# SinOncology/BreakID

Hardware: AMD Instinct MI355X
Metric: M reads/s clustered+split-scanned (higher is better)
Workload: dtype int32/u8 (+f64 sd replay)

## Files before the change

breakid_amd/capi.py:

```python
from __future__ import annotations

import ctypes as C
import math
import os
import subprocess

import numpy as np

from . import abi

_HERE = os.path.dirname(os.path.abspath(__file__))
LIB_PATH = os.path.join(_HERE, "libbreakid_hip.so")
_LIB = None


class BreakIDError(RuntimeError):
    def __init__(self, code, msg):
        super().__init__("libbreakid_hip error %d: %s" % (code, msg))
        self.code = code


def build(verbose=False):
    cmd = ["make", "-C", os.path.join(_HERE, "csrc"), "-j8"]
    r = subprocess.run(cmd, capture_output=not verbose, text=True)
    if r.returncode != 0:
        raise RuntimeError("building libbreakid_hip.so failed:\n" + (r.stdout or "")[-4000:] + (r.stderr or "")[-4000:])


EXPORTS = ["bk_init", "bk_prepare_process", "bk_free", "bk_last_error", "bk_set_stream", "bk_sync", "bk_get_stream", "bk_upload_records", "bk_records", "bk_exclude_regions", "bk_isize_stats",
           "bk_discordant_pairs", "bk_mask_and_cluster", "bk_split_evidence", "bk_cluster_summary",
           "bk_split_breakpoints", "bk_normal_support", "bk_ref_support", "bk_genotype_call", "bk_clip_support", "bk_clip_reads", "bk_base_depth", "bk_clip_rescue", "bk_junctions", "bk_junction_sides", "bk_vcf_breakend_alt", "bk_evidence", "bk_unique_support", "bk_clip_consensus", "bk_junction_fit", "bk_locus_similarity", "bk_window_coverage", "bk_call_windows", "bk_fusion_frame", "bk_link_calls", "bk_locus_partners", "bk_call_partner_sites", "bk_run", "bk_fetch", "bk_timing", "bk_timing_enable", "bk_timing_touched", "bk_group_stats", "bk_qname_hash", "bk_qname_check",
           "bk_bam_open", "bk_bam_header", "bk_bam_decode", "bk_bam_close", "bk_bam_extract", "bk_bam_names_free", "bk_bam_reads", "bk_reads_free", "bk_bam_decode_device", "bk_bam_decode_device_part", "bk_bam_decode_device_ctx", "bk_bam_dev_free", "bk_feed_release_caches", "bk_debug_bgzf_inflate", "bk_debug_std_sort", "bk_debug_scan", "bk_debug_radix_sort", "bk_debug_prims_info", "bk_sort_forms", "bk_debug_ahc", "bk_debug_points", "bk_debug_cigar", "bk_debug_vote", "bk_debug_region", "bk_shard_begin", "bk_shard_get_stats", "bk_shard_set_stats",
           "bk_shard_sd_local", "bk_shard_sd_finish", "bk_shard_buffer", "bk_shard_set_buffer", "bk_shard_group_sizes",
           "bk_shard_own_groups", "bk_shard_route_candidates", "bk_shard_group_keys", "bk_shard_route_pairs", "bk_shard_group_pairs", "bk_shard_bp_cov", "bk_shard_bp_vote", "bk_shard_bp_vote_slice", "bk_shard_bp_set_voted", "bk_shard_bp_depth", "bk_shard_bp_finish"]


def lib():
    global _LIB
    if _LIB is None:
        if not os.path.exists(LIB_PATH):
            raise BreakIDError(abi.BK_ERR_NO_DEVICE, "libbreakid_hip.so is not built (run __graft_entry__.build()); "
                                                     "there is no CPU fallback")
        try:
            import torch
        except Exception:
            pass
        L = C.CDLL(LIB_PATH)
        vp, u64p, dp = C.c_void_p, C.POINTER(C.c_uint64), C.POINTER(C.c_double)
        L.bk_init.argtypes = [C.c_int, vp, C.POINTER(C.c_char_p), C.c_int, C.POINTER(vp)]
        L.bk_free.argtypes = [vp]
        L.bk_last_error.restype = C.c_char_p
        L.bk_last_error.argtypes = [vp]
        L.bk_set_stream.argtypes = [vp, vp]
        L.bk_sync.argtypes = [vp]
        L.bk_upload_records.argtypes = [vp, C.POINTER(abi.Soa), C.c_int]
        L.bk_records.argtypes = [vp, C.POINTER(abi.Soa)]
        L.bk_exclude_regions.argtypes = [vp, C.POINTER(abi.Regions), u64p]
        L.bk_isize_stats.argtypes = [vp, dp, dp]
        L.bk_discordant_pairs.argtypes = [vp, C.c_int, C.c_double, u64p, C.POINTER(C.c_uint32)]
        L.bk_mask_and_cluster.argtypes = [vp, C.c_double, C.c_int, u64p]
        L.bk_split_evidence.argtypes = [vp, u64p]
        L.bk_cluster_summary.argtypes = [vp, C.c_double, u64p]
        L.bk_split_breakpoints.argtypes = [vp, C.c_double, u64p]
        L.bk_run.argtypes = [vp, C.c_int, C.c_int, dp, u64p]
        L.bk_normal_support.argtypes = [vp, vp, C.c_double, C.POINTER(vp), u64p]
        L.bk_ref_support.argtypes = [vp, vp, C.c_int, C.c_int, C.c_double, C.POINTER(vp), u64p]
        L.bk_genotype_call.argtypes = [C.c_uint32, C.c_uint32, C.POINTER(C.c_uint8), C.POINTER(C.c_uint8), C.POINTER(C.c_float)]
        L.bk_clip_support.argtypes = [vp, vp, C.c_int, C.c_int, C.c_double, C.POINTER(vp), u64p]
        L.bk_clip_reads.argtypes = [vp, vp, C.c_uint64, C.c_int, C.c_int, C.POINTER(vp), C.POINTER(vp), C.POINTER(vp)]
        L.bk_base_depth.argtypes = [vp, vp, vp, C.c_uint64, C.POINTER(vp)]
        L.bk_clip_rescue.argtypes = [vp, vp, vp, C.c_uint32] + [C.POINTER(C.c_uint32)] * 4
        L.bk_junctions.argtypes = [vp, C.POINTER(vp), u64p]
        L.bk_junction_sides.argtypes = [vp, C.POINTER(C.c_uint8), C.POINTER(C.c_uint8), C.POINTER(C.c_uint8)]
        L.bk_vcf_breakend_alt.argtypes = [C.c_char, C.c_int, C.c_char_p, C.c_uint32, C.c_int, C.c_char_p, C.c_size_t]
        L.bk_evidence.argtypes = [vp, C.POINTER(vp), u64p, C.POINTER(C.POINTER(C.c_uint64))]
        L.bk_unique_support.argtypes = [vp, C.POINTER(vp), u64p, C.POINTER(C.POINTER(C.c_uint64)), u64p]
        L.bk_clip_consensus.argtypes = [vp, C.POINTER(abi.Reads), vp, C.c_uint64, C.c_int, C.c_int, C.c_uint32, C.c_uint32, C.POINTER(vp), C.POINTER(vp), C.POINTER(vp)]
        L.bk_junction_fit.argtypes = [vp, C.POINTER(abi.RefSeq), vp, C.c_uint64, vp, C.c_uint32, C.c_uint32, C.c_uint32, C.c_uint32, C.POINTER(vp)]
        L.bk_locus_similarity.argtypes = [vp, C.POINTER(abi.RefSeq), vp, C.c_uint64, C.c_uint32, C.POINTER(vp)]
        L.bk_window_coverage.argtypes = [vp, vp, C.c_uint64, C.c_int, C.POINTER(vp)]
        L.bk_call_windows.argtypes = [vp, C.c_int, C.c_int, C.c_uint32, vp, vp]
        L.bk_fusion_frame.argtypes = [vp, C.POINTER(abi.TxModel), vp, C.c_uint64, C.POINTER(vp)]
        L.bk_link_calls.argtypes = [vp, vp, C.c_uint64, C.c_uint32, C.POINTER(vp)]
        L.bk_locus_partners.argtypes = [vp, vp, C.c_uint64, C.c_uint32, C.POINTER(vp)]
        L.bk_call_partner_sites.argtypes = [vp, C.c_double, vp]
        L.bk_fetch.argtypes = [vp, C.c_int, C.POINTER(vp), u64p, C.POINTER(C.POINTER(C.c_uint64)), C.POINTER(C.c_uint32)]
        L.bk_timing.argtypes = [vp, C.POINTER(C.POINTER(C.c_char_p)), C.POINTER(C.POINTER(C.c_float)),
                                C.POINTER(C.POINTER(C.c_uint64)), C.POINTER(C.c_int)]
        L.bk_timing_enable.argtypes = [vp, C.c_int]
        L.bk_timing_touched.argtypes = [vp, C.POINTER(C.POINTER(C.c_uint64)), C.POINTER(C.c_int)]
        L.bk_debug_std_sort.argtypes = [vp, vp, vp, C.c_uint32, vp]
        L.bk_debug_scan.argtypes = [vp, C.c_int, vp, C.c_uint64, C.c_int, vp]
        L.bk_debug_radix_sort.argtypes = [vp, vp, vp, C.c_uint64, C.c_int, C.c_int, vp, vp]
        L.bk_debug_prims_info.argtypes = [u64p]
        L.bk_sort_forms.argtypes = [vp, u64p]
        L.bk_debug_ahc.argtypes = [vp, vp, vp, C.c_uint32, C.c_double, vp, vp, C.POINTER(C.c_uint32)]
        L.bk_debug_points.argtypes = [vp, C.c_int, vp, vp, C.c_uint32, C.c_double, vp, vp, C.POINTER(C.c_uint32)]
        L.bk_debug_cigar.argtypes = [vp, C.c_uint32, vp, vp, vp, vp, vp, vp, vp]
        L.bk_debug_vote.argtypes = [vp, vp, C.c_uint32, vp, C.c_uint32, C.c_int32, C.c_int32, vp]
        L.bk_debug_region.argtypes = [vp, C.c_int32, C.c_uint32, C.c_uint32, C.c_uint64, vp, C.c_uint32, C.POINTER(C.c_uint32), C.POINTER(C.c_uint32),
                                      C.POINTER(C.c_uint32)]
        L.bk_shard_begin.argtypes = [vp, C.c_uint64, C.c_int]
        L.bk_shard_get_stats.argtypes = [vp, C.POINTER(abi.ShardStats)]
        L.bk_shard_set_stats.argtypes = [vp, C.POINTER(abi.ShardStats)]
        L.bk_shard_sd_local.argtypes = [vp, u64p, C.POINTER(vp), u64p]
        L.bk_shard_sd_finish.argtypes = [vp, vp, C.c_uint64, C.c_uint64, dp, dp]
        L.bk_shard_buffer.argtypes = [vp, C.c_int, C.POINTER(vp), u64p, C.POINTER(C.c_uint32)]
        L.bk_shard_set_buffer.argtypes = [vp, C.c_int, vp, C.c_uint64]
        L.bk_shard_group_sizes.argtypes = [vp, C.POINTER(C.POINTER(C.c_uint64)), C.POINTER(C.c_uint32)]
        L.bk_shard_own_groups.argtypes = [vp, vp, C.c_uint32]
        L.bk_shard_route_candidates.argtypes = [vp, C.c_uint32, C.POINTER(vp), C.POINTER(C.POINTER(C.c_uint64))]
        L.bk_shard_group_keys.argtypes = [vp, C.POINTER(C.POINTER(C.c_uint32)), C.POINTER(C.c_uint32)]
        L.bk_shard_route_pairs.argtypes = [vp, vp, C.c_uint32, C.c_uint32, C.POINTER(vp), C.POINTER(C.POINTER(C.c_uint64))]
        L.bk_shard_group_pairs.argtypes = [vp, vp, C.c_uint64, vp, C.c_uint32]
        L.bk_shard_bp_cov.argtypes = [vp, C.c_double, C.POINTER(vp), u64p]
        L.bk_shard_bp_vote.argtypes = [vp, C.c_double, vp]
        L.bk_shard_bp_vote_slice.argtypes = [vp, C.c_double, vp, C.c_uint64, C.c_uint64, C.POINTER(vp), C.POINTER(vp)]
        L.bk_shard_bp_set_voted.argtypes = [vp, vp]
        L.bk_shard_bp_depth.argtypes = [vp, C.POINTER(vp), u64p]
        L.bk_shard_bp_finish.argtypes = [vp, vp]
        L.bk_qname_hash.restype = C.c_uint64
        L.bk_qname_hash.argtypes = [C.c_char_p, C.c_size_t]
        L.bk_qname_check.restype = C.c_uint32
        L.bk_qname_check.argtypes = [C.c_char_p, C.c_size_t]
        L.bk_bam_open.argtypes = [C.c_char_p, C.POINTER(vp), C.c_char_p, C.c_size_t]
        L.bk_bam_header.argtypes = [vp, C.POINTER(C.c_int), C.POINTER(C.POINTER(C.c_char_p)), C.POINTER(C.POINTER(C.c_uint32))]
        L.bk_bam_decode.argtypes = [vp, C.POINTER(abi.Soa), C.c_char_p, C.c_size_t]
        L.bk_bam_close.argtypes = [vp]
        L.bk_bam_extract.argtypes = [C.c_char_p, C.c_char_p, vp, C.c_uint64, C.POINTER(C.c_char_p), C.c_uint64, C.POINTER(vp), u64p, C.c_char_p, C.c_size_t]
        L.bk_bam_names_free.argtypes = [vp]
        L.bk_bam_reads.argtypes = [C.c_char_p, vp, C.c_uint64, C.POINTER(abi.Reads), C.c_char_p, C.c_size_t]
        L.bk_reads_free.argtypes = [C.POINTER(abi.Reads)]
        L.bk_reads_free.restype = None
        L.bk_bam_names_free.restype = None
        L.bk_bam_decode_device.argtypes = [C.c_char_p, C.c_int, C.POINTER(vp), C.POINTER(abi.Soa), C.POINTER(C.c_int), C.POINTER(C.POINTER(C.c_char_p)),
                                           C.POINTER(C.POINTER(C.c_uint32)), C.c_char_p, C.c_size_t]
        L.bk_bam_decode_device_part.argtypes = [C.c_char_p, C.c_int, C.c_int, C.c_int, C.POINTER(vp), C.POINTER(abi.Soa), C.POINTER(C.c_int), C.POINTER(C.POINTER(C.c_char_p)),
                                           C.POINTER(C.POINTER(C.c_uint32)), C.c_char_p, C.c_size_t]
        L.bk_bam_dev_free.argtypes = [vp]
        L.bk_feed_release_caches.argtypes = []
        L.bk_feed_release_caches.restype = None
        L.bk_bam_decode_device_ctx.argtypes = [C.c_char_p, C.c_int, C.c_int, C.POINTER(vp), C.POINTER(vp), C.POINTER(C.c_int), C.POINTER(C.POINTER(C.c_char_p)),
                                               C.POINTER(C.POINTER(C.c_uint32)), C.c_char_p, C.c_size_t]
        L.bk_debug_bgzf_inflate.argtypes = [vp, C.c_uint64, vp, C.c_uint64, C.POINTER(C.c_uint64), C.POINTER(C.c_float), C.c_char_p, C.c_size_t]
        _LIB = L
    return _LIB


MULTI_LIB_PATH = os.path.join(_HERE, "libbreakid_rccl.so")
_MULTI = None
TRANSPORT_AUTO, TRANSPORT_RCCL, TRANSPORT_LOCAL = 0, 1, 2


def multi_lib():
    global _MULTI
    if _MULTI is None:
        lib()
        if not os.path.exists(MULTI_LIB_PATH):
            raise BreakIDError(abi.BK_ERR_NO_DEVICE, "libbreakid_rccl.so is not built (run __graft_entry__.build())")
        M = C.CDLL(MULTI_LIB_PATH)
        vp, dp = C.c_void_p, C.POINTER(C.c_double)
        M.bk_multi_run.argtypes = [C.POINTER(abi.Soa), vp, C.POINTER(C.c_char_p), C.c_int, C.c_int, C.c_int, C.c_int, C.c_int, dp, C.POINTER(C.c_uint64), C.POINTER(vp),
                                   C.c_char_p, C.c_size_t]
        M.bk_multi_stats.argtypes = [vp, dp, dp, C.POINTER(vp), C.POINTER(C.c_uint32)]
        M.bk_multi_free.argtypes = [vp]
        M.bk_multi_free.restype = None
        _MULTI = M
    return _MULTI


def multi_run(contigs, cols, n_gpus, transport=TRANSPORT_LOCAL, qual=20, fast=True):
    M = multi_lib()
    qc = cols.get("qcheck")
    cols = {k: np.ascontiguousarray(cols[k], dtype=dt) for k, dt in abi.SOA_COLS}
    if qc is not None:
        cols["qcheck"] = np.ascontiguousarray(qc, dtype=np.uint32)
    for k in ("cigar", "aux"):
        if cols[k].size == 0:
            cols[k] = np.zeros(1, cols[k].dtype)
    soa = abi.soa_from_numpy(cols)
    lens = np.asarray([l for _, l in contigs], dtype=np.uint32)
    names = (C.c_char_p * len(contigs))(*[n.encode() for n, _ in contigs])
    w, ncl, h = C.c_double(), C.c_uint64(), C.c_void_p()
    err = C.create_string_buffer(512)
    rc = M.bk_multi_run(C.byref(soa), lens.ctypes.data, names, len(contigs), int(n_gpus), int(transport), int(qual), int(fast), C.byref(w), C.byref(ncl), C.byref(h), err, 512)
    if rc != 0:
        raise BreakIDError(rc, err.value.decode())
    try:
        mean, sd = C.c_double(), C.c_double()
        rc = M.bk_multi_stats(h, C.byref(mean), C.byref(sd), None, None)
        if rc != 0:
            raise BreakIDError(rc, "bk_multi_stats")
        L = lib()
        clusters, _ = abi.fetch_array(L, h, lambda hh, st, d, c, g, ng: L.bk_fetch(hh, st, d, c, g, ng), abi.STAGE_CLUSTERS)
        return {"w": w.value, "n_clustered": ncl.value, "mean": mean.value, "sd": sd.value, "clusters": clusters}
    finally:
        M.bk_multi_free(h)


def prims_info():
    out = (C.c_uint64 * 4)()
    rc = lib().bk_debug_prims_info(out)
    if rc != 0:
        raise BreakIDError(rc, "bk_debug_prims_info")
    return dict(zip(("BLOCK", "SCAN_TILE", "SCAN_ONE_MAX", "RS_TILE"), (int(v) for v in out)))


def w_from(mean, sd):
    times = 2
    return times * math.sqrt(times) * (mean + 3 * sd)


def genotype_call(alt, ref):
    gt, gq, vaf = C.c_uint8(), C.c_uint8(), C.c_float()
    rc = lib().bk_genotype_call(int(alt), int(ref), C.byref(gt), C.byref(gq), C.byref(vaf))
    if rc != 0:
        raise BreakIDError(rc, "bk_genotype_call")
    return gt.value, gq.value, np.float32(vaf.value)


def junction_sides(row):
    a = np.zeros(1, abi.JUNCTION)
    a[0] = row
    r1, r2, src = C.c_uint8(), C.c_uint8(), C.c_uint8()
    rc = lib().bk_junction_sides(a.ctypes.data, C.byref(r1), C.byref(r2), C.byref(src))
    if rc != 0:
        raise BreakIDError(rc, "bk_junction_sides")
    return r1.value, r2.value, src.value


def clip_rescue(cluster, junction, clip, min_support=3):
    c, j, s = np.zeros(1, abi.CLUSTER), np.zeros(1, abi.JUNCTION), np.zeros(1, abi.CLIP_SUPPORT)
    c[0], j[0], s[0] = cluster, junction, clip
    out = [C.c_uint32() for _ in range(4)]
    rc = lib().bk_clip_rescue(c.ctypes.data, j.ctypes.data, s.ctypes.data, int(min_support), *[C.byref(o) for o in out])
    if rc < 0:
        raise BreakIDError(rc, "bk_clip_rescue")
    return tuple(o.value for o in out) if rc == 1 else None


def call_windows(cluster, right1, right2, flank, target_len):
    c = np.zeros(1, abi.CLUSTER)
    c[0] = cluster
    lens = np.ascontiguousarray(target_len, np.uint32)
    out = np.zeros(5, abi.COV_WINDOW)
    rc = lib().bk_call_windows(c.ctypes.data, int(right1), int(right2), int(flank), lens.ctypes.data, out.ctypes.data)
    if rc != 0:
        raise BreakIDError(rc, "bk_call_windows")
    return out


def call_partner_sites(cluster, w):
    c = np.zeros(1, abi.CLUSTER)
    c[0] = cluster
    out = np.zeros(2, abi.PARTNER_SITE)
    rc = lib().bk_call_partner_sites(c.ctypes.data, float(w), out.ctypes.data)
    if rc != 0:
        raise BreakIDError(rc, "bk_call_partner_sites")
    return out


def vcf_breakend_alt(ref_base, own_right, mate_chr, mate_pos, mate_right, cap=None):
    chrom = mate_chr.encode()
    if cap is None:
        cap = len(chrom) + 32
    buf = C.create_string_buffer(max(int(cap), 1))
    rc = lib().bk_vcf_breakend_alt(ref_base.encode(), int(bool(own_right)), chrom, int(mate_pos), int(bool(mate_right)), buf, int(cap))
    if rc != 0:
        raise BreakIDError(rc, "bk_vcf_breakend_alt")
    return buf.value.decode()


class Context:

    def __init__(self, contigs, device=0):
        self.L = lib()
        self.contigs = list(contigs)
        lens = np.asarray([l for _, l in contigs], dtype=np.uint32)
        names = (C.c_char_p * len(contigs))(*[n.encode() for n, _ in contigs])
        h = C.c_void_p()
        rc = self.L.bk_init(device, lens.ctypes.data, names, len(contigs), C.byref(h))
        if rc != 0:
            raise BreakIDError(rc, (self.L.bk_last_error(None) or b"").decode())
        self.h = h
        self._keep = None

    def close(self):
        if self.h:
            self.L.bk_free(self.h)
            self.h = None

    def __del__(self):
        try:
            self.close()
        except Exception:
            pass

    def _check(self, rc):
        if rc != 0:
            raise BreakIDError(rc, (self.L.bk_last_error(self.h) or b"").decode())

    def set_stream(self, hip_stream_handle):
        self._check(self.L.bk_set_stream(self.h, C.c_void_p(hip_stream_handle)))

    def sync(self):
        self._check(self.L.bk_sync(self.h))

    def upload(self, cols):
        qc = cols.get("qcheck")
        cols = {k: np.ascontiguousarray(cols[k], dtype=dt) for k, dt in abi.SOA_COLS}
        if qc is not None:
            cols["qcheck"] = np.ascontiguousarray(qc, dtype=np.uint32)
        for k in ("cigar", "aux"):
            if cols[k].size == 0:
                cols[k] = np.zeros(1, cols[k].dtype)
        soa = abi.soa_from_numpy(cols)
        self._keep = (cols, soa)
        self._check(self.L.bk_upload_records(self.h, C.byref(soa), abi.BK_MEM_HOST))

    def attach_device_table(self, table):
        self._keep = table
        self._check(self.L.bk_upload_records(self.h, C.byref(table.soa), abi.BK_MEM_DEVICE))

    def upload_soa(self, handle):
        self._keep = handle
        self._check(self.L.bk_upload_records(self.h, C.byref(handle.soa), abi.BK_MEM_HOST))

    def attach_device(self, ptrs, n, n_cigar_words, n_aux_bytes):
        s = abi.Soa()
        s.n = n
        for name, _ in abi.SOA_COLS:
            setattr(s, name, ptrs[name])
        if ptrs.get("qcheck"):
            s.qcheck = ptrs["qcheck"]
        if ptrs.get("side"):
            s.side = ptrs["side"]
        s.n_cigar_words = n_cigar_words
        s.n_aux_bytes = n_aux_bytes
        self._keep = (ptrs, s)
        self._check(self.L.bk_upload_records(self.h, C.byref(s), abi.BK_MEM_DEVICE))

    def exclude_regions(self, tid, beg, end):
        tid, beg, end = (np.ascontiguousarray(a, np.int32).reshape(-1) for a in (tid, beg, end))
        if not len(tid) == len(beg) == len(end):
            raise ValueError("exclude_regions: tid, beg and end differ in length")
        r = abi.Regions(tid.ctypes.data, beg.ctypes.data, end.ctypes.data, len(tid))
        n = C.c_uint64()
        self._check(self.L.bk_exclude_regions(self.h, C.byref(r), C.byref(n)))
        return n.value

    def isize_stats(self):
        m, s = C.c_double(), C.c_double()
        self._check(self.L.bk_isize_stats(self.h, C.byref(m), C.byref(s)))
        return m.value, s.value

    def shard_begin(self, rec_base, qual=20):
        self._check(self.L.bk_shard_begin(self.h, int(rec_base), int(qual)))

    def shard_get_stats(self):
        st = abi.ShardStats()
        self._check(self.L.bk_shard_get_stats(self.h, C.byref(st)))
        return st

    def shard_set_stats(self, st):
        self._check(self.L.bk_shard_set_stats(self.h, C.byref(st)))

    def shard_sd_local(self):
        lt, ex, nex = C.c_uint64(), C.c_void_p(), C.c_uint64()
        self._check(self.L.bk_shard_sd_local(self.h, C.byref(lt), C.byref(ex), C.byref(nex)))
        return lt.value, ex.value, nex.value

    def shard_sd_finish(self, all_ex_ptr, n_all, l_grand):
        m, s = C.c_double(), C.c_double()
        self._check(self.L.bk_shard_sd_finish(self.h, C.c_void_p(all_ex_ptr or 0), int(n_all), int(l_grand), C.byref(m), C.byref(s)))
        return m.value, s.value

    def discordant_pairs(self, qual, w):
        n, g = C.c_uint64(), C.c_uint32()
        self._check(self.L.bk_discordant_pairs(self.h, qual, w, C.byref(n), C.byref(g)))
        return n.value, g.value

    def mask_and_cluster(self, w, fast):
        n = C.c_uint64()
        self._check(self.L.bk_mask_and_cluster(self.h, w, int(fast), C.byref(n)))
        return n.value

    def split_evidence(self):
        n = C.c_uint64()
        self._check(self.L.bk_split_evidence(self.h, C.byref(n)))
        return n.value

    def cluster_summary(self, w):
        n = C.c_uint64()
        self._check(self.L.bk_cluster_summary(self.h, w, C.byref(n)))
        return n.value

    def split_breakpoints(self, w, count=True):
        n = C.c_uint64()
        self._check(self.L.bk_split_breakpoints(self.h, w, C.byref(n) if count else None))
        return n.value

    def normal_support(self, normal, w):
        data, n = C.c_void_p(), C.c_uint64()
        self._check(self.L.bk_normal_support(self.h, normal.h, w, C.byref(data), C.byref(n)))
        if not n.value:
            return np.zeros(0, abi.NORMAL_SUPPORT)
        buf = (C.c_char * (n.value * abi.NORMAL_SUPPORT.itemsize)).from_address(data.value)
        return np.frombuffer(buf, dtype=abi.NORMAL_SUPPORT, count=n.value).copy()

    def junctions(self):
        data, n = C.c_void_p(), C.c_uint64()
        self._check(self.L.bk_junctions(self.h, C.byref(data), C.byref(n)))
        if not n.value:
            return np.zeros(0, abi.JUNCTION)
        buf = (C.c_char * (n.value * abi.JUNCTION.itemsize)).from_address(data.value)
        return np.frombuffer(buf, dtype=abi.JUNCTION, count=n.value).copy()

    def evidence(self):
        data, n, off = C.c_void_p(), C.c_uint64(), C.POINTER(C.c_uint64)()
        self._check(self.L.bk_evidence(self.h, C.byref(data), C.byref(n), C.byref(off)))
        rows = np.zeros(0, abi.EVIDENCE)
        if n.value:
            buf = (C.c_char * (n.value * abi.EVIDENCE.itemsize)).from_address(data.value)
            rows = np.frombuffer(buf, dtype=abi.EVIDENCE, count=n.value).copy()
        d2, ncl = C.c_void_p(), C.c_uint64()
        self._check(self.L.bk_fetch(self.h, abi.STAGE_CLUSTERS, C.byref(d2), C.byref(ncl), None, None))
        return rows, np.ctypeslib.as_array(off, shape=(ncl.value + 1,)).copy()

    def unique_support(self, listing=True):
        data, n, first, n_rows = C.c_void_p(), C.c_uint64(), C.POINTER(C.c_uint64)(), C.c_uint64()
        if listing:
            self._check(self.L.bk_unique_support(self.h, C.byref(data), C.byref(n), C.byref(first), C.byref(n_rows)))
        else:
            self._check(self.L.bk_unique_support(self.h, C.byref(data), C.byref(n), None, None))
        rows = np.zeros(0, abi.UNIQUE_SUPPORT)
        if n.value:
            buf = (C.c_char * (n.value * abi.UNIQUE_SUPPORT.itemsize)).from_address(data.value)
            rows = np.frombuffer(buf, dtype=abi.UNIQUE_SUPPORT, count=n.value).copy()
        if not listing:
            return rows
        return rows, (np.ctypeslib.as_array(first, shape=(n_rows.value,)).copy() if n_rows.value else np.zeros(0, np.uint64))

    def clip_consensus(self, reads, sites, mapq_min, min_clip, max_len=64, min_depth=2, col_depth=True):
        sites = np.ascontiguousarray(sites, abi.CLIP_SITE)
        assert sites.ndim == 1
        n = len(sites)
        t, keep = reads_struct(reads)
        out, bases, depth = C.c_void_p(), C.c_void_p(), C.c_void_p()
        self._check(self.L.bk_clip_consensus(self.h, C.byref(t), sites.ctypes.data if n else None, n, int(mapq_min), int(min_clip), int(max_len), int(min_depth),
                                             C.byref(out), C.byref(bases), C.byref(depth) if col_depth else None))
        del keep
        if not n:
            return np.zeros(0, abi.CONSENSUS), np.zeros((0, int(max_len)), np.uint8), (np.zeros((0, int(max_len)), np.uint32) if col_depth else None)
        buf = (C.c_char * (n * abi.CONSENSUS.itemsize)).from_address(out.value)
        rows = np.frombuffer(buf, dtype=abi.CONSENSUS, count=n).copy()
        b = np.ctypeslib.as_array(C.cast(bases, C.POINTER(C.c_uint8)), shape=(n, int(max_len))).copy()
        d = np.ctypeslib.as_array(C.cast(depth, C.POINTER(C.c_uint32)), shape=(n, int(max_len))).copy() if col_depth else None
        return rows, b, d

    def junction_fit(self, ref, probes, query, max_shift=32, max_ins=32, max_hom=32):
        probes = np.ascontiguousarray(probes, abi.JUNCTION_PROBE)
        query = np.ascontiguousarray(query, np.uint8)
        assert probes.ndim == 1 and query.ndim == 2 and query.shape[0] == len(probes)
        n, max_len = len(probes), query.shape[1]
        t, keep = refseq_struct(ref)
        out = C.c_void_p()
        self._check(self.L.bk_junction_fit(self.h, C.byref(t), probes.ctypes.data if n else None, n, query.ctypes.data if n else None, max_len, int(max_shift), int(max_ins),
                                           int(max_hom), C.byref(out)))
        del keep
        if not n:
            return np.zeros(0, abi.JUNCTION_FIT)
        buf = (C.c_char * (n * abi.JUNCTION_FIT.itemsize)).from_address(out.value)
        return np.frombuffer(buf, dtype=abi.JUNCTION_FIT, count=n).copy()

    def locus_similarity(self, ref, pairs, flank=150):
        pairs = np.ascontiguousarray(pairs, abi.LOCUS_PAIR)
        assert pairs.ndim == 1
        n = len(pairs)
        t, keep = refseq_struct(ref)
        out = C.c_void_p()
        self._check(self.L.bk_locus_similarity(self.h, C.byref(t), pairs.ctypes.data if n else None, n, int(flank), C.byref(out)))
        del keep
        if not n:
            return np.zeros(0, abi.LOCUS_SIM)
        buf = (C.c_char * (n * abi.LOCUS_SIM.itemsize)).from_address(out.value)
        return np.frombuffer(buf, dtype=abi.LOCUS_SIM, count=n).copy()

    def ref_support(self, records, mapq_min, anchor, w):
        data, n = C.c_void_p(), C.c_uint64()
        self._check(self.L.bk_ref_support(self.h, records.h, int(mapq_min), int(anchor), w, C.byref(data), C.byref(n)))
        if not n.value:
            return np.zeros(0, abi.REF_SUPPORT)
        buf = (C.c_char * (n.value * abi.REF_SUPPORT.itemsize)).from_address(data.value)
        return np.frombuffer(buf, dtype=abi.REF_SUPPORT, count=n.value).copy()

    def clip_support(self, records, mapq_min, min_clip, w):
        data, n = C.c_void_p(), C.c_uint64()
        self._check(self.L.bk_clip_support(self.h, records.h, int(mapq_min), int(min_clip), w, C.byref(data), C.byref(n)))
        if not n.value:
            return np.zeros(0, abi.CLIP_SUPPORT)
        buf = (C.c_char * (n.value * abi.CLIP_SUPPORT.itemsize)).from_address(data.value)
        return np.frombuffer(buf, dtype=abi.CLIP_SUPPORT, count=n.value).copy()

    def clip_reads(self, sites, mapq_min, min_clip, listing=True):
        sites = np.ascontiguousarray(sites, abi.CLIP_SITE)
        assert sites.ndim == 1
        n = len(sites)
        counts, rows, off = C.c_void_p(), C.c_void_p(), C.c_void_p()
        self._check(self.L.bk_clip_reads(self.h, sites.ctypes.data if n else None, n, int(mapq_min), int(min_clip), C.byref(counts),
                                         C.byref(rows) if listing else None, C.byref(off) if listing else None))
        cnt = np.ctypeslib.as_array(C.cast(counts, C.POINTER(C.c_uint32)), shape=(n,)).copy() if n else np.zeros(0, np.uint32)
        if not listing:
            return cnt
        site_off = np.ctypeslib.as_array(C.cast(off, C.POINTER(C.c_uint64)), shape=(n + 1,)).copy()
        out = np.zeros(0, abi.CLIP_READ)
        if site_off[-1]:
            buf = (C.c_char * (int(site_off[-1]) * abi.CLIP_READ.itemsize)).from_address(rows.value)
            out = np.frombuffer(buf, dtype=abi.CLIP_READ, count=int(site_off[-1])).copy()
        return cnt, out, site_off

    def base_depth(self, tid, pos):
        tid = np.ascontiguousarray(tid, np.int32)
        pos = np.ascontiguousarray(pos, np.uint32)
        assert tid.shape == pos.shape and tid.ndim == 1
        data = C.c_void_p()
        self._check(self.L.bk_base_depth(self.h, tid.ctypes.data, pos.ctypes.data, len(tid), C.byref(data)))
        if not len(tid):
            return np.zeros(0, np.uint32)
        return np.ctypeslib.as_array(C.cast(data, C.POINTER(C.c_uint32)), shape=(len(tid),)).copy()

    def window_coverage(self, windows, mapq_min=0):
        windows = np.ascontiguousarray(windows, abi.COV_WINDOW)
        assert windows.ndim == 1
        n = len(windows)
        out = C.c_void_p()
        self._check(self.L.bk_window_coverage(self.h, windows.ctypes.data if n else None, n, int(mapq_min), C.byref(out)))
        if not n:
            return np.zeros(0, abi.WINDOW_COV)
        buf = (C.c_char * (n * abi.WINDOW_COV.itemsize)).from_address(out.value)
        return np.frombuffer(buf, dtype=abi.WINDOW_COV, count=n).copy()

    def fusion_frame(self, model, sites):
        sites = np.ascontiguousarray(sites, abi.FRAME_SITE)
        assert sites.ndim == 1
        n = len(sites)
        t, keep = txmodel_struct(model.cols if isinstance(model, TxModel) else model)
        out = C.c_void_p()
        self._check(self.L.bk_fusion_frame(self.h, C.byref(t), sites.ctypes.data if n else None, n, C.byref(out)))
        del keep
        if not n:
            return np.zeros(0, abi.FRAME_CALL)
        buf = (C.c_char * (n * abi.FRAME_CALL.itemsize)).from_address(out.value)
        return np.frombuffer(buf, dtype=abi.FRAME_CALL, count=n).copy()

    def link_calls(self, sites, max_dist=1000):
        sites = np.ascontiguousarray(sites, abi.LINK_SITE)
        assert sites.ndim == 1
        n = len(sites)
        out = C.c_void_p()
        self._check(self.L.bk_link_calls(self.h, sites.ctypes.data if n else None, n, max_dist, C.byref(out)))
        if not n:
            return np.zeros(0, abi.CALL_LINK)
        buf = (C.c_char * (n * abi.CALL_LINK.itemsize)).from_address(out.value)
        return np.frombuffer(buf, dtype=abi.CALL_LINK, count=n).copy()

    def locus_partners(self, sites, max_gap):
        sites = np.ascontiguousarray(sites, abi.PARTNER_SITE)
        assert sites.ndim == 1
        n = len(sites)
        out = C.c_void_p()
        self._check(self.L.bk_locus_partners(self.h, sites.ctypes.data if n else None, n, max_gap, C.byref(out)))
        if not n:
            return np.zeros(0, abi.LOCUS_PARTNERS)
        buf = (C.c_char * (n * abi.LOCUS_PARTNERS.itemsize)).from_address(out.value)
        return np.frombuffer(buf, dtype=abi.LOCUS_PARTNERS, count=n).copy()

    def run(self, qual=20, fast=True):
        w, n = C.c_double(), C.c_uint64()
        self._check(self.L.bk_run(self.h, qual, int(fast), C.byref(w), C.byref(n)))
        return w.value, n.value

    def fetch(self, stage):
        def fn(h, st, d, c, g, ng):
            return self.L.bk_fetch(h, st, d, c, g, ng)
        try:
            return abi.fetch_array(self.L, self.h, fn, stage)
        except RuntimeError:
            self._check(-1 if not self.L.bk_last_error(self.h) else abi.BK_ERR_ARG)
            raise

    def debug_std_sort(self, key, group_off):
        key = np.ascontiguousarray(key, np.uint32)
        group_off = np.ascontiguousarray(group_off, np.uint64)
        perm = np.zeros(len(key), np.uint32)
        self._check(self.L.bk_debug_std_sort(self.h, key.ctypes.data, group_off.ctypes.data, len(group_off) - 1, perm.ctypes.data))
        return perm

    def debug_scan(self, values, in_place=False):
        values = np.ascontiguousarray(values)
        assert values.ndim == 1 and values.dtype in (np.uint32, np.uint64), values.dtype
        out = np.zeros(len(values) + 1, values.dtype)
        self._check(self.L.bk_debug_scan(self.h, values.dtype.itemsize, values.ctypes.data if len(values) else None, len(values), int(in_place), out.ctypes.data))
        return out

    def debug_radix_sort(self, keys, vals, begin_bit, end_bit):
        keys = np.ascontiguousarray(keys, np.uint64)
        vals = np.ascontiguousarray(vals, np.uint32)
        assert keys.ndim == 1 and keys.shape == vals.shape
        n = len(keys)
        ko, vo = np.zeros(n, np.uint64), np.zeros(n, np.uint32)
        self._check(self.L.bk_debug_radix_sort(self.h, keys.ctypes.data if n else None, vals.ctypes.data if n else None, n, int(begin_bit), int(end_bit),
                                               ko.ctypes.data if n else None, vo.ctypes.data if n else None))
        return ko, vo

    def sort_forms(self):
        out = (C.c_uint64 * 3)()
        self._check(self.L.bk_sort_forms(self.h, out))
        return tuple(int(v) for v in out)

    def debug_ahc(self, x, y, w):
        x = np.ascontiguousarray(x, np.uint32)
        y = np.ascontiguousarray(y, np.uint32)
        n = len(x)
        idx = np.zeros(max(n, 1), np.uint32)
        cl = np.zeros(max(n, 1), np.int32)
        m = C.c_uint32()
        self._check(self.L.bk_debug_ahc(self.h, x.ctypes.data, y.ctypes.data, n, float(w), idx.ctypes.data, cl.ctypes.data, C.byref(m)))
        return idx[:m.value].copy(), cl[:m.value].copy()

    def debug_points(self, mode, x, y, w):
        x = np.ascontiguousarray(x, np.uint32)
        y = np.ascontiguousarray(y, np.uint32)
        n = len(x)
        idx = np.zeros(max(n, 1), np.uint32)
        cl = np.zeros(max(n, 1), np.int32)
        m = C.c_uint32()
        self._check(self.L.bk_debug_points(self.h, {"mask": 0, "iso": 1, "fast": 2}[mode], x.ctypes.data, y.ctypes.data, n, float(w), idx.ctypes.data,
                                           cl.ctypes.data, C.byref(m)))
        return idx[:m.value].copy(), cl[:m.value].copy()

    def debug_cigar(self, rows):
        kind = np.asarray([1 if r[0] == "b" else 0 for r in rows], np.uint8)
        c1 = bytearray()
        o1 = [0]
        for r in rows:
            while r[0] == "b" and len(c1) % 4:
                c1 += b"\0"
                o1[-1] = len(c1)
            c1 += np.asarray(r[1], np.uint32).tobytes() if r[0] == "b" else r[1].encode()
            o1.append(len(c1))
        c2 = bytearray()
        o2 = [0]
        for r in rows:
            c2 += r[2].encode()
            o2.append(len(c2))
        o1a, o2a = np.asarray(o1, np.uint32), np.asarray(o2, np.uint32)
        b1 = np.frombuffer(bytes(c1) + b"\0" * 16, np.uint8)
        b2 = np.frombuffer(bytes(c2) + b"\0" * 16, np.uint8)
        e = np.asarray([r[3] for r in rows], np.int32)
        out = np.zeros((len(rows), 6), np.int32)
        self._check(self.L.bk_debug_cigar(self.h, len(rows), kind.ctypes.data, o1a.ctypes.data, b1.ctypes.data, o2a.ctypes.data, b2.ctypes.data, e.ctypes.data,
                                          out.ctypes.data))
        return out

    def debug_vote(self, s1, s2, p1_tid, p2_tid):
        s1 = np.ascontiguousarray(s1, abi.SPLIT)
        s2 = np.ascontiguousarray(s2, abi.SPLIT)
        out = np.zeros(3, np.int32)
        self._check(self.L.bk_debug_vote(self.h, s1.ctypes.data, len(s1), s2.ctypes.data, len(s2), p1_tid, p2_tid, out.ctypes.data))
        return tuple(int(v) for v in out)

    def debug_region(self, tid, start, end, depth_pos, cap=4096):
        out = np.zeros(cap, abi.SPLIT)
        n, cov, depth = C.c_uint32(), C.c_uint32(), C.c_uint32()
        self._check(self.L.bk_debug_region(self.h, tid, start, end, depth_pos, out.ctypes.data, cap, C.byref(n), C.byref(cov), C.byref(depth)))
        return out[:min(n.value, cap)].copy(), n.value, cov.value, depth.value

    def timing_enable(self, on=True):
        self._check(self.L.bk_timing_enable(self.h, int(on)))

    def timing(self):
        names = C.POINTER(C.c_char_p)()
        ms = C.POINTER(C.c_float)()
        by = C.POINTER(C.c_uint64)()
        n = C.c_int()
        self._check(self.L.bk_timing(self.h, C.byref(names), C.byref(ms), C.byref(by), C.byref(n)))
        return [(names[i].decode(), float(ms[i]), int(by[i])) for i in range(n.value)]

    def timing_touched(self):
        t = C.POINTER(C.c_uint64)()
        n = C.c_int()
        self._check(self.L.bk_timing_touched(self.h, C.byref(t), C.byref(n)))
        return [int(t[i]) for i in range(n.value)]


class DeviceBamTable:

    def __init__(self, L, h, soa, contigs):
        self.L, self.h, self.soa, self.contigs = L, h, soa, contigs

    def close(self):
        if self.h:
            self.L.bk_bam_dev_free(self.h)
            self.h = None


def decode_bam_device(path, device=0):
    L = lib()
    h = C.c_void_p()
    err = C.create_string_buffer(512)
    s = abi.Soa()
    nt = C.c_int()
    names = C.POINTER(C.c_char_p)()
    lens = C.POINTER(C.c_uint32)()
    rc = L.bk_bam_decode_device(path.encode(), device, C.byref(h), C.byref(s), C.byref(nt), C.byref(names), C.byref(lens), err, 512)
    if rc != 0:
        raise BreakIDError(rc, err.value.decode())
    contigs = [(names[i].decode(), int(lens[i])) for i in range(nt.value)]
    return DeviceBamTable(L, h, s, contigs)


def decode_bam_device_part(path, part, parts, device=0):
    L = lib()
    h = C.c_void_p()
    err = C.create_string_buffer(512)
    s = abi.Soa()
    nt = C.c_int()
    names = C.POINTER(C.c_char_p)()
    lens = C.POINTER(C.c_uint32)()
    rc = L.bk_bam_decode_device_part(path.encode(), device, part, parts, C.byref(h), C.byref(s), C.byref(nt), C.byref(names), C.byref(lens), err, 512)
    if rc != 0:
        raise BreakIDError(rc, err.value.decode())
    contigs = [(names[i].decode(), int(lens[i])) for i in range(nt.value)]
    return DeviceBamTable(L, h, s, contigs)


def decode_bam_device_ctx(path, qual=20, device=0):
    L = lib()
    hb, hc = C.c_void_p(), C.c_void_p()
    err = C.create_string_buffer(512)
    nt = C.c_int()
    names = C.POINTER(C.c_char_p)()
    lens = C.POINTER(C.c_uint32)()
    rc = L.bk_bam_decode_device_ctx(path.encode(), device, qual, C.byref(hb), C.byref(hc), C.byref(nt), C.byref(names), C.byref(lens), err, 512)
    if rc != 0:
        raise BreakIDError(rc, err.value.decode())
    contigs = [(names[i].decode(), int(lens[i])) for i in range(nt.value)]
    ctx = Context.__new__(Context)
    ctx.L, ctx.contigs, ctx.h = L, contigs, hc
    table = DeviceBamTable(L, hb, None, contigs)
    ctx._keep = table
    s = abi.Soa()
    ctx._check(L.bk_records(hc, C.byref(s)))
    table.soa = s
    return ctx, table


def bam_extract(in_bam, out_bam, keys, tags):
    keys = np.ascontiguousarray(keys, abi.READ_KEY)
    tag_arr = (C.c_char_p * max(len(tags), 1))(*[t.encode() for t in tags])
    names, n = C.c_void_p(), C.c_uint64()
    err = C.create_string_buffer(512)
    L = lib()
    rc = L.bk_bam_extract(os.fsencode(in_bam), None if out_bam is None else os.fsencode(out_bam), keys.ctypes.data if len(keys) else None, len(keys),
                          tag_arr if len(tags) else None, len(tags), C.byref(names), C.byref(n), err, 512)
    if rc != 0:
        raise BreakIDError(rc, err.value.decode())
    try:
        out, p = [], names.value
        for _ in range(len(keys)):
            t = C.string_at(p)
            out.append(t.decode())
            p += len(t) + 1
    finally:
        L.bk_bam_names_free(names)
    return out, n.value


def reads_struct(reads):
    t, keep = abi.Reads(), []
    t.n = len(reads["tid"])
    for name, dt in abi.READS_COLS:
        if name not in reads:
            continue
        a = np.ascontiguousarray(reads[name], dt)
        keep.append(a)
        setattr(t, name, a.ctypes.data if a.size else None)
    return t, keep


def refseq_struct(ref):
    t, keep = abi.RefSeq(), []
    t.n_segs = len(ref["tid"])
    for name, dt in abi.REFSEQ_COLS:
        a = np.ascontiguousarray(ref[name], dt)
        keep.append(a)
        setattr(t, name, a.ctypes.data if a.size else None)
    return t, keep


def txmodel_struct(cols):
    t, keep = abi.TxModel(), []
    t.n_tx, t.n_parts = len(cols["tid"]), len(cols["ex_start"])
    for name, dt in abi.TXMODEL_COLS:
        a = np.ascontiguousarray(cols[name], dt)
        keep.append(a)
        setattr(t, name, a.ctypes.data if a.size else None)
    return t, keep


class TxModel:

    def __init__(self, rows):
        rows = sorted(rows, key=lambda r: (r[0], r[1]))
        self.names = [r[5] if len(r) > 5 else "" for r in rows]
        self.genes = [r[6] if len(r) > 6 else "" for r in rows]
        off, starts, ends = [0], [], []
        for r in rows:
            starts += [p[0] for p in r[4]]
            ends += [p[1] for p in r[4]]
            off.append(len(starts))
        self.cols = {"tid": np.asarray([r[0] for r in rows], np.int32), "tx_start": np.asarray([r[1] for r in rows], np.uint32),
                     "tx_end": np.asarray([r[2] for r in rows], np.uint32),
                     "strand": np.asarray([{"+": 0, "-": 1}.get(r[3], r[3]) for r in rows], np.uint8),
                     "ex_off": np.asarray(off if rows else [], np.uint32), "ex_start": np.asarray(starts, np.uint32), "ex_end": np.asarray(ends, np.uint32)}

    def __len__(self):
        return len(self.names)

    @classmethod
    def from_refgene(cls, lines, contig_names):
        tid_of = {n: i for i, n in enumerate(contig_names)}
        rows, dropped = [], 0
        for line in lines:
            f = line.rstrip("\n").split("\t")
            if "NR_" in f[1]:
                continue
            if f[2] not in tid_of:
                dropped += 1
                continue
            cs, ce, ne = int(f[6]), int(f[7]), int(f[8])
            xs = [int(v) for v in f[9].split(",") if v][:ne]
            xe = [int(v) for v in f[10].split(",") if v][:ne]
            parts = [(max(s, cs), min(e, ce)) for s, e in zip(xs, xe) if cs != ce and s < ce and e > cs]
            rows.append((tid_of[f[2]], int(f[4]), int(f[5]), f[3], parts, f[1], f[12]))
        return cls(rows), dropped


def bam_reads(path, keys):
    keys = np.ascontiguousarray(keys, abi.READ_KEY)
    L = lib()
    t = abi.Reads()
    err = C.create_string_buffer(512)
    rc = L.bk_bam_reads(os.fsencode(path), keys.ctypes.data if len(keys) else None, len(keys), C.byref(t), err, 512)
    if rc != 0:
        raise BreakIDError(rc, err.value.decode())
    try:
        n = t.n
        cols = {}

        def col(name, dt, cnt):
            ptr = getattr(t, name)
            if cnt == 0 or not ptr:
                return np.zeros(0, dt)
            buf = (C.c_char * (cnt * np.dtype(dt).itemsize)).from_address(ptr)
            return np.frombuffer(buf, dtype=dt, count=cnt).copy()
        for name, dt in abi.READS_COLS:
            if name in ("cigar", "seq"):
                continue
            cols[name] = col(name, dt, n + 1 if name in ("cigar_off", "seq_off") else n)
        cols["cigar"] = col("cigar", np.uint32, int(cols["cigar_off"][-1]))
        cols["seq"] = col("seq", np.uint8, int(cols["seq_off"][-1]))
        return cols
    finally:
        L.bk_reads_free(C.byref(t))


class BamTable:

    def __init__(self, L, h, soa):
        self.L, self.h, self.soa = L, h, soa
        n = soa.n
        self.nbytes = n * (4 * 5 + 2 + 1 + 8) + (n + 1) * 8 + soa.n_cigar_words * 4 + soa.n_aux_bytes

    def close(self):
        if self.h:
            self.L.bk_bam_close(self.h)
            self.h = None


def decode_bam(path, keep=False):
    L = lib()
    h = C.c_void_p()
    err = C.create_string_buffer(512)
    rc = L.bk_bam_open(path.encode(), C.byref(h), err, 512)
    if rc != 0:
        raise BreakIDError(rc, err.value.decode())
    try:
        nt = C.c_int()
        names = C.POINTER(C.c_char_p)()
        lens = C.POINTER(C.c_uint32)()
        L.bk_bam_header(h, C.byref(nt), C.byref(names), C.byref(lens))
        contigs = [(names[i].decode(), int(lens[i])) for i in range(nt.value)]
        s = abi.Soa()
        rc = L.bk_bam_decode(h, C.byref(s), err, 512)
        if rc != 0:
            raise BreakIDError(rc, err.value.decode())
        n = s.n
        sizes = {"cigar_off": n + 1, "aux_off": n + 1, "cigar": max(1, s.n_cigar_words), "aux": max(1, s.n_aux_bytes)}
        cols = {}
        for name, dt in abi.SOA_COLS_ALL:
            cnt = sizes.get(name, n)
            ptr = getattr(s, name)
            if cnt == 0 or not ptr:
                cols[name] = np.zeros(0, dt)
                continue
            buf = (C.c_char * (cnt * np.dtype(dt).itemsize)).from_address(ptr)
            cols[name] = np.frombuffer(buf, dtype=dt, count=cnt).copy()
        cols["cigar"] = cols["cigar"][: s.n_cigar_words]
        cols["aux"] = cols["aux"][: s.n_aux_bytes]
        if keep:
            t = BamTable(L, h, s)
            h = None
            return contigs, cols, t
        return contigs, cols
    finally:
        if h:
            L.bk_bam_close(h)
```

breakid_amd/csrc/api.hip:

```cpp
#include <algorithm>
#include <cmath>
#include <limits>
#include <cstring>
#include <numeric>

#include "bk_common.h"
#include "prims.h"
#include "stream.h"
#include "join.h"
#include "cluster.h"
#include "bp.h"
#include "normal.h"
#include "genotype.h"
#include "clip.h"
#include "junction.h"
#include "evidence.h"
#include "unique.h"
#include "consensus.h"
#include "jfit.h"
#include "locsim.h"
#include "coverage.h"
#include "frame.h"
#include "link.h"
#include "partners.h"
// ... 1955 lines not shown
    };
    if (elem_bytes == 4)
      run(uint32_t(0));
    else
      run(uint64_t(0));
  });
}

int bk_debug_radix_sort(bk_ctx *ctx, const uint64_t *keys, const uint32_t *vals, uint64_t n, int begin_bit, int end_bit, uint64_t *keys_out, uint32_t *vals_out)
{
  return guarded(ctx, [&] {
    if (n && (!keys || !vals || !keys_out || !vals_out)) throw bk_error(BK_ERR_ARG, "bk_debug_radix_sort: null argument");
    if (begin_bit < 0 || end_bit > 64) throw bk_error(BK_ERR_ARG, "bk_debug_radix_sort: bits outside [0, 64]");
    prims::radix_check_count(n);
    if (!n) return;
    prims::RadixBufs &rb = ctx->dbg_radix;
    uint64_t *dk = ctx->dbg_in.as<uint64_t>(n);
    uint32_t *dv = ctx->dbg_vals.as<uint32_t>(n);
    HIP_CHECK(hipMemsetAsync(rb.keys_alt.as<uint64_t>(n), 0xA5, n * 8, ctx->st));
    HIP_CHECK(hipMemsetAsync(rb.vals_alt.as<uint32_t>(n), 0xA5, n * 4, ctx->st));
    HIP_CHECK(hipMemcpyAsync(dk, keys, n * 8, hipMemcpyHostToDevice, ctx->st));
    HIP_CHECK(hipMemcpyAsync(dv, vals, n * 4, hipMemcpyHostToDevice, ctx->st));
    uint64_t *ko = nullptr;
    uint32_t *vo = nullptr;
    prims::radix_sort_pairs(dk, dv, n, begin_bit, end_bit, rb, ctx->st, &ko, &vo);
    HIP_CHECK(hipMemcpyAsync(keys_out, ko, n * 8, hipMemcpyDeviceToHost, ctx->st));
    HIP_CHECK(hipMemcpyAsync(vals_out, vo, n * 4, hipMemcpyDeviceToHost, ctx->st));
    HIP_CHECK(hipStreamSynchronize(ctx->st));
  });
}

int bk_debug_prims_info(uint64_t out[4])
{
  if (!out) return BK_ERR_ARG;
  out[0] = prims::BLOCK;
  out[1] = prims::SCAN_TILE;
  out[2] = prims::SCAN_ONE_MAX;
  out[3] = prims::RS_TILE;
  return BK_OK;
}

int bk_sort_forms(bk_ctx *ctx, uint64_t out[3])
{
  return guarded(ctx, [&] {
    if (!out) throw bk_error(BK_ERR_ARG, "bk_sort_forms: null output");
    ctx->stage.sort_forms(out);
  });
}

int bk_debug_ahc(bk_ctx *ctx, const uint32_t *x, const uint32_t *y, uint32_t n, double w, uint32_t *idx_out, int32_t *cluster_out, uint32_t *n_out)
{
  return guarded(ctx, [&] {
    if (!x || !y || !idx_out || !cluster_out || !n_out) throw bk_error(BK_ERR_ARG, "bk_debug_ahc: null argument");
    std::vector<bk_pair> hp(n);
    for (uint32_t i = 0; i < n; ++i)
    {
      memset(&hp[i], 0, sizeof(bk_pair));
      hp[i].x = x[i];
      hp[i].y = y[i];
    }
    DevBuf dp, dcl;
    PairList L;
    L.n = n;
    L.ng = 1;
    std::vector<uint32_t> iota(n), gof(n, 0);
    std::iota(iota.begin(), iota.end(), 0u);
    uint64_t goff[2] = {0, n};
    HIP_CHECK(hipMemcpy(dp.as<bk_pair>(n + 1), hp.data(), n * sizeof(bk_pair), hipMemcpyHostToDevice));
    HIP_CHECK(hipMemcpy(L.idx.as<uint32_t>(n + 1), iota.data(), n * 4, hipMemcpyHostToDevice));
    HIP_CHECK(hipMemcpy(L.gof.as<uint32_t>(n + 1), gof.data(), n * 4, hipMemcpyHostToDevice));
    HIP_CHECK(hipMemcpy(L.goff.as<uint64_t>(2), goff, 16, hipMemcpyHostToDevice));
    ahc_cluster_all(dp.get<bk_pair>(), L, w, dcl, ctx->stage.ab, ctx->stage.cb(), ctx->st);
    *n_out = (uint32_t) L.n;
    if (L.n)
    {
      HIP_CHECK(hipMemcpyAsync(idx_out, L.idx.get<uint32_t>(), L.n * 4, hipMemcpyDeviceToHost, ctx->st));
      HIP_CHECK(hipMemcpyAsync(cluster_out, dcl.get<uint32_t>(), L.n * 4, hipMemcpyDeviceToHost, ctx->st));
    }
    HIP_CHECK(hipStreamSynchronize(ctx->st));
  });
}

}

namespace
{
struct FeedLink
{
  int device = 0, mapq_min = 20;
  bk_ctx *ctx = nullptr;
  int rc = BK_OK;
  std::string err;
  uint64_t done = 0;
  bool prepared = false, overflow = false;
  hipEvent_t t0 = nullptr, t1 = nullptr;
  template <class F> void guard(F &&f)
  {
    if (rc != BK_OK) return;
    try
    {
      f();
    }
    catch (const bk_error &e)
    {
      rc = e.code;
      err = e.msg;
    }
  }
};
void link_header(void *u, int nt, const char *const *names, const uint32_t *lens)
{
  FeedLink *L = (FeedLink *) u;
  if (L->ctx || L->rc != BK_OK) return;
  L->rc = bk_init(L->device, lens, names, nt, &L->ctx);
  if (L->rc != BK_OK) L->err = bk_last_error(nullptr);
}
void link_reset(void *u)
{
  FeedLink *L = (FeedLink *) u;
  L->guard([&] {
    if (L->ctx) HIP_CHECK(hipStreamSynchronize(L->ctx->st));
    L->done = 0;
    L->prepared = false;
    L->overflow = false;
  });
}
void link_before_move(void *u)
{
  FeedLink *L = (FeedLink *) u;
  L->guard([&] {
    if (L->ctx) HIP_CHECK(hipStreamSynchronize(L->ctx->st));
  });
}
void link_chunk(void *u, const bk_soa *cols, uint64_t n_ready, uint64_t n_est, hipEvent_t ready)
{
  FeedLink *L = (FeedLink *) u;
  L->guard([&] {
    bk_ctx *c = L->ctx;
    if (!c || n_ready < (uint64_t) STREAM_V + 1) return;
    c->rec = *cols;
    c->have_records = true;
    c->mapq_min = L->mapq_min;
    if (!L->prepared)
    {
      stream_prepare(c, n_est + n_est / 4);
      L->prepared = true;
    }
    const uint64_t lim = (n_ready - 1) / STREAM_V * STREAM_V;
    if (lim <= L->done) return;
    HIP_CHECK(hipStreamWaitEvent(c->st, ready, 0));
    StreamArgs a = stream_args(c, lim);
    a.q_begin = L->done / STREAM_V;
    launch_stream(a, c->st);
    L->done = lim;
  });
}
}


extern "C" {

int bk_bam_decode_device_ctx(const char *path, int device, int mapq_min, bk_bam_dev **bam_out, bk_ctx **ctx_out, int *n_targets, const char *const **names,
                             const uint32_t **lens, char *err, size_t errlen)
{
  auto fail = [&](int code, const std::string &m) {
    if (err && errlen) snprintf(err, errlen, "%s", m.c_str());
    return code;
  };
  if (!path || !bam_out || !ctx_out) return fail(BK_ERR_ARG, "bk_bam_decode_device_ctx: null argument");
  *bam_out = nullptr;
  *ctx_out = nullptr;
  FeedLink L;
  L.device = device;
  L.mapq_min = mapq_min;
  FeedConsumer fc;
  fc.user = &L;
  fc.on_header = link_header;
  fc.on_chunk = link_chunk;
  fc.before_move = link_before_move;
  fc.on_reset = link_reset;
  bk_soa cols;
  bk_bam_dev *bam = nullptr;
  int rc = bam_decode_device_impl(path, device, &bam, &cols, n_targets, names, lens, err, errlen, &fc);
  if (rc == BK_OK && L.rc != BK_OK) rc = fail(L.rc, L.err);
  if (rc == BK_OK && !L.ctx) rc = fail(BK_ERR_IO, "bk_bam_decode_device_ctx: no header");
  if (rc != BK_OK)
  {
    if (L.ctx) bk_free(L.ctx);
    if (bam) bk_bam_dev_free(bam);
    return rc;
  }
  bk_ctx *c = L.ctx;
  rc = guarded(c, [&] {
    const uint64_t done = L.prepared ? L.done : 0;
    c->stream_done = c->stats_done = c->clustered = false;
    c->rec = cols;
    c->have_records = true;
    c->mapq_min = mapq_min;
    c->rec_base = 0;
    bool ok = false;
    if (L.prepared)
    {
      Scope s(c, "k_stream", 39ull * cols.n + 4ull * cols.n_cigar_words);
      StreamArgs a = stream_args(c, cols.n);
      a.q_begin = done / STREAM_V;
      launch_stream(a, c->st);
      ok = stream_finish(c);
    }
    if (ok)
      stream_rare_path(c);
    else
      run_stream(c);
    if (bk_debug("feed"))
      fprintf(stderr, "[feed/stream] stream pass %s: %llu of %llu records went through k_stream while the file was still arriving\n", ok ? "overlapped" : "after the feed",
              (unsigned long long) (ok ? done : 0), (unsigned long long) cols.n);
  });
  if (rc != BK_OK)
  {
    fail(rc, c->err);
    bk_free(c);
    bk_bam_dev_free(bam);
    return rc;
  }
  *bam_out = bam;
  *ctx_out = c;
  return BK_OK;
}

int bk_group_stats(bk_ctx *ctx, const bk_group_stat **out, uint32_t *n_groups)
{
  return guarded(ctx, [&] {
    if (!out || !n_groups) throw bk_error(BK_ERR_ARG, "bk_group_stats: null output");
    if (!ctx->clustered) throw bk_error(BK_ERR_ARG, "bk_group_stats: call bk_mask_and_cluster (and bk_cluster_summary) first");
    const uint32_t ng = ctx->jr.n_groups;
    std::vector<uint64_t> iso(ng + 1, 0), clu(ng + 1, 0);
    std::vector<uint32_t> kmax(ng + 1, 0);
    if (ng)
    {
      HIP_CHECK(hipMemcpyAsync(iso.data(), ctx->stage.iso_goff.get<uint64_t>(), ((uint64_t) ng + 1) * 8, hipMemcpyDeviceToHost, ctx->st));
      HIP_CHECK(hipMemcpyAsync(clu.data(), ctx->stage.list.goff.get<uint64_t>(), ((uint64_t) ng + 1) * 8, hipMemcpyDeviceToHost, ctx->st));
      if (ctx->stage.list.n && ctx->bb.kmax.p) HIP_CHECK(hipMemcpyAsync(kmax.data(), ctx->bb.kmax.get<uint32_t>(), (uint64_t) ng * 4, hipMemcpyDeviceToHost, ctx->st));
      HIP_CHECK(hipStreamSynchronize(ctx->st));
    }
    ctx->f_gstats.assign(ng, bk_group_stat{});
    for (uint32_t l = 0; l < ng; ++l)
    {
      const uint32_t g = ctx->lex_to_num[l];
      bk_group_stat &o = ctx->f_gstats[l];
      const uint32_t k = ctx->gkey_host[g];
      o.p1_tid = (int32_t) (k / (uint32_t) (ctx->nt + 1)) - 1;
      o.p2_tid = (int32_t) (k % (uint32_t) (ctx->nt + 1)) - 1;
      o.n_scan = ctx->gstart_host[g + 1] - ctx->gstart_host[g];
      o.n_isolated_removed = iso[g + 1] - iso[g];
      o.n_clustered = clu[g + 1] - clu[g];
      o.cluster_id_end = o.n_clustered ? kmax[g] : 0;
      o.ordinal = ctx->glex_host[g];
    }
    *out = ctx->f_gstats.data();
    *n_groups = ng;
  });
}

int bk_debug_points(bk_ctx *ctx, int mode, const uint32_t *x, const uint32_t *y, uint32_t n, double w, uint32_t *idx_out, int32_t *cluster_out, uint32_t *n_out)
{
  return guarded(ctx, [&] {
    if ((n && (!x || !y)) || !idx_out || !n_out || mode < 0 || mode > 2) throw bk_error(BK_ERR_ARG, "bk_debug_points: bad argument");
    std::vector<bk_pair> hp(n);
    for (uint32_t i = 0; i < n; ++i)
    {
      memset(&hp[i], 0, sizeof(bk_pair));
      hp[i].x = x[i];
      hp[i].y = y[i];
    }
    DevBuf dp, dcl, dgof, dgoff;
    PairList L;
    std::vector<uint32_t> gof(n, 0);
    uint64_t goff[2] = {0, n};
    if (n) HIP_CHECK(hipMemcpy(dp.as<bk_pair>(n + 1), hp.data(), n * sizeof(bk_pair), hipMemcpyHostToDevice));
    if (n) HIP_CHECK(hipMemcpy(dgof.as<uint32_t>(n + 1), gof.data(), n * 4, hipMemcpyHostToDevice));
    HIP_CHECK(hipMemcpy(dgoff.as<uint64_t>(2), goff, 16, hipMemcpyHostToDevice));
    const bk_pair *pairs = dp.as<bk_pair>(n + 1);
    remove_isolated_all(pairs, dgof.get<uint32_t>(), dgoff.get<uint64_t>(), 1, mode == 1 ? n : 0, w, L, ctx->stage.cb(), ctx->st);
    if (mode != 1)
    {
      L.n = n;
      L.ng = 1;
      std::vector<uint32_t> iota(n);
      std::iota(iota.begin(), iota.end(), 0u);
      if (n) HIP_CHECK(hipMemcpy(L.idx.as<uint32_t>(n + 1), iota.data(), n * 4, hipMemcpyHostToDevice));
      if (n) HIP_CHECK(hipMemcpy(L.gof.as<uint32_t>(n + 1), gof.data(), n * 4, hipMemcpyHostToDevice));
      HIP_CHECK(hipMemcpy(L.goff.as<uint64_t>(2), goff, 16, hipMemcpyHostToDevice));
      if (mode == 0)
        debug_mask_list(pairs, L, (long) w, ctx->stage.cb(), ctx->st);
      else
        fast_cluster_all(pairs, L, w, dcl, ctx->stage.cb(), ctx->st);
    }
    *n_out = (uint32_t) L.n;
    if (L.n)
    {
      HIP_CHECK(hipMemcpyAsync(idx_out, L.idx.get<uint32_t>(), L.n * 4, hipMemcpyDeviceToHost, ctx->st));
      if (mode == 2 && cluster_out) HIP_CHECK(hipMemcpyAsync(cluster_out, dcl.get<uint32_t>(), L.n * 4, hipMemcpyDeviceToHost, ctx->st));
    }
    HIP_CHECK(hipStreamSynchronize(ctx->st));
  });
}

int bk_debug_cigar(bk_ctx *ctx, uint32_t n, const uint8_t *kind, const uint32_t *c1_off, const uint8_t *c1, const uint32_t *c2_off, const uint8_t *c2, const int32_t *e,
                   int32_t *out6)
{
  return guarded(ctx, [&] {
    if (!n) return;
    if (!kind || !c1_off || !c1 || !c2_off || !c2 || !e || !out6) throw bk_error(BK_ERR_ARG, "bk_debug_cigar: null argument");
    DevBuf dk, d1o, d1, d2o, d2, de, dout;
    HIP_CHECK(hipMemcpy(dk.as<uint8_t>(n), kind, n, hipMemcpyHostToDevice));
    HIP_CHECK(hipMemcpy(d1o.as<uint32_t>(n + 1), c1_off, (n + 1) * 4, hipMemcpyHostToDevice));
    HIP_CHECK(hipMemcpy(d1.as<uint8_t>(c1_off[n] + 16), c1, c1_off[n], hipMemcpyHostToDevice));
    HIP_CHECK(hipMemcpy(d2o.as<uint32_t>(n + 1), c2_off, (n + 1) * 4, hipMemcpyHostToDevice));
    HIP_CHECK(hipMemcpy(d2.as<uint8_t>(c2_off[n] + 16), c2, c2_off[n], hipMemcpyHostToDevice));
    HIP_CHECK(hipMemcpy(de.as<int32_t>(n), e, n * 4, hipMemcpyHostToDevice));
    int32_t *o = dout.as<int32_t>(6ull * n);
    debug_cigar(dk.get<uint8_t>(), d1o.get<uint32_t>(), d1.get<uint8_t>(), d2o.get<uint32_t>(), d2.get<uint8_t>(), de.get<int32_t>(), n, o, ctx->st);
    HIP_CHECK(hipMemcpyAsync(out6, o, 24ull * n, hipMemcpyDeviceToHost, ctx->st));
    HIP_CHECK(hipStreamSynchronize(ctx->st));
  });
}

int bk_debug_vote(bk_ctx *ctx, const bk_split *side1, uint32_t n1, const bk_split *side2, uint32_t n2, int32_t p1_tid, int32_t p2_tid, int32_t *out3)
{
  return guarded(ctx, [&] {
    if ((n1 && !side1) || (n2 && !side2) || !out3) throw bk_error(BK_ERR_ARG, "bk_debug_vote: null argument");
    const uint32_t pos1 = 100000, pos2 = 300000;
    std::vector<bk_split> t;
    auto put = [&](const bk_split *src, uint32_t n, int32_t tid, uint32_t pos, uint64_t salt) {
      for (uint32_t i = 0; i < n + 2; ++i)
      {
        bk_split s;
        if (i < n)
          s = src[i];
        else
        {
          memset(&s, 0, sizeof s);
          s.qhash = 0xD00D000000000000ull + salt + i;
          s.prim_chr = s.sec_chr = -7;
        }
        s.tid = tid;
        s.pos = (int32_t) pos;
        s.endpos = (int32_t) pos + 50;
        t.push_back(s);
      }
    };
    put(side1, n1, p1_tid, pos1, 0);
    put(side2, n2, p2_tid, pos2, 1000);
    std::stable_sort(t.begin(), t.end(), [](const bk_split &a, const bk_split &b) { return (uint32_t) a.tid != (uint32_t) b.tid ? (uint32_t) a.tid < (uint32_t) b.tid : a.pos < b.pos; });
    for (size_t i = 0; i < t.size(); ++i) t[i].rec = i;
    bk_cluster c;
    memset(&c, 0, sizeof c);
    c.p1_tid = p1_tid;
    c.p2_tid = p2_tid;
    c.p1_mean = pos1 + 10;
    c.p2_mean = pos2 + 10;
    c.p1_exact = 0xFFFFFFFFu;
    c.p2_exact = -1;
    DevBuf dt, dc, dcov;
    HIP_CHECK(hipMemcpy(dt.as<bk_split>(t.size() + 1), t.data(), t.size() * sizeof(bk_split), hipMemcpyHostToDevice));
    HIP_CHECK(hipMemcpy(dc.as<bk_cluster>(2), &c, sizeof c, hipMemcpyHostToDevice));
    const uint32_t cov[2] = {5, 5};
    HIP_CHECK(hipMemcpy(dcov.as<uint32_t>(4), cov, 8, hipMemcpyHostToDevice));
    bp_vote(dt.get<bk_split>(), t.size(), dc.get<bk_cluster>(), 1, 1000.0, 200, dcov.get<uint32_t>(), ctx->d_hdr.get<int32_t>(), ctx->bb, ctx->st);
    uint32_t voted = 0;
    HIP_CHECK(hipMemcpyAsync(&voted, ctx->bb.voted.get<uint32_t>(), 4, hipMemcpyDeviceToHost, ctx->st));
    HIP_CHECK(hipMemcpyAsync(&c, dc.get<bk_cluster>(), sizeof c, hipMemcpyDeviceToHost, ctx->st));
    HIP_CHECK(hipStreamSynchronize(ctx->st));
    out3[0] = voted ? (int32_t) c.p1_exact : -1;
    out3[1] = voted ? c.p2_exact : -1;
    out3[2] = voted ? (int32_t) c.n_sr : 0;
  });
}

int bk_debug_region(bk_ctx *ctx, int32_t tid, uint32_t start, uint32_t end, uint64_t depth_pos, bk_split *out, uint32_t cap, uint32_t *n_out, uint32_t *cov_out,
                    uint32_t *depth_out)
{
  return guarded(ctx, [&] {
    if (!ctx->stream_done) run_stream(ctx);
    ensure_splits_sorted(ctx);
    DevBuf dout, dres;
    bk_split *o = dout.as<bk_split>((uint64_t) cap + 1);
    uint32_t *res = dres.as<uint32_t>(4);
    debug_region(rec_view(ctx), ctx->d_split.get<bk_split>(), ctx->hc.n_split, tid, start, end, (int) ctx->hc.max_span, depth_pos, o, cap, res, ctx->st);
    uint32_t h[4] = {0, 0, 0, 0};
    HIP_CHECK(hipMemcpyAsync(h, res, 16, hipMemcpyDeviceToHost, ctx->st));
    HIP_CHECK(hipStreamSynchronize(ctx->st));
    const uint32_t n = h[0] < cap ? h[0] : cap;
    if (n && out) HIP_CHECK(hipMemcpy(out, o, n * sizeof(bk_split), hipMemcpyDeviceToHost));
    if (n_out) *n_out = h[0];
    if (cov_out) *cov_out = h[1];
    if (depth_out) *depth_out = h[2];
  });
}

int bk_timing_enable(bk_ctx *ctx, int on)
{
  return guarded(ctx, [&] {
    ctx->timing = on != 0;
    for (auto &t : ctx->timers)
    {
      if (t.a) (void) hipEventDestroy(t.a);
      if (t.b) (void) hipEventDestroy(t.b);
    }
    ctx->timers.clear();
  });
}

int bk_timing(bk_ctx *ctx, const char *const **names, const float **ms, const uint64_t **bytes, int *n)
{
  return guarded(ctx, [&] {
    HIP_CHECK(hipStreamSynchronize(ctx->st));
    Timing &t = ctx->tout;
    t.names.clear(); t.ms.clear(); t.bytes.clear(); t.touched.clear(); t.cnames.clear();
    for (auto &s : ctx->timers)
    {
      float v = 0;
      HIP_CHECK(hipEventElapsedTime(&v, s.a, s.b));
      t.names.push_back(s.name);
      t.ms.push_back(v);
      t.bytes.push_back(s.bytes);
      t.touched.push_back(s.touched);
    }
    for (auto &s : t.names) t.cnames.push_back(s.c_str());
    if (names) *names = t.cnames.data();
    if (ms) *ms = t.ms.data();
    if (bytes) *bytes = t.bytes.data();
    if (n) *n = (int) t.names.size();
  });
}

int bk_timing_touched(bk_ctx *ctx, const uint64_t **touched, int *n)
{
  return guarded(ctx, [&] {
    if (touched) *touched = ctx->tout.touched.data();
    if (n) *n = (int) ctx->tout.touched.size();
  });
}

}
```

breakid_amd/csrc/cluster.h:

```cpp
#pragma once
#include "bk_common.h"
#include "prims.h"
#include "sortemu.h"

struct PairList
{
  uint64_t n = 0;
  uint32_t ng = 0;
  DevBuf idx;
  DevBuf gof;
  DevBuf goff;
  uint64_t total(hipStream_t st) const;
};

struct ClusterBufs
{
  std::vector<uint32_t> heavy_x, heavy_y;
  bool observe = false;
  uint64_t max_group_bound = 0;
  DevBuf key, perm, tmp, cnt, off, off2, idx2, gof2, goff2, jump, mark, apos, kid, kprev2, k1, k2, pk, knum, clfull, small, scan_tmp;
  SortEmuBufs se;
  prims::RadixBufs radix;
};

void remove_isolated_all(const bk_pair *pairs, const uint32_t *gof0, const uint64_t *gstart, uint32_t ng, uint64_t n, double w, PairList &L, ClusterBufs &b, hipStream_t st,
                         const uint32_t *drop_group = nullptr);
void remove_isolated_begin(const bk_pair *pairs, const uint32_t *gof0, const uint64_t *gstart, uint32_t ng, uint64_t n, double w, PairList &L, ClusterBufs &b, hipStream_t st,
                           const uint32_t *drop_group = nullptr, const uint64_t *gstart_host = nullptr, const uint8_t *keep_host = nullptr);
void remove_isolated_end(const bk_pair *pairs, PairList &L, ClusterBufs &b, hipStream_t st);
void list_subset_ranges(const PairList &src, const uint64_t *src_goff_host, const uint8_t *keep_host, PairList &dst, hipStream_t st);
void drop_small_groups(PairList &L, ClusterBufs &b, hipStream_t st);
void fast_cluster_all(const bk_pair *pairs, PairList &L, double w, DevBuf &cluster_out, ClusterBufs &b, hipStream_t st);
void merge_lists_many(const PairList *const *lists, const uint32_t *const *cls, int K, PairList &out, DevBuf *cl_out, hipStream_t st);
void debug_mask_list(const bk_pair *pairs, PairList &L, long dist, ClusterBufs &b, hipStream_t st);
```

breakid_amd/csrc/cluster.hip:

```cpp
#include "bk_common.h"
#include "prims.h"
#include "sortemu.h"
#include "cluster.h"

namespace
{
constexpr uint32_t END = 0xFFFFFFFFu;

__global__ __launch_bounds__(256) void k_iota(uint32_t *__restrict__ a, uint64_t n)
{
  uint64_t i = (uint64_t) blockIdx.x * blockDim.x + threadIdx.x;
  if (i < n) a[i] = (uint32_t) i;
}
__global__ __launch_bounds__(256) void k_gather_key(const bk_pair *__restrict__ pairs, const uint32_t *__restrict__ idx, uint64_t n, int use_y, uint32_t *__restrict__ key)
{
  uint64_t p = (uint64_t) blockIdx.x * blockDim.x + threadIdx.x;
  if (p < n) key[p] = use_y ? pairs[idx[p]].y : pairs[idx[p]].x;
}
__global__ __launch_bounds__(256) void k_gather_u32(const uint32_t *__restrict__ src, const uint32_t *__restrict__ perm, uint64_t n, uint32_t *__restrict__ dst)
{
  uint64_t p = (uint64_t) blockIdx.x * blockDim.x + threadIdx.x;
  if (p < n) dst[p] = src[perm[p]];
}

__device__ __forceinline__ long absdiff(uint32_t a, uint32_t b)
{
  long d = (long) (int32_t) (a - b);
  return d < 0 ? -d : d;
}

__global__ __launch_bounds__(256) void k_mask_count(const bk_pair *__restrict__ pairs, const uint32_t *__restrict__ idx, const uint32_t *__restrict__ gof,
                                                    const uint64_t *__restrict__ goff, uint64_t n, long dist, uint32_t *__restrict__ cnt)
{
  uint64_t p = (uint64_t) blockIdx.x * blockDim.x + threadIdx.x;
  if (p >= n) return;
  uint32_t g = gof[p];
  uint64_t gs = goff[g], ge = goff[g + 1];
  uint64_t np = ge - gs, i = p - gs;
  uint32_t c = 0;
  if (np >= 3 && i >= 1 && i + 1 < np)
  {
    const bk_pair a = pairs[idx[p]], l = pairs[idx[p - 1]], r = pairs[idx[p + 1]];
    long ll = absdiff(l.x, a.x), lr = absdiff(r.x, a.x);
    long Lx = ll < lr ? ll : lr;
    ll = absdiff(l.y, a.y);
    lr = absdiff(r.y, a.y);
    long Ly = ll < lr ? ll : lr;
    if (!(Lx > dist || Ly > dist)) c += 1;
    if (i == 1)
    {
      long fx = absdiff(a.x, r.x), fy = absdiff(a.y, r.y);
      if (!(fx > dist || fy > dist)) c += 1;
    }
  }
  cnt[p] = c;
}

__global__ __launch_bounds__(256) void k_expand(const uint32_t *__restrict__ cnt, const uint32_t *__restrict__ off, const uint32_t *__restrict__ idx,
                                                const uint32_t *__restrict__ gof, uint64_t n, uint32_t *__restrict__ oidx, uint32_t *__restrict__ ogof)
{
  uint64_t p = (uint64_t) blockIdx.x * blockDim.x + threadIdx.x;
  if (p >= n) return;
  uint32_t c = cnt[p], o = off[p];
  for (uint32_t k = 0; k < c; ++k)
  {
    oidx[o + k] = idx[p];
    ogof[o + k] = gof[p];
  }
}
__global__ void k_new_goff(const uint32_t *__restrict__ off, const uint64_t *__restrict__ goff, uint32_t ng, uint64_t n, uint64_t *__restrict__ ogoff)
{
  uint32_t g = blockIdx.x * blockDim.x + threadIdx.x;
  if (g > ng) return;
  uint64_t s = g < ng ? goff[g] : n;
  ogoff[g] = off[s];
}

__global__ __launch_bounds__(256) void k_fast_next(const uint32_t *__restrict__ key, const uint32_t *__restrict__ gof, const uint64_t *__restrict__ goff, uint64_t n, double w,
                                                   uint32_t *__restrict__ nxt)
{
  uint64_t p = (uint64_t) blockIdx.x * blockDim.x + threadIdx.x;
  if (p >= n) return;
  uint32_t g = gof[p];
  uint64_t ge = goff[g + 1];
  if (p + 1 >= ge)
  {
    nxt[p] = END;
    return;
  }
  double lim = (double) (long) key[p] + w;
  uint64_t lo = p + 1, hi = ge;
  while (lo < hi)
  {
    uint64_t m = (lo + hi) >> 1;
    if ((double) key[m] <= lim) lo = m + 1; else hi = m;
  }
  if (lo > ge - 1) lo = ge - 1;
  nxt[p] = (uint32_t) lo;
}
__global__ void k_mark_starts(const uint64_t *__restrict__ goff, uint32_t ng, uint32_t *__restrict__ mark)
{
  uint32_t g = blockIdx.x * blockDim.x + threadIdx.x;
  if (g >= ng) return;
  if (goff[g + 1] > goff[g]) mark[goff[g]] = 1;
}
constexpr uint32_t FW_TILE = 1024, FW_LEVELS = 10;
__global__ __launch_bounds__(FW_TILE) void k_fw_exit(const uint32_t *__restrict__ nxt, uint64_t n, uint32_t *__restrict__ exitp)
{
  __shared__ uint32_t e[FW_TILE];
  const uint64_t t0 = (uint64_t) blockIdx.x * FW_TILE, p = t0 + threadIdx.x;
  const uint64_t tend = t0 + FW_TILE;
  e[threadIdx.x] = p < n ? nxt[p] : END;
  for (uint32_t r = 0; r < FW_LEVELS; ++r)
  {
    __syncthreads();
    const uint32_t v = e[threadIdx.x];
    if (v != END && v < tend) e[threadIdx.x] = e[v - t0];
  }
  __syncthreads();
  if (p < n) exitp[p] = e[threadIdx.x];
}
__global__ __launch_bounds__(64) void k_fw_chain(const uint64_t *__restrict__ goff, uint32_t ng, const uint32_t *__restrict__ exitp, uint32_t *__restrict__ mark)
{
  const uint32_t g = blockIdx.x * blockDim.x + threadIdx.x;
  if (g >= ng || goff[g + 1] <= goff[g]) return;
  uint32_t p = (uint32_t) goff[g];
  for (;;)
  {
    const uint32_t q = exitp[p];
    if (q == END) break;
    mark[q] = 1;
    p = q;
  }
}
__global__ __launch_bounds__(FW_TILE) void k_fw_mark(const uint32_t *__restrict__ nxt, uint64_t n, uint32_t *__restrict__ mark)
{
  __shared__ uint16_t j[FW_LEVELS][FW_TILE];
  __shared__ uint32_t m[FW_TILE];
  constexpr uint16_t OUT = 0xFFFFu;
  const uint64_t t0 = (uint64_t) blockIdx.x * FW_TILE, p = t0 + threadIdx.x;
  const uint32_t i = threadIdx.x;
  uint32_t v = p < n ? nxt[p] : END;
  j[0][i] = (v != END && v < t0 + FW_TILE) ? (uint16_t) (v - t0) : OUT;
  m[i] = p < n ? mark[p] : 0u;
  for (uint32_t k = 1; k < FW_LEVELS; ++k)
  {
    __syncthreads();
    const uint16_t a = j[k - 1][i];
    j[k][i] = a == OUT ? OUT : j[k - 1][a];
  }
  for (int k = FW_LEVELS - 1; k >= 0; --k)
  {
    __syncthreads();
    if (m[i])
    {
      const uint16_t t = j[k][i];
      if (t != OUT) m[t] = 1u;
    }
  }
  __syncthreads();
  if (p < n) mark[p] = m[i];
}

__global__ __launch_bounds__(256) void k_anchor_pos(const uint32_t *__restrict__ mark, const uint32_t *__restrict__ ascan, uint64_t n, uint32_t *__restrict__ apos)
{
  uint64_t p = (uint64_t) blockIdx.x * blockDim.x + threadIdx.x;
  if (p < n && mark[p]) apos[ascan[p]] = (uint32_t) p;
}
__global__ __launch_bounds__(256) void k_fast_keep(const uint32_t *__restrict__ mark, const uint32_t *__restrict__ ascan, const uint32_t *__restrict__ apos,
                                                   const uint32_t *__restrict__ nxt, uint64_t n, uint32_t *__restrict__ keep, uint32_t *__restrict__ kid)
{
  uint64_t p = (uint64_t) blockIdx.x * blockDim.x + threadIdx.x;
  if (p >= n) return;
  uint32_t ord = ascan[p] + mark[p] - 1;
  uint32_t a = apos[ord];
  uint32_t e = nxt[a];
  keep[p] = (e != END && e - a >= 2) ? 1u : 0u;
  kid[p] = ord;
}
__global__ __launch_bounds__(256) void k_compact3(const uint32_t *__restrict__ keep, const uint32_t *__restrict__ off, uint64_t n, const uint32_t *__restrict__ a0,
                                                  const uint32_t *__restrict__ a1, const uint32_t *__restrict__ a2, const uint32_t *__restrict__ a3, uint32_t *__restrict__ o0,
                                                  uint32_t *__restrict__ o1, uint32_t *__restrict__ o2, uint32_t *__restrict__ o3)
{
  uint64_t p = (uint64_t) blockIdx.x * blockDim.x + threadIdx.x;
  if (p >= n || !keep[p]) return;
  uint32_t o = off[p];
  o0[o] = a0[p];
  if (a1) o1[o] = a1[p];
  if (a2) o2[o] = a2[p];
  if (a3) o3[o] = a3[p];
}
__global__ __launch_bounds__(256) void k_pack_k(const uint32_t *__restrict__ k1, const uint32_t *__restrict__ k2, uint64_t n, int kbits, uint64_t *__restrict__ key, uint32_t *__restrict__ val)
{
  uint64_t p = (uint64_t) blockIdx.x * blockDim.x + threadIdx.x;
  if (p >= n) return;
  key[p] = ((uint64_t) k2[p] << kbits) | k1[p];
  val[p] = (uint32_t) p;
}
__global__ __launch_bounds__(256) void k_run_flag(const uint64_t *__restrict__ key, uint64_t n, uint32_t *__restrict__ flag)
{
  uint64_t p = (uint64_t) blockIdx.x * blockDim.x + threadIdx.x;
  if (p < n) flag[p] = (p == 0 || key[p] != key[p - 1]) ? 1u : 0u;
}
__global__ __launch_bounds__(256) void k_uid_stats(const uint32_t *__restrict__ flag, const uint32_t *__restrict__ fscan, const uint32_t *__restrict__ val, uint64_t n,
                                                   uint32_t *__restrict__ uid_of_elem, uint32_t *__restrict__ ustart, uint32_t *__restrict__ uminpos)
{
  uint64_t q = (uint64_t) blockIdx.x * blockDim.x + threadIdx.x;
  if (q >= n) return;
  const uint32_t f = flag[q];
  uint32_t u = fscan[q] + f - 1;
  uint32_t e = val[q];
  uid_of_elem[e] = u;
  if (f)
  {
    ustart[u] = (uint32_t) q;
    uminpos[u] = e;
  }
  if (q == n - 1) ustart[u + 1] = (uint32_t) n;
}
__global__ __launch_bounds__(256) void k_first_flag(const uint32_t *__restrict__ uid, const uint32_t *__restrict__ ustart, const uint32_t *__restrict__ uminpos, uint64_t n,
                                                    uint32_t *__restrict__ keep, uint32_t *__restrict__ first)
{
  uint64_t p = (uint64_t) blockIdx.x * blockDim.x + threadIdx.x;
  if (p >= n) return;
  uint32_t u = uid[p];
  uint32_t k = ustart[u + 1] - ustart[u] >= 2 ? 1u : 0u;
  keep[p] = k;
  first[p] = (k && uminpos[u] == (uint32_t) p) ? 1u : 0u;
}
__global__ __launch_bounds__(256) void k_knum(const uint32_t *__restrict__ first, const uint32_t *__restrict__ fscan, const uint32_t *__restrict__ uid,
                                              const uint32_t *__restrict__ gof, const uint64_t *__restrict__ goff, uint64_t n, uint32_t *__restrict__ knum)
{
  uint64_t p = (uint64_t) blockIdx.x * blockDim.x + threadIdx.x;
  if (p >= n || !first[p]) return;
  uint64_t gs = goff[gof[p]];
  knum[uid[p]] = fscan[p] - fscan[gs] + 1;
}
__global__ __launch_bounds__(256) void k_cluster_of(const uint32_t *__restrict__ uid, const uint32_t *__restrict__ knum, const uint32_t *__restrict__ keep, uint64_t n,
                                                    uint32_t *__restrict__ cl)
{
  uint64_t p = (uint64_t) blockIdx.x * blockDim.x + threadIdx.x;
  if (p < n) cl[p] = keep[p] ? knum[uid[p]] : 0u;
}
__global__ void k_group_small(const uint64_t *__restrict__ goff, uint32_t ng, uint32_t *__restrict__ small)
{
  uint32_t g = blockIdx.x * blockDim.x + threadIdx.x;
  if (g < ng) small[g] = (goff[g + 1] - goff[g]) < 2 ? 1u : 0u;
}
__global__ __launch_bounds__(256) void k_drop_small(const uint32_t *__restrict__ gof, const uint32_t *__restrict__ small, uint64_t n, uint32_t *__restrict__ keep)
{
  uint64_t p = (uint64_t) blockIdx.x * blockDim.x + threadIdx.x;
  if (p < n) keep[p] = small[gof[p]] ? 0u : 1u;
}
}

uint64_t PairList::total(hipStream_t st) const
{
  uint64_t t = 0;
  if (ng == 0) return 0;
  HIP_CHECK(hipMemcpyAsync(&t, goff.get<uint64_t>() + ng, 8, hipMemcpyDeviceToHost, st));
  HIP_CHECK(hipStreamSynchronize(st));
  return t;
}

static inline unsigned nb(uint64_t n) { return cdiv(n ? n : 1, 256); }
static void filter_groups(PairList &L, const uint32_t *drop, ClusterBufs &b, hipStream_t st);

static void sort_list(const bk_pair *pairs, PairList &L, int use_y, uint32_t **extra, int n_extra, ClusterBufs &b, hipStream_t st)
{
  if (L.n == 0) return;
  uint32_t *key = b.key.as<uint32_t>(L.n), *perm = b.perm.as<uint32_t>(L.n);
  hipLaunchKernelGGL(k_gather_key, dim3(nb(L.n)), dim3(256), 0, st, pairs, L.idx.get<uint32_t>(), L.n, use_y, key);
  hipLaunchKernelGGL(k_iota, dim3(nb(L.n)), dim3(256), 0, st, perm, L.n);
  b.se.heavy = b.observe ? (use_y ? &b.heavy_y : &b.heavy_x) : nullptr;
  std_sort_groups(key, perm, L.gof.get<uint32_t>(), L.goff.get<uint64_t>(), L.ng, L.n, b.se, st);
  b.se.heavy = nullptr;
  uint32_t *tmp = b.tmp.as<uint32_t>(L.n);
  auto apply = [&](uint32_t *arr) {
    hipLaunchKernelGGL(k_gather_u32, dim3(nb(L.n)), dim3(256), 0, st, arr, perm, L.n, tmp);
    HIP_CHECK(hipMemcpyAsync(arr, tmp, L.n * 4, hipMemcpyDeviceToDevice, st));
  };
  apply(L.idx.get<uint32_t>());
  for (int k = 0; k < n_extra; ++k) apply(extra[k]);
}

static void mask_list(const bk_pair *pairs, PairList &L, long dist, ClusterBufs &b, hipStream_t st)
{
  if (L.n == 0) return;
  uint32_t *cnt = b.cnt.as<uint32_t>(L.n + 1);
  hipLaunchKernelGGL(k_mask_count, dim3(nb(L.n)), dim3(256), 0, st, pairs, L.idx.get<uint32_t>(), L.gof.get<uint32_t>(), L.goff.get<uint64_t>(), L.n, dist, cnt);
  uint32_t *off = b.off.as<uint32_t>(L.n + 1);
  prims::exclusive_scan<uint32_t>(cnt, off, L.n, b.scan_tmp, st);
  uint32_t total = 0;
  HIP_CHECK(hipMemcpyAsync(&total, off + L.n, 4, hipMemcpyDeviceToHost, st));
  HIP_CHECK(hipStreamSynchronize(st));
  uint32_t *oidx = b.idx2.as<uint32_t>((uint64_t) total + 1), *ogof = b.gof2.as<uint32_t>((uint64_t) total + 1);
  uint64_t *ogoff = b.goff2.as<uint64_t>((uint64_t) L.ng + 1);
  hipLaunchKernelGGL(k_expand, dim3(nb(L.n)), dim3(256), 0, st, cnt, off, L.idx.get<uint32_t>(), L.gof.get<uint32_t>(), L.n, oidx, ogof);
  hipLaunchKernelGGL(k_new_goff, dim3(cdiv(L.ng + 1, 256)), dim3(256), 0, st, off, L.goff.get<uint64_t>(), L.ng, L.n, ogoff);
  std::swap(L.idx, b.idx2);
  std::swap(L.gof, b.gof2);
  std::swap(L.goff, b.goff2);
  L.n = total;
}

void remove_isolated_all(const bk_pair *pairs, const uint32_t *gof0, const uint64_t *gstart, uint32_t ng, uint64_t n, double w, PairList &L, ClusterBufs &b, hipStream_t st,
                         const uint32_t *drop_group)
{
  remove_isolated_begin(pairs, gof0, gstart, ng, n, w, L, b, st, drop_group, nullptr, nullptr);
  remove_isolated_end(pairs, L, b, st);
}

void remove_isolated_end(const bk_pair *pairs, PairList &L, ClusterBufs &b, hipStream_t st)
{
  if (L.n == 0 || L.ng == 0) return;
  sort_list(pairs, L, 0, nullptr, 0, b, st);
}

namespace
{
__global__ __launch_bounds__(256) void k_subset_list(const uint64_t *__restrict__ gstart, const uint64_t *__restrict__ goff, uint32_t ng, uint64_t n_list,
                                                     uint32_t *__restrict__ idx, uint32_t *__restrict__ gof)
{
  const uint64_t p = (uint64_t) blockIdx.x * blockDim.x + threadIdx.x;
  if (p >= n_list) return;
  uint32_t lo = 0, hi = ng;
  while (hi - lo > 1)
  {
    const uint32_t m = (lo + hi) >> 1;
    if (goff[m] <= p) lo = m; else hi = m;
  }
  idx[p] = (uint32_t) (gstart[lo] + (p - goff[lo]));
  gof[p] = lo;
}
}
namespace
{
__global__ __launch_bounds__(256) void k_subset_of_list(const uint32_t *__restrict__ src_idx, const uint64_t *__restrict__ src_goff, const uint64_t *__restrict__ goff, uint32_t ng,
                                                        uint64_t n_list, uint32_t *__restrict__ idx, uint32_t *__restrict__ gof)
{
  const uint64_t p = (uint64_t) blockIdx.x * blockDim.x + threadIdx.x;
  if (p >= n_list) return;
  uint32_t lo = 0, hi = ng;
  while (hi - lo > 1)
  {
    const uint32_t m = (lo + hi) >> 1;
    if (goff[m] <= p) lo = m; else hi = m;
  }
  idx[p] = src_idx[src_goff[lo] + (p - goff[lo])];
  gof[p] = lo;
}
}
void list_subset_ranges(const PairList &src, const uint64_t *src_goff_host, const uint8_t *keep_host, PairList &dst, hipStream_t st)
{
  const uint32_t ng = src.ng;
  std::vector<uint64_t> goff((size_t) ng + 1, 0);
  for (uint32_t g = 0; g < ng; ++g) goff[g + 1] = goff[g] + (keep_host[g] ? src_goff_host[g + 1] - src_goff_host[g] : 0);
  dst.n = goff[ng];
  dst.ng = ng;
  uint32_t *idx = dst.idx.as<uint32_t>(dst.n + 1), *gof = dst.gof.as<uint32_t>(dst.n + 1);
  uint64_t *dgoff = dst.goff.as<uint64_t>((uint64_t) ng + 1);
  HIP_CHECK(hipMemcpyAsync(dgoff, goff.data(), ((size_t) ng + 1) * 8, hipMemcpyHostToDevice, st));
  HIP_CHECK(hipStreamSynchronize(st));
  if (dst.n) hipLaunchKernelGGL(k_subset_of_list, dim3(nb(dst.n)), dim3(256), 0, st, src.idx.get<uint32_t>(), src.goff.get<uint64_t>(), dgoff, ng, dst.n, idx, gof);
}

void list_of_groups(const uint64_t *gstart_dev, const uint64_t *gstart_host, const uint8_t *keep_host, uint32_t ng, PairList &L, hipStream_t st)
{
  std::vector<uint64_t> goff((size_t) ng + 1, 0);
  for (uint32_t g = 0; g < ng; ++g) goff[g + 1] = goff[g] + (keep_host[g] ? gstart_host[g + 1] - gstart_host[g] : 0);
  L.n = goff[ng];
  L.ng = ng;
  uint32_t *idx = L.idx.as<uint32_t>(L.n + 1), *gof = L.gof.as<uint32_t>(L.n + 1);
  uint64_t *dgoff = L.goff.as<uint64_t>((uint64_t) ng + 1);
  HIP_CHECK(hipMemcpyAsync(dgoff, goff.data(), ((size_t) ng + 1) * 8, hipMemcpyHostToDevice, st));
  HIP_CHECK(hipStreamSynchronize(st));
  if (L.n) hipLaunchKernelGGL(k_subset_list, dim3(nb(L.n)), dim3(256), 0, st, gstart_dev, dgoff, ng, L.n, idx, gof);
}

void remove_isolated_begin(const bk_pair *pairs, const uint32_t *gof0, const uint64_t *gstart, uint32_t ng, uint64_t n, double w, PairList &L, ClusterBufs &b, hipStream_t st,
                           const uint32_t *drop_group, const uint64_t *gstart_host, const uint8_t *keep_host)
{
  if (gstart_host && keep_host)
  {
    if (n == 0 || ng == 0)
    {
      L.n = 0;
      L.ng = ng;
      (void) L.idx.as<uint32_t>(1);
      (void) L.gof.as<uint32_t>(1);
      (void) L.goff.as<uint64_t>((uint64_t) ng + 1);
      return;
    }
    list_of_groups(gstart, gstart_host, keep_host, ng, L, st);
  }
  else
  {
    L.n = n;
    L.ng = ng;
    uint32_t *idx = L.idx.as<uint32_t>(n + 1);
    uint32_t *gof = L.gof.as<uint32_t>(n + 1);
    uint64_t *goff = L.goff.as<uint64_t>((uint64_t) ng + 1);
    if (n == 0 || ng == 0) return;
    hipLaunchKernelGGL(k_iota, dim3(nb(n)), dim3(256), 0, st, idx, n);
    HIP_CHECK(hipMemcpyAsync(gof, gof0, n * 4, hipMemcpyDeviceToDevice, st));
    HIP_CHECK(hipMemcpyAsync(goff, gstart, ((uint64_t) ng + 1) * 8, hipMemcpyDeviceToDevice, st));
    if (drop_group) filter_groups(L, drop_group, b, st);
  }
  if (L.n == 0) return;
  const long dist = (long) w;
  sort_list(pairs, L, 0, nullptr, 0, b, st);
  mask_list(pairs, L, dist, b, st);
  sort_list(pairs, L, 1, nullptr, 0, b, st);
  mask_list(pairs, L, dist, b, st);
}

static void fast_pass(const bk_pair *pairs, PairList &L, int use_y, double w, DevBuf &k_prev, DevBuf &k_new, ClusterBufs &b, hipStream_t st)
{
  if (L.n == 0) return;
  const uint64_t n = L.n;
  uint32_t *key = b.key.as<uint32_t>(n);
  hipLaunchKernelGGL(k_gather_key, dim3(nb(n)), dim3(256), 0, st, pairs, L.idx.get<uint32_t>(), n, use_y, key);
  uint32_t *jump = b.jump.as<uint32_t>(n * 2ull);
  hipLaunchKernelGGL(k_fast_next, dim3(nb(n)), dim3(256), 0, st, key, L.gof.get<uint32_t>(), L.goff.get<uint64_t>(), n, w, jump);
  uint32_t *mark = b.mark.as<uint32_t>(n + 1);
  HIP_CHECK(hipMemsetAsync(mark, 0, (n + 1) * 4, st));
  hipLaunchKernelGGL(k_mark_starts, dim3(cdiv(L.ng, 256)), dim3(256), 0, st, L.goff.get<uint64_t>(), L.ng, mark);
  {
    uint32_t *exitp = jump + n;
    const unsigned tiles = (unsigned) cdiv(n, FW_TILE);
    hipLaunchKernelGGL(k_fw_exit, dim3(tiles), dim3(FW_TILE), 0, st, jump, n, exitp);
    hipLaunchKernelGGL(k_fw_chain, dim3(cdiv(L.ng, 64)), dim3(64), 0, st, L.goff.get<uint64_t>(), L.ng, exitp, mark);
    hipLaunchKernelGGL(k_fw_mark, dim3(tiles), dim3(FW_TILE), 0, st, jump, n, mark);
  }
  uint32_t *ascan = b.off.as<uint32_t>(n + 1);
  prims::exclusive_scan<uint32_t>(mark, ascan, n, b.scan_tmp, st);
  uint32_t *apos = b.apos.as<uint32_t>(n + 1);
  hipLaunchKernelGGL(k_anchor_pos, dim3(nb(n)), dim3(256), 0, st, mark, ascan, n, apos);
  uint32_t *keep = b.cnt.as<uint32_t>(n + 1), *kid = b.kid.as<uint32_t>(n + 1);
  hipLaunchKernelGGL(k_fast_keep, dim3(nb(n)), dim3(256), 0, st, mark, ascan, apos, jump, n, keep, kid);
  uint32_t *off = b.off2.as<uint32_t>(n + 1);
  prims::exclusive_scan<uint32_t>(keep, off, n, b.scan_tmp, st);
  uint32_t total = 0;
  HIP_CHECK(hipMemcpyAsync(&total, off + n, 4, hipMemcpyDeviceToHost, st));
  HIP_CHECK(hipStreamSynchronize(st));
  uint32_t *oidx = b.idx2.as<uint32_t>((uint64_t) total + 1), *ogof = b.gof2.as<uint32_t>((uint64_t) total + 1);
  uint32_t *okn = k_new.as<uint32_t>((uint64_t) total + 1);
  uint32_t *okp = k_prev.p ? b.kprev2.as<uint32_t>((uint64_t) total + 1) : nullptr;
  uint64_t *ogoff = b.goff2.as<uint64_t>((uint64_t) L.ng + 1);
  hipLaunchKernelGGL(k_compact3, dim3(nb(n)), dim3(256), 0, st, keep, off, n, L.idx.get<uint32_t>(), L.gof.get<uint32_t>(), kid, k_prev.get<uint32_t>(), oidx, ogof, okn, okp);
  hipLaunchKernelGGL(k_new_goff, dim3(cdiv(L.ng + 1, 256)), dim3(256), 0, st, off, L.goff.get<uint64_t>(), L.ng, n, ogoff);
  std::swap(L.idx, b.idx2);
  std::swap(L.gof, b.gof2);
  std::swap(L.goff, b.goff2);
  if (k_prev.p) std::swap(k_prev, b.kprev2);
  L.n = total;
}

static void filter_groups(PairList &L, const uint32_t *drop, ClusterBufs &b, hipStream_t st)
{
  if (L.n == 0) return;
  uint32_t *keep = b.cnt.as<uint32_t>(L.n + 1), *off = b.off.as<uint32_t>(L.n + 1);
  hipLaunchKernelGGL(k_drop_small, dim3(nb(L.n)), dim3(256), 0, st, L.gof.get<uint32_t>(), drop, L.n, keep);
  prims::exclusive_scan<uint32_t>(keep, off, L.n, b.scan_tmp, st);
  uint32_t total = 0;
  HIP_CHECK(hipMemcpyAsync(&total, off + L.n, 4, hipMemcpyDeviceToHost, st));
  HIP_CHECK(hipStreamSynchronize(st));
  if (total != L.n)
  {
    uint32_t *oidx = b.idx2.as<uint32_t>((uint64_t) total + 1), *ogof = b.gof2.as<uint32_t>((uint64_t) total + 1);
    uint64_t *ogoff = b.goff2.as<uint64_t>((uint64_t) L.ng + 1);
    hipLaunchKernelGGL(k_compact3, dim3(nb(L.n)), dim3(256), 0, st, keep, off, L.n, L.idx.get<uint32_t>(), L.gof.get<uint32_t>(), (const uint32_t *) nullptr,
                       (const uint32_t *) nullptr, oidx, ogof, (uint32_t *) nullptr, (uint32_t *) nullptr);
    hipLaunchKernelGGL(k_new_goff, dim3(cdiv(L.ng + 1, 256)), dim3(256), 0, st, off, L.goff.get<uint64_t>(), L.ng, L.n, ogoff);
    std::swap(L.idx, b.idx2);
    std::swap(L.gof, b.gof2);
    std::swap(L.goff, b.goff2);
    L.n = total;
  }
}

void drop_small_groups(PairList &L, ClusterBufs &b, hipStream_t st)
{
  if (L.n == 0) return;
  uint32_t *small = b.small.as<uint32_t>((uint64_t) L.ng + 1);
  hipLaunchKernelGGL(k_group_small, dim3(cdiv(L.ng, 256)), dim3(256), 0, st, L.goff.get<uint64_t>(), L.ng, small);
  filter_groups(L, small, b, st);
}

void fast_cluster_all(const bk_pair *pairs, PairList &L, double w, DevBuf &cluster_out, ClusterBufs &b, hipStream_t st)
{
  drop_small_groups(L, b, st);
  DevBuf none;
  const uint64_t n_first = L.n;
  fast_pass(pairs, L, 0, w, none, b.k1, b, st);
  {
    uint32_t *extra[1] = {b.k1.get<uint32_t>()};
    sort_list(pairs, L, 1, extra, L.n ? 1 : 0, b, st);
  }
  fast_pass(pairs, L, 1, w, b.k1, b.k2, b, st);
  {
    uint32_t *extra[2] = {b.k1.get<uint32_t>(), b.k2.get<uint32_t>()};
    sort_list(pairs, L, 0, extra, L.n ? 2 : 0, b, st);
  }
  const uint64_t n = L.n;
  uint32_t *cl = cluster_out.as<uint32_t>(n + 1);
  if (n == 0) return;
  uint64_t *pk = b.pk.as<uint64_t>(n);
  uint32_t *pv = b.perm.as<uint32_t>(n);
  int kbits = 1;
  while (kbits < 32 && (n_first >> kbits) != 0) ++kbits;
  hipLaunchKernelGGL(k_pack_k, dim3(nb(n)), dim3(256), 0, st, b.k1.get<uint32_t>(), b.k2.get<uint32_t>(), n, kbits, pk, pv);
  uint64_t *ks;
  uint32_t *vs;
  prims::radix_sort_pairs(pk, pv, n, 0, std::min(64, 2 * kbits), b.radix, st, &ks, &vs);
  uint32_t *flag = b.cnt.as<uint32_t>(n + 1), *fscan = b.off.as<uint32_t>(n + 1);
  hipLaunchKernelGGL(k_run_flag, dim3(nb(n)), dim3(256), 0, st, ks, n, flag);
  prims::exclusive_scan<uint32_t>(flag, fscan, n, b.scan_tmp, st);
  uint32_t *uid = b.kid.as<uint32_t>(n + 1), *ucount = b.mark.as<uint32_t>(n + 2), *uminpos = b.apos.as<uint32_t>(n + 1);
  hipLaunchKernelGGL(k_uid_stats, dim3(nb(n)), dim3(256), 0, st, flag, fscan, vs, n, uid, ucount, uminpos);
  uint32_t *keep = b.off2.as<uint32_t>(n + 1), *first = b.key.as<uint32_t>(n + 1);
  hipLaunchKernelGGL(k_first_flag, dim3(nb(n)), dim3(256), 0, st, uid, ucount, uminpos, n, keep, first);
  uint32_t *fs2 = b.tmp.as<uint32_t>(n + 1);
  prims::exclusive_scan<uint32_t>(first, fs2, n, b.scan_tmp, st);
  uint32_t *knum = b.knum.as<uint32_t>(n + 1);
  hipLaunchKernelGGL(k_knum, dim3(nb(n)), dim3(256), 0, st, first, fs2, uid, L.gof.get<uint32_t>(), L.goff.get<uint64_t>(), n, knum);
  uint32_t *clfull = b.clfull.as<uint32_t>(n + 1);
  hipLaunchKernelGGL(k_cluster_of, dim3(nb(n)), dim3(256), 0, st, uid, knum, keep, n, clfull);
  uint32_t *off = b.off.as<uint32_t>(n + 1);
  prims::exclusive_scan<uint32_t>(keep, off, n, b.scan_tmp, st);
  uint32_t total = 0;
  HIP_CHECK(hipMemcpyAsync(&total, off + n, 4, hipMemcpyDeviceToHost, st));
  HIP_CHECK(hipStreamSynchronize(st));
  uint32_t *oidx = b.idx2.as<uint32_t>((uint64_t) total + 1), *ogof = b.gof2.as<uint32_t>((uint64_t) total + 1);
  uint64_t *ogoff = b.goff2.as<uint64_t>((uint64_t) L.ng + 1);
  cl = cluster_out.as<uint32_t>((uint64_t) total + 1);
  hipLaunchKernelGGL(k_compact3, dim3(nb(n)), dim3(256), 0, st, keep, off, n, L.idx.get<uint32_t>(), L.gof.get<uint32_t>(), clfull, (const uint32_t *) nullptr, oidx, ogof, cl,
                     (uint32_t *) nullptr);
  hipLaunchKernelGGL(k_new_goff, dim3(cdiv(L.ng + 1, 256)), dim3(256), 0, st, off, L.goff.get<uint64_t>(), L.ng, n, ogoff);
  std::swap(L.idx, b.idx2);
  std::swap(L.gof, b.gof2);
  std::swap(L.goff, b.goff2);
  L.n = total;
}

void debug_mask_list(const bk_pair *pairs, PairList &L, long dist, ClusterBufs &b, hipStream_t st) { mask_list(pairs, L, dist, b, st); }

namespace
{
__global__ __launch_bounds__(256) void k_merge_goff(const uint64_t *__restrict__ b, uint32_t ng, uint64_t *__restrict__ out)
{
  uint32_t g = blockIdx.x * blockDim.x + threadIdx.x;
  if (g <= ng) out[g] += b[g];
}
__global__ __launch_bounds__(256) void k_merge_copy(const uint32_t *__restrict__ idx, const uint32_t *__restrict__ gof, const uint32_t *__restrict__ cl, const uint64_t *__restrict__ goff,
                                                    uint64_t n, const uint64_t *__restrict__ mgoff, uint32_t *__restrict__ oidx, uint32_t *__restrict__ ogof, uint32_t *__restrict__ ocl)
{
  uint64_t p = (uint64_t) blockIdx.x * blockDim.x + threadIdx.x;
  if (p >= n) return;
  const uint32_t g = gof[p];
  const uint64_t d = mgoff[g] + (p - goff[g]);
  oidx[d] = idx[p];
  ogof[d] = g;
  if (cl) ocl[d] = cl[p];
}
}

void merge_lists_many(const PairList *const *lists, const uint32_t *const *cls, int K, PairList &out, DevBuf *cl_out, hipStream_t st)
{
  const uint32_t ng = lists[0]->ng;
  out.ng = ng;
  out.n = 0;
  for (int l = 0; l < K; ++l) out.n += lists[l]->n;
  uint32_t *oidx = out.idx.as<uint32_t>(out.n + 1), *ogof = out.gof.as<uint32_t>(out.n + 1);
  uint64_t *ogoff = out.goff.as<uint64_t>((uint64_t) ng + 1);
  uint32_t *ocl = cl_out ? cl_out->as<uint32_t>(out.n + 1) : nullptr;
  HIP_CHECK(hipMemsetAsync(ogoff, 0, ((size_t) ng + 1) * 8, st));
  for (int l = 0; l < K; ++l) hipLaunchKernelGGL(k_merge_goff, dim3(cdiv(ng + 1, 256)), dim3(256), 0, st, lists[l]->goff.get<uint64_t>(), ng, ogoff);
  for (int l = 0; l < K; ++l)
  {
    const PairList &A = *lists[l];
    if (A.n) hipLaunchKernelGGL(k_merge_copy, dim3(nb(A.n)), dim3(256), 0, st, A.idx.get<uint32_t>(), A.gof.get<uint32_t>(), cls ? cls[l] : nullptr, A.goff.get<uint64_t>(), A.n, ogoff, oidx, ogof, ocl);
  }
}
```

breakid_amd/csrc/lanes.h:

```cpp
#pragma once
#include <functional>
#include <memory>

#include "join.h"
#include "cluster.h"
#include "ahc.h"

void stage_set_hw_queues(int n);

struct StageInput
{
  int device;
  hipStream_t st;
  const JoinResult &jr;
  const std::vector<uint64_t> &gstart_host;
  const std::vector<uint8_t> &own_groups;
  std::function<void(const char *name, const std::function<void()> &body)> timed;
};

struct ClusterStage
{
  SortService svc;
  std::vector<hipEvent_t> svc_probe;
  int svc_late = 0;
  bool svc_refused = false;
  struct Lane
  {
    ClusterBufs cb;
    PairList list, iso;
    DevBuf d_cluster;
    hipStream_t st = nullptr;
    ~Lane()
    {
      if (st) (void) hipStreamDestroy(st);
    }
  };
  std::vector<std::unique_ptr<Lane>> lanes;
  ClusterBufs &cb() { return lanes[0]->cb; }
  AhcBufs ab;
  PairList list;
  DevBuf d_cluster, iso_idx, iso_goff;
  uint64_t iso_n = 0;
  PairList lane_mid, lane_iso_m;
  DevBuf d_drop;

  ClusterStage() { lanes.emplace_back(new Lane()); }
  void run(const StageInput &in, double w, int fast);
  void sort_forms(uint64_t out[3]) const;
  void debug_sort(int device, hipStream_t st, uint32_t *key, uint32_t *idx, const uint32_t *gof, const uint64_t *goff, uint32_t ng, uint64_t n, uint64_t max_group);
};
```

breakid_amd/csrc/lanes.hip:

```cpp
#include <algorithm>
#include <atomic>
#include <chrono>
#include <cmath>
#include <cstdio>
#include <numeric>
#include <thread>
#include <dirent.h>

#include "lanes.h"

static int g_hw_queues_at_init = 0;
void stage_set_hw_queues(int n) { g_hw_queues_at_init = n; }

static bool sort_service_on()
{
  static const bool on = !(getenv("BREAKID_SORT_SERVICE") && atoi(getenv("BREAKID_SORT_SERVICE")) == 0);
  return on;
}
constexpr int LANE_STREAMS_MAX = 4;
constexpr int SVC_STAGE_QUEUES = LANE_STREAMS_MAX + 3;
static bool lane_service(int fast) { return sort_service_on() && fast && g_hw_queues_at_init >= SVC_STAGE_QUEUES; }
static int stage_queues() { return std::max(1, g_hw_queues_at_init - 1); }
static int lanes_wanted(bool svc)
{
  const char *env = getenv("BREAKID_GROUP_LANES");
  static const int want_svc = env ? atoi(env) : 12;
  if (svc) return want_svc < 1 ? 1 : (want_svc > 26 ? 26 : want_svc);
  static const int want = env ? atoi(env) : std::min(4, stage_queues());
  return want < 1 ? 1 : (want > 26 ? 26 : want);
}
static bool lanes_apply(const StageInput &in, int fast)
{
  static const uint64_t min_pairs = getenv("BREAKID_LANES_MIN_PAIRS") ? strtoull(getenv("BREAKID_LANES_MIN_PAIRS"), nullptr, 10) : (1ull << 20);
  uint32_t large = 0;
  const uint64_t big = std::max<uint64_t>(2, min_pairs >> 6);
  for (uint32_t g = 0; g < in.jr.n_groups && g + 1 < in.gstart_host.size(); ++g) large += in.gstart_host[g + 1] - in.gstart_host[g] >= big ? 1u : 0u;
  const bool yes = lanes_wanted(lane_service(fast)) >= 2 && fast && in.jr.n_groups >= 4 && in.jr.n_pairs >= min_pairs && large >= 2;
  if (yes)
  {
    static bool told = false;
    const int K = lanes_wanted(lane_service(fast));
    if (!told && !lane_service(fast) && K > stage_queues() && bk_debug("lanes"))
    {
      told = true;
      fprintf(stderr, "[breakid] GPU_MAX_HW_QUEUES=%d: the lanes of chromosome-pair groups (bk_mask_and_cluster) and their heap kernels will share hardware queues "
                        "(BREAKID_GROUP_LANES=1: one pass)\n", g_hw_queues_at_init);
    }
  }
  return yes;
}

__global__ void k_svc_probe() {}
static int kfd_compute_queues(int device)
{
  char bus[64] = {0};
  if (hipDeviceGetPCIBusId(bus, (int) sizeof bus, device) != hipSuccess) return -1;
  unsigned dom = 0, b = 0, d = 0, f = 0;
  if (sscanf(bus, "%x:%x:%x.%x", &dom, &b, &d, &f) != 4) return -1;
  const unsigned long want_loc = (b << 8) | (d << 3) | f;
  auto read_file = [](const std::string &path, std::string &out) {
    FILE *fp = fopen(path.c_str(), "r");
    if (!fp) return false;
    char buf[4096];
    const size_t n = fread(buf, 1, sizeof buf - 1, fp);
    fclose(fp);
    buf[n] = 0;
    out = buf;
    return true;
  };
  auto list_dir = [](const std::string &path, std::vector<std::string> &names) {
    DIR *dp = opendir(path.c_str());
    if (!dp) return false;
    while (dirent *e = readdir(dp))
      if (e->d_name[0] != '.') names.push_back(e->d_name);
    closedir(dp);
    return true;
  };
  unsigned long gpu_id = 0;
  {
    std::vector<std::string> nodes;
    if (!list_dir("/sys/class/kfd/kfd/topology/nodes", nodes)) return -1;
    for (const std::string &n : nodes)
    {
      std::string props, id;
      const std::string base = "/sys/class/kfd/kfd/topology/nodes/" + n;
      if (!read_file(base + "/properties", props) || !read_file(base + "/gpu_id", id)) continue;
      unsigned long loc = ~0ul, domain = ~0ul;
      size_t p = props.find("location_id ");
      if (p != std::string::npos) loc = strtoul(props.c_str() + p + 12, nullptr, 10);
      p = props.find("domain ");
      if (p != std::string::npos) domain = strtoul(props.c_str() + p + 7, nullptr, 10);
      if (loc == want_loc && (domain == ~0ul || domain == dom) && strtoul(id.c_str(), nullptr, 10) != 0) gpu_id = strtoul(id.c_str(), nullptr, 10);
    }
  }
  if (!gpu_id) return -1;
  std::vector<std::string> procs;
  if (!list_dir("/sys/class/kfd/kfd/proc", procs)) return -1;
  int total = 0;
  for (const std::string &pid : procs)
  {
    std::vector<std::string> qs;
    const std::string qdir = "/sys/class/kfd/kfd/proc/" + pid + "/queues";
    if (!list_dir(qdir, qs)) continue;
    for (const std::string &q : qs)
    {
      std::string g, t;
      if (!read_file(qdir + "/" + q + "/gpuid", g) || !read_file(qdir + "/" + q + "/type", t)) continue;
      if (strtoul(g.c_str(), nullptr, 10) == gpu_id && strtoul(t.c_str(), nullptr, 10) == 0) ++total;
    }
  }
  return total;
}
constexpr int SVC_MAX_DEVICE_QUEUES = 24;
static std::mutex g_svc_device_m[64];
static void tell_no_service()
{
  static std::atomic<bool> told{false};
  if (!getenv("BREAKID_QUIET") && !told.exchange(true))
    fprintf(stderr, "[breakid] the resident sort service shares a hardware queue with a stream of its own stage (GPU_MAX_HW_QUEUES too low for the streams of this process), or other processes hold hardware queues on this device: sorting by launches instead\n");
}
struct SvcStage
{
  ClusterStage &cs;
  hipStream_t st;
  bool on;
  std::unique_lock<std::mutex> device_turn;
  SvcStage(ClusterStage &s, int device, hipStream_t st, bool want, uint64_t n_bound, uint64_t max_group, const std::vector<hipStream_t> &streams)
      : cs(s), st(st), on(want && sort_service_on() && !s.svc_refused)
  {
    if (on && device >= 0 && device < 64)
    {
      device_turn = std::unique_lock<std::mutex>(g_svc_device_m[device], std::try_to_lock);
      on = device_turn.owns_lock();
    }
    if (!on) return;
    const auto ts0 = std::chrono::steady_clock::now();
    cs.svc.start(n_bound, max_group + 2, st);
    const auto ts1 = std::chrono::steady_clock::now();
    int census;
    {
      static std::mutex cm;
      static std::chrono::steady_clock::time_point when[64];
      static int last[64];
      static bool have[64] = {};
      std::lock_guard<std::mutex> l(cm);
      const int d = device & 63;
      if (!have[d] || std::chrono::duration<double>(ts1 - when[d]).count() > 0.25)
      {
        last[d] = kfd_compute_queues(device);
        when[d] = std::chrono::steady_clock::now();
        have[d] = true;
      }
      census = last[d];
    }
    if (bk_debug("lanes"))
      fprintf(stderr, "[lanes] sort service started in %.3f ms; compute queues on the device (all processes): %d (counted in %.3f ms)\n", std::chrono::duration<double, std::milli>(ts1 - ts0).count(), census,
              std::chrono::duration<double, std::milli>(std::chrono::steady_clock::now() - ts1).count());
    const bool crowded = census > SVC_MAX_DEVICE_QUEUES;
    const bool behind = !crowded && !reachable(streams);
    const bool late = !crowded && !behind && !cs.svc.narrow_running(0.03);
    if (crowded || behind || late)
    {
      cs.svc.stop();
      on = false;
      if (crowded || behind || ++cs.svc_late >= 2) cs.svc_refused = true;
      device_turn.unlock();
      tell_no_service();
      return;
    }
    cs.svc_late = 0;
    set(&cs.svc);
  }
  bool reachable(const std::vector<hipStream_t> &streams)
  {
    while (cs.svc_probe.size() < streams.size())
    {
      hipEvent_t e;
      HIP_CHECK(hipEventCreateWithFlags(&e, hipEventDisableTiming));
      cs.svc_probe.push_back(e);
    }
    for (size_t k = 0; k < streams.size(); ++k)
    {
      hipLaunchKernelGGL(k_svc_probe, dim3(1), dim3(64), 0, streams[k]);
      HIP_CHECK(hipEventRecord(cs.svc_probe[k], streams[k]));
    }
    const auto t0 = std::chrono::steady_clock::now();
    auto since = [&] { return std::chrono::duration<double>(std::chrono::steady_clock::now() - t0).count(); };
    bool ok = true;
    for (size_t k = 0; k < streams.size() && ok; ++k)
      for (;;)
      {
        const hipError_t e = hipEventQuery(cs.svc_probe[k]);
        if (e == hipSuccess) break;
        if (e != hipErrorNotReady) throw bk_error(BK_ERR_HIP, std::string("sort service probe: ") + hipGetErrorString(e));
        if (since() > 0.05)
        {
          ok = false;
          break;
        }
      }
    const double took = since();
    if (bk_debug("lanes")) fprintf(stderr, "[lanes] sort service probe: %zu streams in %.3f ms%s\n", streams.size(), took * 1e3, ok ? "" : " (gave up)");
    return ok && took < 0.003;
  }
  void set(SortService *s)
  {
    for (auto &l : cs.lanes)
    {
      l->cb.se.svc = s;
      l->cb.se.svc_slot = 0xFFFFFFFFu;
    }
  }
  void finish()
  {
    if (!on) return;
    on = false;
    set(nullptr);
    hipError_t e = hipStreamSynchronize(st);
    for (auto &l : cs.lanes)
      if (l->st && e == hipSuccess) e = hipStreamSynchronize(l->st);
    cs.svc.stop();
    device_turn.unlock();
    if (e != hipSuccess) throw bk_error(BK_ERR_HIP, std::string("sort service: ") + hipGetErrorString(e));
  }
  ~SvcStage()
  {
    try
    {
      finish();
    }
    catch (const bk_error &)
    {
    }
  }
};

static void snapshot_list(const PairList &L, DevBuf &idx, DevBuf *gof, DevBuf &goff, hipStream_t st)
{
  uint32_t *ii = idx.as<uint32_t>(L.n + 1), *ig = gof ? gof->as<uint32_t>(L.n + 1) : nullptr;
  uint64_t *io = goff.as<uint64_t>((uint64_t) L.ng + 1);
  if (L.n) HIP_CHECK(hipMemcpyAsync(ii, L.idx.get<uint32_t>(), L.n * 4, hipMemcpyDeviceToDevice, st));
  if (L.n && ig) HIP_CHECK(hipMemcpyAsync(ig, L.gof.get<uint32_t>(), L.n * 4, hipMemcpyDeviceToDevice, st));
  if (L.ng) HIP_CHECK(hipMemcpyAsync(io, L.goff.get<uint64_t>(), ((uint64_t) L.ng + 1) * 8, hipMemcpyDeviceToDevice, st));
}
static void cluster_list(const bk_pair *pairs, PairList &L, double w, int fast, DevBuf &cl, ClusterBufs &cb, AhcBufs &ab, hipStream_t st)
{
  if (fast)
    fast_cluster_all(pairs, L, w, cl, cb, st);
  else
    ahc_cluster_all(pairs, L, w, cl, ab, cb, st);
}

using LanePlan = std::vector<int>;
static LanePlan plan_owned(const StageInput &in)
{
  const uint32_t ng = in.jr.n_groups;
  const bool owned_only = !in.own_groups.empty();
  if (owned_only && in.own_groups.size() != ng) throw bk_error(BK_ERR_ARG, "bk_shard_own_groups: group count changed");
  LanePlan p(ng, 0);
  for (uint32_t g = 0; owned_only && g < ng; ++g)
    if (!in.own_groups[g]) p[g] = -1;
  return p;
}
static LanePlan plan_blind(const StageInput &in, int K)
{
  const uint32_t ng = in.jr.n_groups;
  std::vector<uint32_t> order(ng);
  std::iota(order.begin(), order.end(), 0u);
  auto size_of = [&](uint32_t g) { return in.gstart_host[g + 1] - in.gstart_host[g]; };
  std::stable_sort(order.begin(), order.end(), [&](uint32_t a, uint32_t b) { return size_of(a) > size_of(b); });
  constexpr double wexp = 2.0;
  LanePlan p = plan_owned(in);
  std::vector<double> load(K, 0.0);
  for (uint32_t i = 0; i < ng; ++i)
  {
    const uint32_t g = order[i];
    if (p[g] < 0) continue;
    int l = 0;
    for (int k = 1; k < K; ++k)
      if (load[k] < load[l]) l = k;
    load[l] += std::pow((double) size_of(g), wexp);
    p[g] = l;
  }
  return p;
}
static LanePlan plan_observed(const std::vector<uint64_t> &sizes, const std::vector<uint32_t> &hx, const std::vector<uint32_t> &hy, int K)
{
  const uint32_t ng = (uint32_t) sizes.size();
  constexpr double per_pair = 0.001;
  auto heap_cost = [](uint32_t m) { return (double) m + (m > 40947u ? 1.0 * (double) (m - 40947u) : 0.0); };
  std::vector<uint32_t> order(ng);
  std::iota(order.begin(), order.end(), 0u);
  auto chain = [&](uint32_t g) { return heap_cost(hx[g]) + heap_cost(hy[g]); };
  std::stable_sort(order.begin(), order.end(), [&](uint32_t a, uint32_t b) {
    const double ca = chain(a), cb = chain(b);
    return ca != cb ? ca > cb : sizes[a] > sizes[b];
  });
  LanePlan p(ng, 0);
  std::vector<double> mx(K, 0.0), my(K, 0.0), pairs(K, 0.0);
  auto cost = [&](int l) { return mx[l] + my[l] + per_pair * pairs[l]; };
  for (uint32_t g : order)
  {
    int best = 0;
    double best_cost = 0;
    for (int l = 0; l < K; ++l)
    {
      const double c = std::max(mx[l], heap_cost(hx[g])) + std::max(my[l], heap_cost(hy[g])) + per_pair * (pairs[l] + (double) sizes[g]);
      if (l == 0 || c < best_cost || (c == best_cost && cost(l) < cost(best)))
      {
        best = l;
        best_cost = c;
      }
    }
    mx[best] = std::max(mx[best], heap_cost(hx[g]));
    my[best] = std::max(my[best], heap_cost(hy[g]));
    pairs[best] += (double) sizes[g];
    p[g] = best;
  }
  if (bk_debug("lanes"))
    for (int l = 0; l < K; ++l)
    {
      fprintf(stderr, "[lanes] lane %d: max heap x %.0f y %.0f, %.0f pairs, cost %.0f; heavy groups:", l, mx[l], my[l], pairs[l], cost(l));
      for (uint32_t g = 0; g < ng; ++g)
        if (p[g] == l && (hx[g] || hy[g])) fprintf(stderr, " %u(%u,%u)", g, hx[g], hy[g]);
      fprintf(stderr, "\n");
    }
  return p;
}
static uint32_t *upload_drop(const LanePlan &p, int K, DevBuf &buf, hipStream_t st)
{
  const size_t row = p.size() + 1;
  std::vector<uint32_t> drop((size_t) K * row, 0u);
  for (int l = 0; l < K; ++l)
    for (size_t g = 0; g + 1 < row; ++g) drop[(size_t) l * row + g] = p[g] == l ? 0u : 1u;
  uint32_t *d = buf.as<uint32_t>(drop.size() + 1);
  HIP_CHECK(hipMemcpyAsync(d, drop.data(), drop.size() * 4, hipMemcpyHostToDevice, st));
  HIP_CHECK(hipStreamSynchronize(st));
  return d;
}

static void group_lanes(ClusterStage &cs, const StageInput &in, double w, int fast)
{
  const uint32_t ng = in.jr.n_groups;
  static const bool dbg = bk_debug("lanes");
  auto make_lanes = [&](int K, int S) {
    while ((int) cs.lanes.size() < K)
    {
      cs.lanes.emplace_back(new ClusterStage::Lane());
      cs.lanes.back()->cb.max_group_bound = cs.cb().max_group_bound;
    }
    for (int k = 1; k < S; ++k)
      if (!cs.lanes[k]->st) HIP_CHECK(hipStreamCreateWithFlags(&cs.lanes[k]->st, hipStreamNonBlocking));
  };
  bool use_svc = sort_service_on() && fast;
  if (use_svc && !lane_service(fast))
  {
    use_svc = false;
    tell_no_service();
    if (bk_debug("lanes")) fprintf(stderr, "[lanes] %d hardware queues, the sort service needs %d: not started\n", g_hw_queues_at_init, SVC_STAGE_QUEUES);
  }
  int K = lanes_wanted(use_svc);
  int S = use_svc ? std::max(1, std::min(LANE_STREAMS_MAX, K)) : K;
  make_lanes(K, S);
  std::vector<hipStream_t> stage_streams{in.st};
  for (int k = 1; k < S; ++k) stage_streams.push_back(cs.lanes[k]->st);
  SvcStage svc_stage(cs, in.device, in.st, use_svc, in.jr.n_pairs + 2ull * ng + 4096, cs.cb().max_group_bound, stage_streams);
  if (use_svc && !svc_stage.on)
  {
    use_svc = false;
    K = lanes_wanted(false);
    S = K;
    make_lanes(K, S);
  }
  if (!use_svc && bk_debug("lanes"))
  {
    fprintf(stderr, "[lanes] launch path: %d lanes, 1 stream each, %d hardware queues\n", K, g_hw_queues_at_init);
    fprintf(stderr, "[lanes] sorts as task dispatches on the lane streams\n");
  }
  auto lane = [&](int l) -> ClusterStage::Lane & { return *cs.lanes[l]; };
  auto lane_st = [&](int l) { const int k = l % S; return k == 0 ? in.st : cs.lanes[k]->st; };
  uint32_t *drop_base = nullptr;
  auto lane_drop = [&](int l) { return drop_base + (size_t) l * ((size_t) ng + 1); };
  std::vector<std::vector<uint8_t>> keep(K, std::vector<uint8_t>(ng, 0));
  auto upload_plan = [&](const LanePlan &p) {
    for (int l = 0; l < K; ++l)
      for (uint32_t g = 0; g < ng; ++g) keep[l][g] = p[g] == l ? 1 : 0;
    drop_base = upload_drop(p, K, cs.d_drop, in.st);
  };
  auto in_lanes = [&](auto body) {
    std::vector<std::string> err(K);
    std::vector<int> code(K, BK_OK);
    const auto t_start = std::chrono::steady_clock::now();
    auto guarded_body = [&](int l) {
      try
      {
        body(l);
        HIP_CHECK(hipStreamSynchronize(lane_st(l)));
        if (dbg)
          fprintf(stderr, "[lanes] lane %d done after %.2f ms\n", l, std::chrono::duration<double, std::milli>(std::chrono::steady_clock::now() - t_start).count());
      }
      catch (const bk_error &e)
      {
        code[l] = e.code;
        err[l] = e.msg;
      }
    };
    std::vector<std::thread> th;
    for (int l = 1; l < K; ++l)
      th.emplace_back([&, l] {
        (void) hipSetDevice(in.device);
        guarded_body(l);
      });
    guarded_body(0);
    for (std::thread &t : th) t.join();
    for (int l = 0; l < K; ++l)
      if (code[l] != BK_OK) throw bk_error(code[l], err[l]);
  };
  auto merge_all = [&](PairList ClusterStage::Lane::*which, PairList &out, DevBuf *cl_out) {
    std::vector<const PairList *> ls(K);
    std::vector<const uint32_t *> cls(K);
    for (int l = 0; l < K; ++l)
    {
      ls[l] = &(lane(l).*which);
      cls[l] = lane(l).d_cluster.get<uint32_t>();
    }
    merge_lists_many(ls.data(), cl_out ? cls.data() : nullptr, K, out, cl_out, in.st);
  };
  const bk_pair *pairs = in.jr.pairs;
  auto mask_lane = [&](int l, bool observe) {
    ClusterBufs &cb = lane(l).cb;
    if (observe)
    {
      cb.heavy_x.assign(ng, 0u);
      cb.heavy_y.assign(ng, 0u);
      cb.observe = true;
      cb.se.heavy_all = false;
    }
    remove_isolated_begin(pairs, in.jr.gof, in.jr.gstart, ng, in.jr.n_pairs, w, lane(l).list, cb, lane_st(l), lane_drop(l), in.gstart_host.data(), keep[l].data());
    if (observe) cb.heavy_x.assign(ng, 0u);
    remove_isolated_end(pairs, lane(l).list, cb, lane_st(l));
    if (observe) cb.observe = false;
  };
  auto cluster_lane = [&](int l) {
    PairList &L = lane(l).list, &iso = lane(l).iso;
    iso.n = L.n;
    iso.ng = L.ng;
    snapshot_list(L, iso.idx, &iso.gof, iso.goff, lane_st(l));
    cluster_list(pairs, L, w, fast, lane(l).d_cluster, lane(l).cb, cs.ab, lane_st(l));
  };
  const auto tp0 = std::chrono::steady_clock::now();
  auto phase = [&](const char *what) {
    if (dbg) fprintf(stderr, "[lanes] %s at %.2f ms\n", what, std::chrono::duration<double, std::milli>(std::chrono::steady_clock::now() - tp0).count());
  };
  upload_plan(plan_blind(in, K));
  phase("plan uploaded");
  if (use_svc)
    in_lanes([&](int l) {
      mask_lane(l, false);
      cluster_lane(l);
    });
  else
  {
    in_lanes([&](int l) { mask_lane(l, true); });
    PairList &mid = cs.lane_mid;
    merge_all(&ClusterStage::Lane::list, mid, nullptr);
    std::vector<uint64_t> goff_h((size_t) ng + 1);
    HIP_CHECK(hipMemcpyAsync(goff_h.data(), mid.goff.get<uint64_t>(), ((size_t) ng + 1) * 8, hipMemcpyDeviceToHost, in.st));
    HIP_CHECK(hipStreamSynchronize(in.st));
    std::vector<uint64_t> sizes(ng);
    std::vector<uint32_t> hx(ng, 0u), hy(ng, 0u);
    for (uint32_t g = 0; g < ng; ++g) sizes[g] = goff_h[g + 1] - goff_h[g];
    for (int l = 0; l < K; ++l)
      for (uint32_t g = 0; g < ng; ++g)
      {
        hx[g] = std::max(hx[g], lane(l).cb.heavy_x[g]);
        hy[g] = std::max(hy[g], lane(l).cb.heavy_y[g]);
      }
    upload_plan(plan_observed(sizes, hx, hy, K));
    in_lanes([&](int l) {
      list_subset_ranges(mid, goff_h.data(), keep[l].data(), lane(l).list, lane_st(l));
      cluster_lane(l);
    });
  }
  phase("lanes done");
  svc_stage.finish();
  phase("service stopped");
  if (use_svc && bk_debug("lanes")) fprintf(stderr, "[svc] tasks: %u wide, %u narrow\n", cs.svc.stats[0], cs.svc.stats[1]);
  PairList &iso_m = cs.lane_iso_m;
  merge_all(&ClusterStage::Lane::iso, iso_m, nullptr);
  merge_all(&ClusterStage::Lane::list, cs.list, &cs.d_cluster);
  HIP_CHECK(hipStreamSynchronize(in.st));
  phase("lists merged");
  cs.iso_n = iso_m.n;
  std::swap(cs.iso_idx, iso_m.idx);
  std::swap(cs.iso_goff, iso_m.goff);
}

void ClusterStage::run(const StageInput &in, double w, int fast)
{
  uint64_t mg = 0;
  for (uint32_t g = 0; g < in.jr.n_groups && g + 1 < in.gstart_host.size(); ++g) mg = std::max<uint64_t>(mg, in.gstart_host[g + 1] - in.gstart_host[g]);
  for (auto &l : lanes) l->cb.max_group_bound = mg;
  if (lanes_apply(in, fast))
  {
    in.timed("mask_and_cluster_lanes", [&] { group_lanes(*this, in, w, fast); });
    return;
  }
  SvcStage svc_stage(*this, in.device, in.st, true, in.jr.n_pairs + 2ull * in.jr.n_groups + 4096, cb().max_group_bound, {in.st});
  in.timed("remove_isolated", [&] {
    const uint32_t *drop = in.own_groups.empty() ? nullptr : upload_drop(plan_owned(in), 1, d_drop, in.st);
    remove_isolated_all(in.jr.pairs, in.jr.gof, in.jr.gstart, in.jr.n_groups, in.jr.n_pairs, w, list, cb(), in.st, drop);
  });
  iso_n = list.n;
  snapshot_list(list, iso_idx, nullptr, iso_goff, in.st);
  if (!fast) svc_stage.finish();
  in.timed(fast ? "fast_cluster" : "ahc_cluster", [&] { cluster_list(in.jr.pairs, list, w, fast, d_cluster, cb(), ab, in.st); });
  svc_stage.finish();
}

void ClusterStage::sort_forms(uint64_t out[3]) const
{
  out[0] = out[1] = out[2] = 0;
  for (const auto &l : lanes)
    for (int k = 0; k < 2; ++k) out[k] += l->cb.se.sorts[k];
}

void ClusterStage::debug_sort(int device, hipStream_t st, uint32_t *key, uint32_t *idx, const uint32_t *gof, const uint64_t *goff, uint32_t ng, uint64_t n, uint64_t max_group)
{
  SvcStage svc_stage(*this, device, st, true, n + 2ull * ng + 4096, max_group, {st});
  std_sort_groups(key, idx, gof, goff, ng, n, cb().se, st);
  svc_stage.finish();
}
```

include/breakid_hip.h:

```cpp
#ifndef BREAKID_HIP_H
#define BREAKID_HIP_H

#include <stdint.h>
#include <stddef.h>

#ifdef __cplusplus
extern "C" {
#endif

#define BK_OK 0
#define BK_ERR_ARG (-1)
#define BK_ERR_HIP (-2)
#define BK_ERR_NO_DEVICE (-3)
#define BK_ERR_UNSORTED (-4)
#define BK_ERR_CIGAR (-5)
#define BK_ERR_IO (-6)
#define BK_ERR_LIMIT (-7)
#define BK_ERR_COLLISION (-8)

#define BK_MEM_HOST 0
#define BK_MEM_DEVICE 1

typedef struct bk_ctx bk_ctx;

typedef struct bk_soa {
  uint64_t n;
  const int32_t *tid, *pos, *mtid, *mpos, *isize;
  const uint16_t *flag;
  const uint8_t *mapq;
  const uint64_t *qhash;
  const uint32_t *cigar_off;
  const uint32_t *cigar;
  const uint32_t *aux_off;
  const uint8_t *aux;
  uint64_t n_cigar_words;
  uint64_t n_aux_bytes;
  const uint32_t *qcheck;
  const struct bk_side *side;
} bk_soa;

typedef struct bk_side {
  uint64_t qhash;
  int32_t mtid, mpos;
  uint32_t qcheck;
  uint32_t reserved[3];
} bk_side;

typedef struct bk_pair {
  uint32_t x, y;
  uint32_t p1_pos, p2_pos;
  int32_t p1_tid, p2_tid;
  uint16_t p1_flag, p2_flag;
  uint8_t p1_mapq, p2_mapq, p1_rev, p2_rev;
  uint64_t rec;
  uint32_t id;
  int32_t cluster;
  uint32_t group;
  uint32_t reserved;
} bk_pair;

typedef struct bk_split {
  uint64_t rec;
  int32_t tid, pos, endpos;
  uint32_t reserved;
  uint64_t qhash;
  int32_t prim_chr, sec_chr;
  uint32_t prim_start, prim_end, prim_bp, sec_start, sec_end, sec_bp;
  uint64_t prim_cigar, sec_cigar;
  uint32_t flags;
  uint32_t qcheck;
} bk_split;

#define BK_TYPE_DIFF_CHR 1u
#define BK_TYPE_SAME_ORIENT 2u
#define BK_TYPE_ABS_REVERSE 4u
#define BK_TYPE_DEFAULT_ORIENT 8u

typedef struct bk_cluster {
  uint32_t group;
  int32_t id;
  int32_t p1_tid, p2_tid;
  uint32_t p1_mean, p2_mean, p1_min, p1_max, p2_min, p2_max;
  uint32_t p1_exact;
  int32_t p2_exact;
  uint32_t n_drp, n_sr;
  uint32_t depth1, depth2;
  uint32_t type_mask;
  uint32_t flags;
} bk_cluster;

#define BK_STAGE_SCAN 0
#define BK_STAGE_ISO 1
#define BK_STAGE_CLUSTERED 2
#define BK_STAGE_SPLITS 3
#define BK_STAGE_CLUSTERS 4
#define BK_STAGE_GROUP_KEYS 5

int bk_init(int device, const uint32_t *target_len, const char *const *target_name, int n_targets, bk_ctx **out);
void bk_prepare_process(void);
void bk_free(bk_ctx *ctx);
const char *bk_last_error(const bk_ctx *ctx);
int bk_set_stream(bk_ctx *ctx, void *hip_stream);
int bk_sync(bk_ctx *ctx);
int bk_get_stream(bk_ctx *ctx, void **hip_stream);

int bk_upload_records(bk_ctx *ctx, const bk_soa *cols, int mem_space);

typedef struct bk_regions {
  const int32_t *tid, *beg, *end;
  uint64_t n;
} bk_regions;
int bk_exclude_regions(bk_ctx *ctx, const bk_regions *r, uint64_t *n_removed);

int bk_isize_stats(bk_ctx *ctx, double *mean, double *sd);
int bk_discordant_pairs(bk_ctx *ctx, int mapq_min, double w, uint64_t *n_pairs, uint32_t *n_groups);
int bk_mask_and_cluster(bk_ctx *ctx, double w, int fast, uint64_t *n_clustered);
int bk_split_evidence(bk_ctx *ctx, uint64_t *n_tuples);
int bk_cluster_summary(bk_ctx *ctx, double w, uint64_t *n_clusters);
int bk_split_breakpoints(bk_ctx *ctx, double w, uint64_t *n_valid);

int bk_run(bk_ctx *ctx, int mapq_min, int fast, double *w_out, uint64_t *n_valid);

struct bk_normal_support { uint32_t n_drp, n_sr, depth1, depth2; };
int bk_normal_support(bk_ctx *tumor, bk_ctx *normal, double w, const struct bk_normal_support **out, uint64_t *count);

struct bk_ref_support { uint32_t ref_pairs1, ref_pairs2, ref_reads1, ref_reads2; };
int bk_ref_support(bk_ctx *calls, bk_ctx *records, int mapq_min, int anchor, double w, const struct bk_ref_support **out, uint64_t *count);
int bk_genotype_call(uint32_t alt, uint32_t ref, uint8_t *gt, uint8_t *gq, float *vaf);

struct bk_junction {
  uint32_t pairs[4];
  uint32_t splits[4];
  uint64_t mapq_sum1, mapq_sum2;
};
int bk_junctions(bk_ctx *ctx, const struct bk_junction **out, uint64_t *count);
int bk_junction_sides(const struct bk_junction *j, uint8_t *right1, uint8_t *right2, uint8_t *source);
int bk_vcf_breakend_alt(char ref_base, int own_right, const char *mate_chr, uint32_t mate_pos, int mate_right, char *buf, size_t cap);

struct bk_clip_support { uint32_t at[2][2], peak_pos[2][2], peak_n[2][2], events[2][2]; };
int bk_clip_support(bk_ctx *calls, bk_ctx *records, int mapq_min, int min_clip, double w, const struct bk_clip_support **out, uint64_t *count);
int bk_base_depth(bk_ctx *records, const int32_t *tid, const uint32_t *pos, uint64_t n, const uint32_t **out);
int bk_clip_rescue(const bk_cluster *c, const struct bk_junction *j, const struct bk_clip_support *s, uint32_t min_support, uint32_t *pos1, uint32_t *pos2, uint32_t *n1,
                   uint32_t *n2);

struct bk_clip_site { int32_t tid; uint32_t pos; uint32_t tol; uint32_t dir; };
struct bk_clip_read {
  uint64_t rec;
  uint64_t qhash;
  uint32_t qcheck;
  uint32_t site;
  int32_t tid; uint32_t p;
  uint32_t clip_len;
  uint16_t flag;
  uint8_t mapq;
  uint8_t dir;
};
int bk_clip_reads(bk_ctx *records, const struct bk_clip_site *sites, uint64_t n_sites, int mapq_min, int min_clip, const uint32_t **counts,
                  const struct bk_clip_read **rows, const uint64_t **site_off);

#define BK_EV_PAIR 1
#define BK_EV_SPLIT 2
struct bk_evidence {
  uint64_t rec;
  uint64_t qhash;
  uint32_t qcheck;
  uint32_t call;
  int32_t tid1; uint32_t pos1;
  int32_t tid2; uint32_t pos2;
  uint16_t flag1, flag2;
  uint8_t mapq1, mapq2;
  uint8_t kind;
  uint8_t sides;
};
int bk_evidence(bk_ctx *ctx, const struct bk_evidence **out, uint64_t *count, const uint64_t **call_off);

struct bk_unique_support { uint32_t uniq_pairs, top_pairs, uniq_splits, top_splits; };
int bk_unique_support(bk_ctx *ctx, const struct bk_unique_support **out, uint64_t *count, const uint64_t **first, uint64_t *n_rows);

typedef struct bk_reads {
  uint64_t n;
  const int32_t *tid, *pos;
  const uint16_t *flag;
  const uint8_t *mapq;
  const uint32_t *key;
  const uint32_t *cigar_off;
  const uint32_t *cigar;
  const uint32_t *l_seq;
  const uint64_t *seq_off;
  const uint8_t *seq;
  void *owner;
} bk_reads;
struct bk_consensus { uint32_t n_reads, len, match, total; };
int bk_clip_consensus(bk_ctx *ctx, const bk_reads *reads, const struct bk_clip_site *sites, uint64_t n_sites, int mapq_min, int min_clip, uint32_t max_len,
                      uint32_t min_depth, const struct bk_consensus **out, const uint8_t **bases, const uint32_t **col_depth);

typedef struct bk_refseq {
  uint64_t n_segs;
  const int32_t *tid;
  const uint32_t *start;
  const uint32_t *len;
  const uint64_t *off;
  const uint8_t *bases;
} bk_refseq;
struct bk_junction_probe { int32_t tid_own; uint32_t pos_own, dir_own; int32_t tid_mate; uint32_t pos_mate, dir_mate; uint32_t qlen, reserved; };
struct bk_junction_fit { int32_t shift; uint32_t ins, aligned, mism, hom_fwd, hom_back; int32_t score; uint32_t placed; };
int bk_junction_fit(bk_ctx *ctx, const bk_refseq *ref, const struct bk_junction_probe *probes, uint64_t n, const uint8_t *query, uint32_t max_len, uint32_t max_shift,
                    uint32_t max_ins, uint32_t max_hom, const struct bk_junction_fit **out);

struct bk_locus_pair { int32_t tid_a; uint32_t pos_a; int32_t tid_b; uint32_t pos_b; };
struct bk_locus_sim  { uint32_t score, len, mism, run; int32_t diag; uint32_t start, orient, found; };
int bk_locus_similarity(bk_ctx *ctx, const bk_refseq *ref, const struct bk_locus_pair *pairs, uint64_t n, uint32_t flank, const struct bk_locus_sim **out);

struct bk_cov_window { int32_t tid; uint32_t beg, end; uint32_t reserved; };
struct bk_window_cov { uint64_t bases; uint32_t reads; uint32_t reserved; };
int bk_window_coverage(bk_ctx *records, const struct bk_cov_window *windows, uint64_t n, int mapq_min, const struct bk_window_cov **out);
int bk_call_windows(const bk_cluster *c, int right1, int right2, uint32_t flank, const uint32_t *target_len, struct bk_cov_window out[5]);

#define BK_FRAME_NONE 0
#define BK_FRAME_ANTISENSE 1
#define BK_FRAME_TRUNCATING 2
#define BK_FRAME_PROMOTER 3
#define BK_FRAME_OUTFRAME 4
#define BK_FRAME_INFRAME 5
#define BK_FRAME_HEAD 1
#define BK_FRAME_TAIL 2
#define BK_LOC_NONCODING 1
#define BK_LOC_5UTR 2
#define BK_LOC_CDS 3
#define BK_LOC_INTRON 4
#define BK_LOC_3UTR 5
typedef struct bk_txmodel {
  uint64_t n_tx, n_parts;
  const int32_t *tid;
  const uint32_t *tx_start, *tx_end;
  const uint8_t *strand;
  const uint32_t *ex_off;
  const uint32_t *ex_start, *ex_end;
} bk_txmodel;
struct bk_frame_site { int32_t tid1; uint32_t pos1; int32_t tid2; uint32_t pos2; uint8_t right1, right2; uint8_t reserved[6]; };
struct bk_frame_call { uint8_t cls, order, loc[2], role[2]; uint16_t exon[2]; uint16_t reserved; int32_t tx[2]; uint32_t cod[2], n_tx[2], n_inframe, n_compatible; uint32_t reserved2; };
int bk_fusion_frame(bk_ctx *ctx, const bk_txmodel *model, const struct bk_frame_site *sites, uint64_t n, const struct bk_frame_call **out);

#define BK_LINK_NONE 0
#define BK_LINK_DUPLICATE 1
#define BK_LINK_RECIPROCAL 2
#define BK_LINK_ADJACENT 3
#define BK_LINK_MAX_DIST 1000000u
struct bk_link_site { int32_t tid1; uint32_t pos1; int32_t tid2; uint32_t pos2; uint8_t right1, right2; uint8_t reserved[6]; };
struct bk_call_link { uint32_t n_dup, n_recip, n_adj; int32_t dup_of, mate; int32_t off[2]; uint32_t event, event_size; uint8_t mate_crossed; uint8_t reserved[3]; };
int bk_link_calls(bk_ctx *ctx, const struct bk_link_site *sites, uint64_t n, uint32_t max_dist, const struct bk_call_link **out);

struct bk_partner_site { int32_t tid; uint32_t beg, end; int32_t mtid; uint32_t mbeg, mend; uint32_t reserved[2]; };
struct bk_locus_partners { uint32_t ends, to_partner, loci, top_n; int32_t top_tid; uint32_t top_beg, top_end, reserved; };
int bk_locus_partners(bk_ctx *ctx, const struct bk_partner_site *sites, uint64_t n, uint32_t max_gap, const struct bk_locus_partners **out);
int bk_call_partner_sites(const bk_cluster *c, double w, struct bk_partner_site out[2]);

int bk_fetch(bk_ctx *ctx, int stage, const void **data, uint64_t *count, const uint64_t **group_off, uint32_t *n_groups);

typedef struct bk_group_stat {
  int32_t p1_tid, p2_tid;
  uint64_t n_scan, n_isolated_removed, n_clustered;
  uint32_t cluster_id_end;
  uint32_t ordinal;
} bk_group_stat;
int bk_group_stats(bk_ctx *ctx, const bk_group_stat **out, uint32_t *n_groups);

int bk_timing(bk_ctx *ctx, const char *const **names, const float **ms, const uint64_t **bytes, int *n);
int bk_timing_enable(bk_ctx *ctx, int on);
int bk_timing_touched(bk_ctx *ctx, const uint64_t **touched, int *n);

typedef struct bk_shard_stats {
  uint64_t isize_sum, isize_n;
  double sumsq;
  uint32_t vmax, max_span;
  uint64_t n_cand, n_split;
} bk_shard_stats;
#define BK_BUF_CANDIDATES 0
#define BK_BUF_TUPLES 1
#define BK_BUF_CLUSTERS 2
int bk_shard_begin(bk_ctx *ctx, uint64_t rec_base, int mapq_min);
int bk_shard_get_stats(bk_ctx *ctx, bk_shard_stats *out);
int bk_shard_set_stats(bk_ctx *ctx, const bk_shard_stats *total);
int bk_shard_sd_local(bk_ctx *ctx, uint64_t *l_total, void **ex_dev, uint64_t *n_ex);
int bk_shard_sd_finish(bk_ctx *ctx, const void *all_ex_dev, uint64_t n_all, uint64_t l_grand, double *mean, double *sd);
int bk_shard_buffer(bk_ctx *ctx, int which, void **dev, uint64_t *count, uint32_t *elem_bytes);
int bk_shard_set_buffer(bk_ctx *ctx, int which, const void *dev, uint64_t count);
int bk_shard_group_sizes(bk_ctx *ctx, const uint64_t **starts, uint32_t *n_groups);
int bk_shard_own_groups(bk_ctx *ctx, const uint8_t *own, uint32_t n_groups);
int bk_shard_route_candidates(bk_ctx *ctx, uint32_t world, void **dev, const uint64_t **counts);
int bk_shard_group_keys(bk_ctx *ctx, const uint32_t **keys, uint32_t *n_groups);
int bk_shard_route_pairs(bk_ctx *ctx, const uint32_t *dest_of_group, uint32_t n_groups, uint32_t world, void **dev, const uint64_t **counts);
int bk_shard_group_pairs(bk_ctx *ctx, const void *pairs_dev, uint64_t n, const uint32_t *all_keys, uint32_t n_all_keys);
int bk_shard_bp_cov(bk_ctx *ctx, double w, void **cov_dev, uint64_t *n);
int bk_shard_bp_vote(bk_ctx *ctx, double w, const void *cov_total_dev);
int bk_shard_bp_vote_slice(bk_ctx *ctx, double w, const void *cov_total_dev, uint64_t lo, uint64_t hi, void **clusters_dev, void **voted_dev);
int bk_shard_bp_set_voted(bk_ctx *ctx, const void *voted_all_dev);
int bk_shard_bp_depth(bk_ctx *ctx, void **depth_dev, uint64_t *n);
int bk_shard_bp_finish(bk_ctx *ctx, const void *depth_total_dev);

int bk_debug_std_sort(bk_ctx *ctx, const uint32_t *key, const uint64_t *group_off, uint32_t n_groups, uint32_t *perm_out);

int bk_debug_scan(bk_ctx *ctx, int elem_bytes, const void *in, uint64_t n, int in_place, void *out);
int bk_debug_radix_sort(bk_ctx *ctx, const uint64_t *keys, const uint32_t *vals, uint64_t n, int begin_bit, int end_bit, uint64_t *keys_out, uint32_t *vals_out);
int bk_debug_prims_info(uint64_t out[4]);

int bk_sort_forms(bk_ctx *ctx, uint64_t out[3]);

int bk_debug_ahc(bk_ctx *ctx, const uint32_t *x, const uint32_t *y, uint32_t n, double w, uint32_t *idx_out, int32_t *cluster_out, uint32_t *n_out);

int bk_debug_points(bk_ctx *ctx, int mode, const uint32_t *x, const uint32_t *y, uint32_t n, double w, uint32_t *idx_out, int32_t *cluster_out, uint32_t *n_out);
int bk_debug_cigar(bk_ctx *ctx, uint32_t n, const uint8_t *kind, const uint32_t *c1_off, const uint8_t *c1, const uint32_t *c2_off, const uint8_t *c2, const int32_t *e,
                   int32_t *out6);
int bk_debug_vote(bk_ctx *ctx, const bk_split *side1, uint32_t n1, const bk_split *side2, uint32_t n2, int32_t p1_tid, int32_t p2_tid, int32_t *out3);
int bk_debug_region(bk_ctx *ctx, int32_t tid, uint32_t start, uint32_t end, uint64_t depth_pos, bk_split *out, uint32_t cap, uint32_t *n_out, uint32_t *cov_out,
                    uint32_t *depth_out);

typedef struct bk_bam bk_bam;
uint64_t bk_qname_hash(const char *name, size_t len);
uint32_t bk_qname_check(const char *name, size_t len);
int bk_bam_open(const char *path, bk_bam **out, char *err, size_t errlen);
int bk_bam_header(const bk_bam *b, int *n_targets, const char *const **names, const uint32_t **lens);
int bk_bam_decode(bk_bam *b, bk_soa *out, char *err, size_t errlen);
void bk_bam_close(bk_bam *b);
typedef struct bk_read_key { uint64_t qhash; uint32_t qcheck; uint32_t tag; } bk_read_key;
int bk_bam_extract(const char *in_bam, const char *out_bam, const bk_read_key *keys, uint64_t n_keys, const char *const *tags, uint64_t n_tags, char **names_out,
                   uint64_t *n_written, char *err, size_t errlen);
void bk_bam_names_free(char *names);
int bk_bam_reads(const char *in_bam, const bk_read_key *keys, uint64_t n_keys, bk_reads *out, char *err, size_t errlen);
void bk_reads_free(bk_reads *r);

typedef struct bk_bam_dev bk_bam_dev;
int bk_bam_decode_device(const char *path, int device, bk_bam_dev **out, bk_soa *cols, int *n_targets, const char *const **names, const uint32_t **lens,
                         char *err, size_t errlen);
int bk_bam_decode_device_part(const char *path, int device, int part, int parts, bk_bam_dev **out, bk_soa *cols, int *n_targets, const char *const **names,
                              const uint32_t **lens, char *err, size_t errlen);
void bk_bam_dev_free(bk_bam_dev *h);
void bk_feed_release_caches(void);
int bk_bam_decode_device_ctx(const char *path, int device, int mapq_min, bk_bam_dev **bam_out, bk_ctx **ctx_out, int *n_targets, const char *const **names,
                             const uint32_t **lens, char *err, size_t errlen);
int bk_records(bk_ctx *ctx, bk_soa *cols);
int bk_debug_bgzf_inflate(const void *file, uint64_t n, void *out, uint64_t out_cap, uint64_t *out_len, float *kernel_ms, char *err, size_t errlen);

#ifdef __cplusplus
}
#endif
#endif
```

Before: 11720.

## Replace radix-sort key matching with per-run wave matching and gather lanes directly

Adds a key-match path that splits each group into runs of equal first keys, already sorted, and matches second keys within a run using wavefront ballots, with an LDS bitonic sort for long runs. This replaces the full 64-bit radix sort plus several scans in fast clustering. The lane re-deal also now gathers groups straight from per-lane snapshots instead of first merging into a middle list and subsetting with a per-element binary search. Order and length errors are detected, presumably falling back to radix, and a debug entry point is added to compare the two modes.

```diff
diff --git a/breakid_amd/capi.py b/breakid_amd/capi.py
--- a/breakid_amd/capi.py
+++ b/breakid_amd/capi.py
@@ -30,7 +30,7 @@
 EXPORTS = ["bk_init", "bk_prepare_process", "bk_free", "bk_last_error", "bk_set_stream", "bk_sync", "bk_get_stream", "bk_upload_records", "bk_records", "bk_exclude_regions", "bk_isize_stats",
            "bk_discordant_pairs", "bk_mask_and_cluster", "bk_split_evidence", "bk_cluster_summary",
            "bk_split_breakpoints", "bk_normal_support", "bk_ref_support", "bk_genotype_call", "bk_clip_support", "bk_clip_reads", "bk_base_depth", "bk_clip_rescue", "bk_junctions", "bk_junction_sides", "bk_vcf_breakend_alt", "bk_evidence", "bk_unique_support", "bk_clip_consensus", "bk_junction_fit", "bk_locus_similarity", "bk_window_coverage", "bk_call_windows", "bk_fusion_frame", "bk_link_calls", "bk_locus_partners", "bk_call_partner_sites", "bk_run", "bk_fetch", "bk_timing", "bk_timing_enable", "bk_timing_touched", "bk_group_stats", "bk_qname_hash", "bk_qname_check",
-           "bk_bam_open", "bk_bam_header", "bk_bam_decode", "bk_bam_close", "bk_bam_extract", "bk_bam_names_free", "bk_bam_reads", "bk_reads_free", "bk_bam_decode_device", "bk_bam_decode_device_part", "bk_bam_decode_device_ctx", "bk_bam_dev_free", "bk_feed_release_caches", "bk_debug_bgzf_inflate", "bk_debug_std_sort", "bk_debug_scan", "bk_debug_radix_sort", "bk_debug_prims_info", "bk_sort_forms", "bk_debug_ahc", "bk_debug_points", "bk_debug_cigar", "bk_debug_vote", "bk_debug_region", "bk_shard_begin", "bk_shard_get_stats", "bk_shard_set_stats",
+           "bk_bam_open", "bk_bam_header", "bk_bam_decode", "bk_bam_close", "bk_bam_extract", "bk_bam_names_free", "bk_bam_reads", "bk_reads_free", "bk_bam_decode_device", "bk_bam_decode_device_part", "bk_bam_decode_device_ctx", "bk_bam_dev_free", "bk_feed_release_caches", "bk_debug_bgzf_inflate", "bk_debug_std_sort", "bk_debug_scan", "bk_debug_radix_sort", "bk_debug_prims_info", "bk_sort_forms", "bk_debug_ahc", "bk_debug_points", "bk_debug_key_match", "bk_debug_cigar", "bk_debug_vote", "bk_debug_region", "bk_shard_begin", "bk_shard_get_stats", "bk_shard_set_stats",
            "bk_shard_sd_local", "bk_shard_sd_finish", "bk_shard_buffer", "bk_shard_set_buffer", "bk_shard_group_sizes",
            "bk_shard_own_groups", "bk_shard_route_candidates", "bk_shard_group_keys", "bk_shard_route_pairs", "bk_shard_group_pairs", "bk_shard_bp_cov", "bk_shard_bp_vote", "bk_shard_bp_vote_slice", "bk_shard_bp_set_voted", "bk_shard_bp_depth", "bk_shard_bp_finish"]
 
@@ -96,6 +96,7 @@
         L.bk_sort_forms.argtypes = [vp, u64p]
         L.bk_debug_ahc.argtypes = [vp, vp, vp, C.c_uint32, C.c_double, vp, vp, C.POINTER(C.c_uint32)]
         L.bk_debug_points.argtypes = [vp, C.c_int, vp, vp, C.c_uint32, C.c_double, vp, vp, C.POINTER(C.c_uint32)]
+        L.bk_debug_key_match.argtypes = [vp, C.c_int, vp, vp, vp, C.c_uint32, vp, vp, C.POINTER(C.c_int)]
         L.bk_debug_cigar.argtypes = [vp, C.c_uint32, vp, vp, vp, vp, vp, vp, vp]
         L.bk_debug_vote.argtypes = [vp, vp, C.c_uint32, vp, C.c_uint32, C.c_int32, C.c_int32, vp]
         L.bk_debug_region.argtypes = [vp, C.c_int32, C.c_uint32, C.c_uint32, C.c_uint64, vp, C.c_uint32, C.POINTER(C.c_uint32), C.POINTER(C.c_uint32),
@@ -639,6 +640,18 @@
                                            cl.ctypes.data, C.byref(m)))
         return idx[:m.value].copy(), cl[:m.value].copy()
 
+    def debug_key_match(self, k1, k2, group_off, mode="runs"):
+        k1 = np.ascontiguousarray(k1, np.uint32)
+        k2 = np.ascontiguousarray(k2, np.uint32)
+        group_off = np.ascontiguousarray(group_off, np.uint64)
+        n = len(k1)
+        assert k1.shape == k2.shape and k1.ndim == 1 and len(group_off) >= 2 and int(group_off[-1]) == n
+        cl, keep = np.zeros(max(n, 1), np.uint32), np.zeros(max(n, 1), np.uint32)
+        took = C.c_int(-1)
+        self._check(self.L.bk_debug_key_match(self.h, {"runs": 0, "radix": 1, "env": -1}[mode], k1.ctypes.data if n else None, k2.ctypes.data if n else None,
+                                              group_off.ctypes.data, len(group_off) - 1, cl.ctypes.data, keep.ctypes.data, C.byref(took)))
+        return cl[:n].copy(), keep[:n].copy(), ("runs", "radix")[took.value]
+
     def debug_cigar(self, rows):
         kind = np.asarray([1 if r[0] == "b" else 0 for r in rows], np.uint8)
         c1 = bytearray()
diff --git a/breakid_amd/csrc/api.hip b/breakid_amd/csrc/api.hip
--- a/breakid_amd/csrc/api.hip
+++ b/breakid_amd/csrc/api.hip
@@ -2281,6 +2281,41 @@
       if (mode == 2 && cluster_out) HIP_CHECK(hipMemcpyAsync(cluster_out, dcl.get<uint32_t>(), L.n * 4, hipMemcpyDeviceToHost, ctx->st));
     }
     HIP_CHECK(hipStreamSynchronize(ctx->st));
+  });
+}
+
+int bk_debug_key_match(bk_ctx *ctx, int mode, const uint32_t *k1, const uint32_t *k2, const uint64_t *group_off, uint32_t n_groups, uint32_t *cluster_out, uint32_t *keep_out,
+                       int *mode_out)
+{
+  return guarded(ctx, [&] {
+    if (!group_off || !n_groups || mode < -1 || mode > KEYMATCH_RADIX) throw bk_error(BK_ERR_ARG, "bk_debug_key_match: bad argument");
+    const uint64_t n = group_off[n_groups];
+    if (group_off[0] != 0 || n > 0xFFFFFFF0ull) throw bk_error(BK_ERR_ARG, "bk_debug_key_match: group_off must start at 0 and end below 2^32");
+    for (uint32_t g = 0; g < n_groups; ++g)
+      if (group_off[g + 1] < group_off[g]) throw bk_error(BK_ERR_ARG, "bk_debug_key_match: group_off decreases");
+    if (n && (!k1 || !k2 || !cluster_out || !keep_out)) throw bk_error(BK_ERR_ARG, "bk_debug_key_match: null argument");
+    std::vector<uint32_t> gof(n);
+    uint64_t bound = 1;
+    for (uint32_t g = 0; g < n_groups; ++g)
+      for (uint64_t p = group_off[g]; p < group_off[g + 1]; ++p) gof[p] = g;
+    for (uint64_t p = 0; p < n; ++p) bound = std::max<uint64_t>(bound, (uint64_t) std::max(k1[p], k2[p]) + 1);
+    DevBuf d1, d2, dgof, dgoff, dcl, dkeep;
+    if (n)
+    {
+      HIP_CHECK(hipMemcpy(d1.as<uint32_t>(n), k1, n * 4, hipMemcpyHostToDevice));
+      HIP_CHECK(hipMemcpy(d2.as<uint32_t>(n), k2, n * 4, hipMemcpyHostToDevice));
+      HIP_CHECK(hipMemcpy(dgof.as<uint32_t>(n), gof.data(), n * 4, hipMemcpyHostToDevice));
+    }
+    HIP_CHECK(hipMemcpy(dgoff.as<uint64_t>((uint64_t) n_groups + 1), group_off, ((uint64_t) n_groups + 1) * 8, hipMemcpyHostToDevice));
+    const int took = debug_key_match(d1.get<uint32_t>(), d2.get<uint32_t>(), dgof.get<uint32_t>(), dgoff.get<uint64_t>(), n, bound, mode, dcl.as<uint32_t>(n + 1),
+                                     dkeep.as<uint32_t>(n + 1), ctx->stage.cb(), ctx->st);
+    if (n)
+    {
+      HIP_CHECK(hipMemcpyAsync(cluster_out, dcl.get<uint32_t>(), n * 4, hipMemcpyDeviceToHost, ctx->st));
+      HIP_CHECK(hipMemcpyAsync(keep_out, dkeep.get<uint32_t>(), n * 4, hipMemcpyDeviceToHost, ctx->st));
+    }
+    HIP_CHECK(hipStreamSynchronize(ctx->st));
+    if (mode_out) *mode_out = took;
   });
 }
 
diff --git a/breakid_amd/csrc/cluster.h b/breakid_amd/csrc/cluster.h
--- a/breakid_amd/csrc/cluster.h
+++ b/breakid_amd/csrc/cluster.h
@@ -18,7 +18,7 @@
   std::vector<uint32_t> heavy_x, heavy_y;
   bool observe = false;
   uint64_t max_group_bound = 0;
-  DevBuf key, perm, tmp, cnt, off, off2, idx2, gof2, goff2, jump, mark, apos, kid, kprev2, k1, k2, pk, knum, clfull, small, scan_tmp;
+  DevBuf key, perm, tmp, cnt, off, off2, idx2, gof2, goff2, jump, mark, apos, kid, kprev2, k1, k2, pk, knum, clfull, small, km, scan_tmp;
   SortEmuBufs se;
   prims::RadixBufs radix;
 };
@@ -28,8 +28,15 @@
 void remove_isolated_begin(const bk_pair *pairs, const uint32_t *gof0, const uint64_t *gstart, uint32_t ng, uint64_t n, double w, PairList &L, ClusterBufs &b, hipStream_t st,
                            const uint32_t *drop_group = nullptr, const uint64_t *gstart_host = nullptr, const uint8_t *keep_host = nullptr);
 void remove_isolated_end(const bk_pair *pairs, PairList &L, ClusterBufs &b, hipStream_t st);
-void list_subset_ranges(const PairList &src, const uint64_t *src_goff_host, const uint8_t *keep_host, PairList &dst, hipStream_t st);
+void gather_groups_many(const PairList *const *src, int K, const uint64_t *goff_host, uint32_t ng, PairList &dst, hipStream_t st);
 void drop_small_groups(PairList &L, ClusterBufs &b, hipStream_t st);
-void fast_cluster_all(const bk_pair *pairs, PairList &L, double w, DevBuf &cluster_out, ClusterBufs &b, hipStream_t st);
+void fast_cluster_all(const bk_pair *pairs, PairList &L, double w, DevBuf &cluster_out, ClusterBufs &b, hipStream_t st, bool small_dropped = false);
 void merge_lists_many(const PairList *const *lists, const uint32_t *const *cls, int K, PairList &out, DevBuf *cl_out, hipStream_t st);
+enum
+{
+  KEYMATCH_RUNS = 0,
+  KEYMATCH_RADIX = 1
+};
+int debug_key_match(const uint32_t *k1, const uint32_t *k2, const uint32_t *gof, const uint64_t *goff, uint64_t n, uint64_t k_bound, int mode, uint32_t *clfull, uint32_t *keep,
+                    ClusterBufs &b, hipStream_t st);
 void debug_mask_list(const bk_pair *pairs, PairList &L, long dist, ClusterBufs &b, hipStream_t st);
diff --git a/breakid_amd/csrc/cluster.hip b/breakid_amd/csrc/cluster.hip
--- a/breakid_amd/csrc/cluster.hip
+++ b/breakid_amd/csrc/cluster.hip
@@ -1,3 +1,4 @@
+#include <cstring>
 #include "bk_common.h"
 #include "prims.h"
 #include "sortemu.h"
@@ -241,6 +242,157 @@
 {
   uint64_t p = (uint64_t) blockIdx.x * blockDim.x + threadIdx.x;
   if (p < n) cl[p] = keep[p] ? knum[uid[p]] : 0u;
+}
+constexpr uint32_t KM_CHUNKS = 4, KM_WAVE_MAX = 64 * KM_CHUNKS, KM_LDS_MAX = 4096, KM_LONG_LIST = 1024;
+constexpr uint32_t KM_ERR_ORDER = 1u, KM_ERR_LONG = 2u;
+constexpr unsigned KM_MATCH_BLOCKS = 2048, KM_LONG_BLOCKS = 32;
+
+__global__ __launch_bounds__(256) void k_km_run_start(const uint32_t *__restrict__ k1, const uint32_t *__restrict__ gof, uint64_t n, uint32_t *__restrict__ flag,
+                                                      uint32_t *__restrict__ err, uint32_t *__restrict__ nlong, uint32_t *__restrict__ upos, uint32_t *__restrict__ keep,
+                                                      uint32_t *__restrict__ first)
+{
+  uint64_t p = (uint64_t) blockIdx.x * blockDim.x + threadIdx.x;
+  if (p >= n) return;
+  if (p == 0) *nlong = 0;
+  upos[p] = (uint32_t) p;
+  keep[p] = 0;
+  first[p] = 0;
+  uint32_t f = 1;
+  if (p > 0 && gof[p] == gof[p - 1])
+  {
+    const uint32_t a = k1[p - 1], c = k1[p];
+    f = a != c ? 1u : 0u;
+    if (c < a) atomicOr(err, KM_ERR_ORDER);
+  }
+  flag[p] = f;
+}
+__global__ __launch_bounds__(256) void k_km_run_pos(const uint32_t *__restrict__ flag, const uint32_t *__restrict__ rscan, uint64_t n, uint32_t *__restrict__ rstart)
+{
+  uint64_t p = (uint64_t) blockIdx.x * blockDim.x + threadIdx.x;
+  if (p >= n) return;
+  const uint32_t f = flag[p], r = rscan[p];
+  if (f) rstart[r] = (uint32_t) p;
+  if (p == n - 1) rstart[r + f] = (uint32_t) n;
+}
+__global__ __launch_bounds__(256) void k_km_match(const uint32_t *__restrict__ k2, const uint32_t *__restrict__ rstart, const uint32_t *__restrict__ n_runs,
+                                                  uint32_t *__restrict__ upos, uint32_t *__restrict__ keep, uint32_t *__restrict__ first, uint32_t *__restrict__ err,
+                                                  uint32_t *__restrict__ nlong, uint32_t *__restrict__ longs)
+{
+  const uint32_t lane = threadIdx.x & 63u;
+  const uint32_t R = *n_runs, W = gridDim.x * (blockDim.x >> 6);
+  for (uint32_t r = blockIdx.x * (blockDim.x >> 6) + (threadIdx.x >> 6); r < R; r += W)
+  {
+    const uint32_t s = rstart[r], e = rstart[r + 1], len = e - s;
+    if (len > KM_WAVE_MAX)
+    {
+      if (lane == 0)
+      {
+        if (len > KM_LDS_MAX)
+          atomicOr(err, KM_ERR_LONG);
+        else
+        {
+          const uint32_t i = atomicAdd(nlong, 1u);
+          if (i < KM_LONG_LIST) longs[i] = r; else atomicOr(err, KM_ERR_LONG);
+        }
+      }
+      continue;
+    }
+    uint32_t v[KM_CHUNKS];
+    bool live[KM_CHUNKS];
+#pragma unroll
+    for (uint32_t c = 0; c < KM_CHUNKS; ++c)
+    {
+      const uint32_t p = s + c * 64u + lane;
+      live[c] = p < e;
+      v[c] = live[c] ? k2[p] : 0u;
+    }
+#pragma unroll
+    for (uint32_t c = 0; c < KM_CHUNKS; ++c)
+    {
+      if (c * 64u >= len) break;
+      for (;;)
+      {
+        const unsigned long long m = __ballot(live[c]);
+        if (!m) break;
+        const uint32_t lead = (uint32_t) __ffsll((long long) m) - 1u;
+        const uint32_t lk = (uint32_t) __shfl((int) v[c], (int) lead);
+        bool hit[KM_CHUNKS];
+        uint32_t cnt = 0;
+#pragma unroll
+        for (uint32_t d = 0; d < KM_CHUNKS; ++d)
+        {
+          hit[d] = live[d] && v[d] == lk;
+          cnt += (uint32_t) __popcll(__ballot(hit[d]));
+        }
+        const uint32_t fp = s + c * 64u + lead, k = cnt >= 2 ? 1u : 0u;
+#pragma unroll
+        for (uint32_t d = 0; d < KM_CHUNKS; ++d)
+          if (hit[d])
+          {
+            const uint32_t p = s + d * 64u + lane;
+            upos[p] = fp;
+            keep[p] = k;
+            first[p] = (k && p == fp) ? 1u : 0u;
+            live[d] = false;
+          }
+      }
+    }
+  }
+}
+__global__ __launch_bounds__(256) void k_km_long(const uint32_t *__restrict__ k2, const uint32_t *__restrict__ rstart, const uint32_t *__restrict__ nlong,
+                                                 const uint32_t *__restrict__ longs, uint32_t *__restrict__ upos, uint32_t *__restrict__ keep, uint32_t *__restrict__ first)
+{
+  __shared__ uint64_t sk[KM_LDS_MAX];
+  const uint32_t nl = min(*nlong, KM_LONG_LIST);
+  for (uint32_t i = blockIdx.x; i < nl; i += gridDim.x)
+  {
+    const uint32_t r = longs[i], s = rstart[r], len = rstart[r + 1] - s;
+    uint32_t P = 2 * KM_WAVE_MAX;
+    while (P < len) P <<= 1;
+    for (uint32_t t = threadIdx.x; t < P; t += 256) sk[t] = t < len ? ((uint64_t) k2[s + t] << 32) | t : ~0ull;
+    for (uint32_t k = 2; k <= P; k <<= 1)
+      for (uint32_t j = k >> 1; j > 0; j >>= 1)
+      {
+        __syncthreads();
+        for (uint32_t t = threadIdx.x; t < P; t += 256)
+        {
+          const uint32_t u = t ^ j;
+          if (u > t)
+          {
+            const uint64_t a = sk[t], c = sk[u];
+            if ((a > c) == ((t & k) == 0))
+            {
+              sk[t] = c;
+              sk[u] = a;
+            }
+          }
+        }
+      }
+    __syncthreads();
+    for (uint32_t t = threadIdx.x; t < len; t += 256)
+    {
+      const uint64_t key = sk[t], lo_key = key & 0xFFFFFFFF00000000ull, hi_key = key | 0xFFFFFFFFull;
+      uint32_t lo = 0, hi = t;
+      while (lo < hi)
+      {
+        const uint32_t m = (lo + hi) >> 1;
+        if (sk[m] < lo_key) lo = m + 1; else hi = m;
+      }
+      const uint32_t lb = lo;
+      lo = t + 1;
+      hi = len;
+      while (lo < hi)
+      {
+        const uint32_t m = (lo + hi) >> 1;
+        if (sk[m] <= hi_key) lo = m + 1; else hi = m;
+      }
+      const uint32_t kk = lo - lb >= 2 ? 1u : 0u, p = s + (uint32_t) key;
+      upos[p] = s + (uint32_t) sk[lb];
+      keep[p] = kk;
+      first[p] = (kk && t == lb) ? 1u : 0u;
+    }
+    __syncthreads();
+  }
 }
 __global__ void k_group_small(const uint64_t *__restrict__ goff, uint32_t ng, uint32_t *__restrict__ small)
 {
@@ -336,33 +488,32 @@
 }
 namespace
 {
-__global__ __launch_bounds__(256) void k_subset_of_list(const uint32_t *__restrict__ src_idx, const uint64_t *__restrict__ src_goff, const uint64_t *__restrict__ goff, uint32_t ng,
-                                                        uint64_t n_list, uint32_t *__restrict__ idx, uint32_t *__restrict__ gof)
+__global__ __launch_bounds__(256) void k_gather_groups(const uint32_t *__restrict__ src_idx, const uint32_t *__restrict__ src_gof, const uint64_t *__restrict__ src_goff, uint64_t n_src,
+                                                       const uint64_t *__restrict__ goff, uint32_t *__restrict__ idx, uint32_t *__restrict__ gof)
 {
   const uint64_t p = (uint64_t) blockIdx.x * blockDim.x + threadIdx.x;
-  if (p >= n_list) return;
-  uint32_t lo = 0, hi = ng;
-  while (hi - lo > 1)
-  {
-    const uint32_t m = (lo + hi) >> 1;
-    if (goff[m] <= p) lo = m; else hi = m;
-  }
-  idx[p] = src_idx[src_goff[lo] + (p - goff[lo])];
-  gof[p] = lo;
-}
-}
-void list_subset_ranges(const PairList &src, const uint64_t *src_goff_host, const uint8_t *keep_host, PairList &dst, hipStream_t st)
-{
-  const uint32_t ng = src.ng;
-  std::vector<uint64_t> goff((size_t) ng + 1, 0);
-  for (uint32_t g = 0; g < ng; ++g) goff[g + 1] = goff[g] + (keep_host[g] ? src_goff_host[g + 1] - src_goff_host[g] : 0);
-  dst.n = goff[ng];
+  if (p >= n_src) return;
+  const uint32_t g = src_gof[p];
+  const uint64_t d0 = goff[g];
+  if (goff[g + 1] == d0) return;
+  const uint64_t d = d0 + (p - src_goff[g]);
+  idx[d] = src_idx[p];
+  gof[d] = g;
+}
+}
+void gather_groups_many(const PairList *const *src, int K, const uint64_t *goff_host, uint32_t ng, PairList &dst, hipStream_t st)
+{
+  dst.n = goff_host[ng];
   dst.ng = ng;
   uint32_t *idx = dst.idx.as<uint32_t>(dst.n + 1), *gof = dst.gof.as<uint32_t>(dst.n + 1);
   uint64_t *dgoff = dst.goff.as<uint64_t>((uint64_t) ng + 1);
-  HIP_CHECK(hipMemcpyAsync(dgoff, goff.data(), ((size_t) ng + 1) * 8, hipMemcpyHostToDevice, st));
-  HIP_CHECK(hipStreamSynchronize(st));
-  if (dst.n) hipLaunchKernelGGL(k_subset_of_list, dim3(nb(dst.n)), dim3(256), 0, st, src.idx.get<uint32_t>(), src.goff.get<uint64_t>(), dgoff, ng, dst.n, idx, gof);
+  HIP_CHECK(hipMemcpyAsync(dgoff, goff_host, ((size_t) ng + 1) * 8, hipMemcpyHostToDevice, st));
+  if (dst.n == 0) return;
+  for (int l = 0; l < K; ++l)
+  {
+    const PairList &A = *src[l];
+    if (A.n) hipLaunchKernelGGL(k_gather_groups, dim3(nb(A.n)), dim3(256), 0, st, A.idx.get<uint32_t>(), A.gof.get<uint32_t>(), A.goff.get<uint64_t>(), A.n, dgoff, idx, gof);
+  }
 }
 
 void list_of_groups(const uint64_t *gstart_dev, const uint64_t *gstart_host, const uint8_t *keep_host, uint32_t ng, PairList &L, hipStream_t st)
@@ -488,9 +639,64 @@
   filter_groups(L, small, b, st);
 }
 
-void fast_cluster_all(const bk_pair *pairs, PairList &L, double w, DevBuf &cluster_out, ClusterBufs &b, hipStream_t st)
-{
-  drop_small_groups(L, b, st);
+static int keymatch_mode()
+{
+  const char *e = getenv("BREAKID_KEYMATCH");
+  return e && !strcmp(e, "radix") ? KEYMATCH_RADIX : KEYMATCH_RUNS;
+}
+
+static int key_match(const uint32_t *k1, const uint32_t *k2, const uint32_t *gof, const uint64_t *goff, uint64_t n, uint64_t n_first, int mode, ClusterBufs &b, hipStream_t st,
+                     uint32_t *total)
+{
+  uint32_t *uid = b.kid.as<uint32_t>(n + 1), *keep = b.off2.as<uint32_t>(n + 1), *first = b.key.as<uint32_t>(n + 1);
+  uint32_t *off = b.off.as<uint32_t>(n + 2), *err = off + n + 1;
+  if (mode == KEYMATCH_RUNS)
+  {
+    uint32_t *flag = b.cnt.as<uint32_t>(n + 1), *rscan = b.mark.as<uint32_t>(n + 2), *rstart = b.apos.as<uint32_t>(n + 2);
+    uint32_t *nlong = b.km.as<uint32_t>((uint64_t) KM_LONG_LIST + 1), *longs = nlong + 1;
+    HIP_CHECK(hipMemsetAsync(err, 0, 4, st));
+    hipLaunchKernelGGL(k_km_run_start, dim3(nb(n)), dim3(256), 0, st, k1, gof, n, flag, err, nlong, uid, keep, first);
+    prims::exclusive_scan<uint32_t>(flag, rscan, n, b.scan_tmp, st);
+    hipLaunchKernelGGL(k_km_run_pos, dim3(nb(n)), dim3(256), 0, st, flag, rscan, n, rstart);
+    hipLaunchKernelGGL(k_km_match, dim3(std::min(nb(n), KM_MATCH_BLOCKS)), dim3(256), 0, st, k2, rstart, rscan + n, uid, keep, first, err, nlong, longs);
+    hipLaunchKernelGGL(k_km_long, dim3(KM_LONG_BLOCKS), dim3(256), 0, st, k2, rstart, nlong, longs, uid, keep, first);
+  }
+  else
+  {
+    uint64_t *pk = b.pk.as<uint64_t>(n);
+    uint32_t *pv = b.perm.as<uint32_t>(n);
+    int kbits = 1;
+    while (kbits < 32 && (n_first >> kbits) != 0) ++kbits;
+    hipLaunchKernelGGL(k_pack_k, dim3(nb(n)), dim3(256), 0, st, k1, k2, n, kbits, pk, pv);
+    uint64_t *ks;
+    uint32_t *vs;
+    prims::radix_sort_pairs(pk, pv, n, 0, std::min(64, 2 * kbits), b.radix, st, &ks, &vs);
+    uint32_t *flag = b.cnt.as<uint32_t>(n + 1), *fscan = off;
+    hipLaunchKernelGGL(k_run_flag, dim3(nb(n)), dim3(256), 0, st, ks, n, flag);
+    prims::exclusive_scan<uint32_t>(flag, fscan, n, b.scan_tmp, st);
+    uint32_t *ucount = b.mark.as<uint32_t>(n + 2), *uminpos = b.apos.as<uint32_t>(n + 2);
+    hipLaunchKernelGGL(k_uid_stats, dim3(nb(n)), dim3(256), 0, st, flag, fscan, vs, n, uid, ucount, uminpos);
+    hipLaunchKernelGGL(k_first_flag, dim3(nb(n)), dim3(256), 0, st, uid, ucount, uminpos, n, keep, first);
+    HIP_CHECK(hipMemsetAsync(err, 0, 4, st));
+  }
+  uint32_t *fs2 = b.tmp.as<uint32_t>(n + 1);
+  prims::exclusive_scan<uint32_t>(first, fs2, n, b.scan_tmp, st);
+  uint32_t *knum = b.knum.as<uint32_t>(n + 1);
+  hipLaunchKernelGGL(k_knum, dim3(nb(n)), dim3(256), 0, st, first, fs2, uid, gof, goff, n, knum);
+  uint32_t *clfull = b.clfull.as<uint32_t>(n + 1);
+  hipLaunchKernelGGL(k_cluster_of, dim3(nb(n)), dim3(256), 0, st, uid, knum, keep, n, clfull);
+  prims::exclusive_scan<uint32_t>(keep, off, n, b.scan_tmp, st);
+  uint32_t back[2] = {0, 0};
+  HIP_CHECK(hipMemcpyAsync(back, off + n, 8, hipMemcpyDeviceToHost, st));
+  HIP_CHECK(hipStreamSynchronize(st));
+  if (back[1]) return key_match(k1, k2, gof, goff, n, n_first, KEYMATCH_RADIX, b, st, total);
+  *total = back[0];
+  return mode;
+}
+
+void fast_cluster_all(const bk_pair *pairs, PairList &L, double w, DevBuf &cluster_out, ClusterBufs &b, hipStream_t st, bool small_dropped)
+{
+  if (!small_dropped) drop_small_groups(L, b, st);
   DevBuf none;
   const uint64_t n_first = L.n;
   fast_pass(pairs, L, 0, w, none, b.k1, b, st);
@@ -506,32 +712,9 @@
   const uint64_t n = L.n;
   uint32_t *cl = cluster_out.as<uint32_t>(n + 1);
   if (n == 0) return;
-  uint64_t *pk = b.pk.as<uint64_t>(n);
-  uint32_t *pv = b.perm.as<uint32_t>(n);
-  int kbits = 1;
-  while (kbits < 32 && (n_first >> kbits) != 0) ++kbits;
-  hipLaunchKernelGGL(k_pack_k, dim3(nb(n)), dim3(256), 0, st, b.k1.get<uint32_t>(), b.k2.get<uint32_t>(), n, kbits, pk, pv);
-  uint64_t *ks;
-  uint32_t *vs;
-  prims::radix_sort_pairs(pk, pv, n, 0, std::min(64, 2 * kbits), b.radix, st, &ks, &vs);
-  uint32_t *flag = b.cnt.as<uint32_t>(n + 1), *fscan = b.off.as<uint32_t>(n + 1);
-  hipLaunchKernelGGL(k_run_flag, dim3(nb(n)), dim3(256), 0, st, ks, n, flag);
-  prims::exclusive_scan<uint32_t>(flag, fscan, n, b.scan_tmp, st);
-  uint32_t *uid = b.kid.as<uint32_t>(n + 1), *ucount = b.mark.as<uint32_t>(n + 2), *uminpos = b.apos.as<uint32_t>(n + 1);
-  hipLaunchKernelGGL(k_uid_stats, dim3(nb(n)), dim3(256), 0, st, flag, fscan, vs, n, uid, ucount, uminpos);
-  uint32_t *keep = b.off2.as<uint32_t>(n + 1), *first = b.key.as<uint32_t>(n + 1);
-  hipLaunchKernelGGL(k_first_flag, dim3(nb(n)), dim3(256), 0, st, uid, ucount, uminpos, n, keep, first);
-  uint32_t *fs2 = b.tmp.as<uint32_t>(n + 1);
-  prims::exclusive_scan<uint32_t>(first, fs2, n, b.scan_tmp, st);
-  uint32_t *knum = b.knum.as<uint32_t>(n + 1);
-  hipLaunchKernelGGL(k_knum, dim3(nb(n)), dim3(256), 0, st, first, fs2, uid, L.gof.get<uint32_t>(), L.goff.get<uint64_t>(), n, knum);
-  uint32_t *clfull = b.clfull.as<uint32_t>(n + 1);
-  hipLaunchKernelGGL(k_cluster_of, dim3(nb(n)), dim3(256), 0, st, uid, knum, keep, n, clfull);
-  uint32_t *off = b.off.as<uint32_t>(n + 1);
-  prims::exclusive_scan<uint32_t>(keep, off, n, b.scan_tmp, st);
   uint32_t total = 0;
-  HIP_CHECK(hipMemcpyAsync(&total, off + n, 4, hipMemcpyDeviceToHost, st));
-  HIP_CHECK(hipStreamSynchronize(st));
+  key_match(b.k1.get<uint32_t>(), b.k2.get<uint32_t>(), L.gof.get<uint32_t>(), L.goff.get<uint64_t>(), n, n_first, keymatch_mode(), b, st, &total);
+  const uint32_t *keep = b.off2.get<uint32_t>(), *off = b.off.get<uint32_t>(), *clfull = b.clfull.get<uint32_t>();
   uint32_t *oidx = b.idx2.as<uint32_t>((uint64_t) total + 1), *ogof = b.gof2.as<uint32_t>((uint64_t) total + 1);
   uint64_t *ogoff = b.goff2.as<uint64_t>((uint64_t) L.ng + 1);
   cl = cluster_out.as<uint32_t>((uint64_t) total + 1);
@@ -544,6 +727,17 @@
   L.n = total;
 }
 
+int debug_key_match(const uint32_t *k1, const uint32_t *k2, const uint32_t *gof, const uint64_t *goff, uint64_t n, uint64_t k_bound, int mode, uint32_t *clfull, uint32_t *keep,
+                    ClusterBufs &b, hipStream_t st)
+{
+  if (n == 0) return mode < 0 ? keymatch_mode() : mode;
+  uint32_t total = 0;
+  const int took = key_match(k1, k2, gof, goff, n, k_bound, mode < 0 ? keymatch_mode() : mode, b, st, &total);
+  HIP_CHECK(hipMemcpyAsync(clfull, b.clfull.get<uint32_t>(), n * 4, hipMemcpyDeviceToDevice, st));
+  HIP_CHECK(hipMemcpyAsync(keep, b.off2.get<uint32_t>(), n * 4, hipMemcpyDeviceToDevice, st));
+  return took;
+}
+
 void debug_mask_list(const bk_pair *pairs, PairList &L, long dist, ClusterBufs &b, hipStream_t st) { mask_list(pairs, L, dist, b, st); }
 
 namespace
diff --git a/breakid_amd/csrc/lanes.h b/breakid_amd/csrc/lanes.h
--- a/breakid_amd/csrc/lanes.h
+++ b/breakid_amd/csrc/lanes.h
@@ -41,7 +41,7 @@
   PairList list;
   DevBuf d_cluster, iso_idx, iso_goff;
   uint64_t iso_n = 0;
-  PairList lane_mid, lane_iso_m;
+  PairList lane_iso_m;
   DevBuf d_drop;
 
   ClusterStage() { lanes.emplace_back(new Lane()); }
diff --git a/breakid_amd/csrc/lanes.hip b/breakid_amd/csrc/lanes.hip
--- a/breakid_amd/csrc/lanes.hip
+++ b/breakid_amd/csrc/lanes.hip
@@ -243,10 +243,10 @@
   if (L.n && ig) HIP_CHECK(hipMemcpyAsync(ig, L.gof.get<uint32_t>(), L.n * 4, hipMemcpyDeviceToDevice, st));
   if (L.ng) HIP_CHECK(hipMemcpyAsync(io, L.goff.get<uint64_t>(), ((uint64_t) L.ng + 1) * 8, hipMemcpyDeviceToDevice, st));
 }
-static void cluster_list(const bk_pair *pairs, PairList &L, double w, int fast, DevBuf &cl, ClusterBufs &cb, AhcBufs &ab, hipStream_t st)
+static void cluster_list(const bk_pair *pairs, PairList &L, double w, int fast, DevBuf &cl, ClusterBufs &cb, AhcBufs &ab, hipStream_t st, bool small_dropped = false)
 {
   if (fast)
-    fast_cluster_all(pairs, L, w, cl, cb, st);
+    fast_cluster_all(pairs, L, w, cl, cb, st, small_dropped);
   else
     ahc_cluster_all(pairs, L, w, cl, ab, cb, st);
 }
@@ -429,6 +429,7 @@
   const bk_pair *pairs = in.jr.pairs;
   auto mask_lane = [&](int l, bool observe) {
     ClusterBufs &cb = lane(l).cb;
+    PairList &L = lane(l).list;
     if (observe)
     {
       cb.heavy_x.assign(ng, 0u);
@@ -436,9 +437,9 @@
       cb.observe = true;
       cb.se.heavy_all = false;
     }
-    remove_isolated_begin(pairs, in.jr.gof, in.jr.gstart, ng, in.jr.n_pairs, w, lane(l).list, cb, lane_st(l), lane_drop(l), in.gstart_host.data(), keep[l].data());
+    remove_isolated_begin(pairs, in.jr.gof, in.jr.gstart, ng, in.jr.n_pairs, w, L, cb, lane_st(l), lane_drop(l), in.gstart_host.data(), keep[l].data());
     if (observe) cb.heavy_x.assign(ng, 0u);
-    remove_isolated_end(pairs, lane(l).list, cb, lane_st(l));
+    remove_isolated_end(pairs, L, cb, lane_st(l));
     if (observe) cb.observe = false;
   };
   auto cluster_lane = [&](int l) {
@@ -461,25 +462,37 @@
     });
   else
   {
-    in_lanes([&](int l) { mask_lane(l, true); });
-    PairList &mid = cs.lane_mid;
-    merge_all(&ClusterStage::Lane::list, mid, nullptr);
-    std::vector<uint64_t> goff_h((size_t) ng + 1);
-    HIP_CHECK(hipMemcpyAsync(goff_h.data(), mid.goff.get<uint64_t>(), ((size_t) ng + 1) * 8, hipMemcpyDeviceToHost, in.st));
-    HIP_CHECK(hipStreamSynchronize(in.st));
-    std::vector<uint64_t> sizes(ng);
+    std::vector<std::vector<uint64_t>> goff_old(K, std::vector<uint64_t>((size_t) ng + 1, 0)), goff_new(K, std::vector<uint64_t>((size_t) ng + 1, 0));
+    in_lanes([&](int l) {
+      mask_lane(l, true);
+      PairList &L = lane(l).list, &iso = lane(l).iso;
+      iso.n = L.n;
+      iso.ng = L.ng;
+      snapshot_list(L, iso.idx, &iso.gof, iso.goff, lane_st(l));
+      HIP_CHECK(hipMemcpyAsync(goff_old[l].data(), L.goff.get<uint64_t>(), ((size_t) ng + 1) * 8, hipMemcpyDeviceToHost, lane_st(l)));
+    });
+    std::vector<uint64_t> sizes(ng, 0);
     std::vector<uint32_t> hx(ng, 0u), hy(ng, 0u);
-    for (uint32_t g = 0; g < ng; ++g) sizes[g] = goff_h[g + 1] - goff_h[g];
     for (int l = 0; l < K; ++l)
       for (uint32_t g = 0; g < ng; ++g)
       {
+        sizes[g] += goff_old[l][g + 1] - goff_old[l][g];
         hx[g] = std::max(hx[g], lane(l).cb.heavy_x[g]);
         hy[g] = std::max(hy[g], lane(l).cb.heavy_y[g]);
       }
-    upload_plan(plan_observed(sizes, hx, hy, K));
+    if (bk_debug("lanes"))
+      for (int l = 0; l < K; ++l) fprintf(stderr, "[lanes] lane %d: %llu pairs after masking\n", l, (unsigned long long) lane(l).iso.n);
+    const LanePlan deal = plan_observed(sizes, hx, hy, K);
+    std::vector<const PairList *> part1(K);
+    for (int l = 0; l < K; ++l)
+    {
+      for (uint32_t g = 0; g < ng; ++g) goff_new[l][g + 1] = goff_new[l][g] + (deal[g] == l && sizes[g] >= 2 ? sizes[g] : 0);
+      part1[l] = &lane(l).iso;
+    }
+    phase("lanes dealt again");
     in_lanes([&](int l) {
-      list_subset_ranges(mid, goff_h.data(), keep[l].data(), lane(l).list, lane_st(l));
-      cluster_lane(l);
+      gather_groups_many(part1.data(), K, goff_new[l].data(), ng, lane(l).list, lane_st(l));
+      cluster_list(pairs, lane(l).list, w, fast, lane(l).d_cluster, lane(l).cb, cs.ab, lane_st(l), true);
     });
   }
   phase("lanes done");
diff --git a/include/breakid_hip.h b/include/breakid_hip.h
--- a/include/breakid_hip.h
+++ b/include/breakid_hip.h
@@ -309,6 +309,8 @@
 int bk_debug_ahc(bk_ctx *ctx, const uint32_t *x, const uint32_t *y, uint32_t n, double w, uint32_t *idx_out, int32_t *cluster_out, uint32_t *n_out);
 
 int bk_debug_points(bk_ctx *ctx, int mode, const uint32_t *x, const uint32_t *y, uint32_t n, double w, uint32_t *idx_out, int32_t *cluster_out, uint32_t *n_out);
+int bk_debug_key_match(bk_ctx *ctx, int mode, const uint32_t *k1, const uint32_t *k2, const uint64_t *group_off, uint32_t n_groups, uint32_t *cluster_out, uint32_t *keep_out,
+                       int *mode_out);
 int bk_debug_cigar(bk_ctx *ctx, uint32_t n, const uint8_t *kind, const uint32_t *c1_off, const uint8_t *c1, const uint32_t *c2_off, const uint8_t *c2, const int32_t *e,
                    int32_t *out6);
 int bk_debug_vote(bk_ctx *ctx, const bk_split *side1, uint32_t n1, const bk_split *side2, uint32_t n2, int32_t p1_tid, int32_t p2_tid, int32_t *out3);
```

New measurement: 11920, median of 6. 1.8% higher.
